# ALRhub/fancy_gym

Measured on AMD Instinct MI355X. Metric: MP trajectories/sec (7-DoF, 5 basis, 100 steps) at 1/2/4/8 GPUs; % roofline, higher is better.
Workload: dtype f32; 1 GPU; cfg2: ProDMP 7-DoF, 5 basis(+goal), 100 steps, exp phase tau=1.5, alpha=10; trajectory (pos, vel) + PD tracking-controller actions, fused; batch_per_gpu=4096, global_batch=4096, launch=hipgraph

## Files before the change

fancy_gym_amd/_lib.py:

```python
from __future__ import annotations

import ctypes as C
import os
from typing import Optional

_HERE = os.path.dirname(os.path.abspath(__file__))
LIB_PATH = os.environ.get("MPK_LIB") or os.path.join(_HERE, "libmpk.so")

MPK_ABI_VERSION = 4
MP_TYPES = {"promp": 0, "dmp": 1, "prodmp": 2}
PHASE_TYPES = {"linear": 0, "exp": 1}
BASIS_TYPES = {"rbf": 0, "zero_rbf": 1, "prodmp": 2}
CTRL_TYPES = {"motor": 0, "velocity": 1, "position": 2}
PLANT_TYPES = {"static": 0, "double_integrator": 1, "velocity_direct": 2}

MPK_EINVAL, MPK_ENOTIMPL, MPK_EHIP, MPK_ERANGE, MPK_ENODEV, MPK_ECOMM = -1, -2, -3, -4, -5, -6
MPK_COMM_ID_BYTES = 128
MPK_OPT_AUTO = -1
RELATIVE_GOAL_MODES = {"before_scale": 0, "after_scale": 1}
GOAL_OFFSET_MODES = {"ignore": 0, "add": 1}
SINGLE_RBF_MODES = {"unit_gap": 0, "refuse": 1}
DMP_FIRST_SAMPLE_MODES = {"init": 0, "step": 1}
REWARD_TYPES = {None: 0, "none": 0, "simple_reacher": 1}
AGG_MODES = {"sum": 0, "mean": 1, "last": 2}
OPTION_KEYS = ("mapping", "bulk", "quad", "pd_quad", "write_through", "ipw", "phase", "phase_table", "phase_chunk",
               "pd_simple", "split", "lds_pad", "pipe", "flat", "phase_flat", "ring", "ring_np", "ring_ns", "ring_m", "ring_dbg", "ring_parts", "tiles_wpb", "serial_order", "ring_nc", "pd_generic", "dmp_response", "ablations", "ring_tb", "pd_helper", "phase_waves", "phase_split", "phase_pipe", "pd_pipe", "hole_sampled", "vjp_generic")


class MPKLibraryError(RuntimeError):
    """libmpk.so is missing / failed to load / reported a HIP failure."""


class mpk_config(C.Structure):
    _fields_ = [
        ("abi_version", C.c_int32), ("device", C.c_int32),
        ("mp_type", C.c_int32), ("phase_type", C.c_int32), ("basis_type", C.c_int32),
        ("num_dof", C.c_int32), ("num_basis", C.c_int32), ("num_basis_outside", C.c_int32),
        ("num_basis_zero_start", C.c_int32), ("num_basis_zero_goal", C.c_int32),
        ("learn_tau", C.c_int32), ("learn_delay", C.c_int32),
        ("auto_scale_basis", C.c_int32), ("relative_goal", C.c_int32),
        ("disable_goal", C.c_int32), ("disable_weights", C.c_int32),
        ("pre_compute_length_factor", C.c_int32),
        ("relative_goal_mode", C.c_int32), ("goal_offset_mode", C.c_int32), ("single_rbf_mode", C.c_int32),
        ("dmp_first_sample", C.c_int32), ("reserved0", C.c_int32),
        ("tau", C.c_double), ("delay", C.c_double), ("alpha_phase", C.c_double),
        ("tau_bound", C.c_double * 2), ("delay_bound", C.c_double * 2),
        ("basis_bandwidth_factor", C.c_double), ("basis_alpha", C.c_double), ("basis_dt", C.c_double),
        ("weights_scale", C.c_double), ("goal_scale", C.c_double), ("dmp_alpha", C.c_double),
        ("dt", C.c_double), ("duration", C.c_double), ("goal_offset", C.c_double),
    ]


class mpk_rollout_cfg(C.Structure):
    _fields_ = [
        ("controller_type", C.c_int32), ("plant_type", C.c_int32), ("dt", C.c_double),
        ("p_gains", C.POINTER(C.c_double)), ("d_gains", C.POINTER(C.c_double)),
        ("act_low", C.POINTER(C.c_double)), ("act_high", C.POINTER(C.c_double)),
    ]


class mpk_validity_gate(C.Structure):
    _fields_ = [
        ("pos_low", C.POINTER(C.c_double)), ("pos_high", C.POINTER(C.c_double)),
        ("check_tau_delay", C.c_int32), ("reserved0", C.c_int32),
        ("tau_bound", C.c_double * 2), ("delay_bound", C.c_double * 2),
        ("raw_params", C.c_void_p), ("valid", C.c_void_p), ("penalty", C.c_void_p),
    ]


class mpk_hole_task(C.Structure):
    _fields_ = [
        ("collision_penalty", C.c_double), ("allow_self_collision", C.c_int32), ("allow_wall_collision", C.c_int32),
        ("steps_before_reward", C.c_int32), ("rew_fct", C.c_int32),
    ]


HOLE_REW_FCTS = {"simple": 0, "vel_acc": 1, "unbounded": 2}


def hole_rew_fct(rew_fct: str, steps_before_reward: int) -> int:
    if rew_fct not in HOLE_REW_FCTS:
        raise ValueError("Unknown reward function {}".format(rew_fct))
    if rew_fct != "simple" and int(steps_before_reward) != 199:
        raise ValueError(f"rew_fct {rew_fct!r} pays at the reference's step 199: steps_before_reward must be 199, "
                         f"got {steps_before_reward}")
    return HOLE_REW_FCTS[rew_fct]


RESET_ENVS = {"simple_reacher": 0, "hole_reacher": 1}


class mpk_reacher_reset_task(C.Structure):
    _fields_ = [
        ("env", C.c_int32), ("random_start", C.c_int32), ("target", C.c_double * 2),
        ("hole_width", C.c_double), ("hole_x", C.c_double), ("hole_depth", C.c_double),
        ("seed_base", C.c_uint64), ("seed_base_given", C.c_int32), ("reserved0", C.c_int32), ("reserved1", C.c_int64 * 2),
    ]


class mpk_obs_cfg(C.Structure):
    _fields_ = [
        ("env", C.c_int32), ("n_links", C.c_int32), ("col_mask", C.c_uint64), ("time_div", C.c_double), ("reserved", C.c_int64 * 2),
    ]


class mpk_env_step_task(C.Structure):
    _fields_ = [
        ("env", C.c_int32), ("n_links", C.c_int32), ("dt", C.c_double), ("max_episode_steps", C.c_int32), ("autoreset", C.c_int32),
        ("hole", mpk_hole_task), ("reserved", C.c_int64 * 2),
    ]


class mpk_replan_state(C.Structure):
    _fields_ = [
        ("traj_steps", C.c_void_p), ("plan_steps", C.c_void_p), ("done", C.c_void_p), ("seg_len", C.c_void_p),
        ("done_out", C.c_void_p), ("cond_pos", C.c_void_p), ("cond_vel", C.c_void_p),
        ("every", C.c_int32), ("max_planning_times", C.c_int32), ("horizon", C.c_int32), ("reserved0", C.c_int32),
    ]


_vp, _i32, _dbl = C.c_void_p, C.c_int32, C.c_double

SIGNATURES = {
    "mpk_last_error": (C.c_char_p, []),
    "mpk_abi_version": (C.c_int, []),
    "mpk_source_hash": (C.c_char_p, []),
    "mpk_device_count": (C.c_int, []),
    "mpk_create": (C.c_int, [C.POINTER(mpk_config), C.POINTER(_vp)]),
    "mpk_destroy": (None, [_vp]),
    "mpk_num_params": (C.c_int, [_vp]),
    "mpk_num_steps": (C.c_int, [_vp]),
    "mpk_num_dof": (C.c_int, [_vp]),
    "mpk_params_bounds": (C.c_int, [_vp, _vp, _vp]),
    "mpk_set_duration": (C.c_int, [_vp, _dbl, _dbl]),
    "mpk_set_option": (C.c_int, [_vp, C.c_char_p, C.c_int64]),
    "mpk_get_option": (C.c_int, [_vp, C.c_char_p, C.POINTER(C.c_int64)]),
    "mpk_times": (C.c_int, [_vp, _vp]),
    "mpk_trajectory": (C.c_int, [_vp, _vp, _vp, _vp, _vp, _dbl, _vp, _vp, _i32, _vp]),
    "mpk_trajectory_actions": (C.c_int, [_vp, _vp, _vp, _vp, _dbl, C.POINTER(mpk_rollout_cfg), _vp, _vp,
                                         _vp, _vp, _vp, _i32, _vp]),
    "mpk_trajectory_rollout": (C.c_int, [_vp, _vp, _vp, _vp, _dbl, C.POINTER(mpk_rollout_cfg), _vp, _vp, _vp,
                                         _vp, _vp, _vp, _i32, _vp]),
    "mpk_episode_reset": (C.c_int, [_vp, _vp, _vp, _vp, _vp, _vp, _vp, _vp, _vp, _vp, _i32, _vp]),
    "mpk_replan_step": (C.c_int, [_vp, _vp, _vp, _vp, _dbl, C.POINTER(mpk_rollout_cfg), _vp, _vp,
                                  C.POINTER(mpk_replan_state), _vp, _vp, _vp, _i32, _vp]),
    "mpk_episode_return": (C.c_int, [_vp, _vp, _vp, _vp, _dbl, C.POINTER(mpk_rollout_cfg), _vp, _vp, C.POINTER(mpk_replan_state),
                                     _vp, _vp, _i32, _vp, _vp, _i32, _i32, _vp, _i32, _vp]),
    "mpk_replan_step_gated": (C.c_int, [_vp, _vp, _vp, _vp, _dbl, C.POINTER(mpk_rollout_cfg), _vp, _vp,
                                        C.POINTER(mpk_replan_state), C.POINTER(mpk_validity_gate), _vp, _vp, _vp, _i32, _vp]),
    "mpk_episode_return_gated": (C.c_int, [_vp, _vp, _vp, _vp, _dbl, C.POINTER(mpk_rollout_cfg), _vp, _vp, C.POINTER(mpk_replan_state),
                                           C.POINTER(mpk_validity_gate), _vp, _vp, _i32, _vp, _vp, _i32, _i32, _vp, _i32, _vp]),
    "mpk_reward_aggregate": (C.c_int, [_vp, _vp, _vp, _i32, _vp, _i32, _i32, _vp]),
    "mpk_pd_rollout": (C.c_int, [_vp, C.POINTER(mpk_rollout_cfg), _vp, _vp, _vp, _vp, _vp, _vp, _i32, _i32, _vp]),
    "mpk_condition_gather": (C.c_int, [_vp, _vp, _vp, _vp, _vp, _vp, _i32, _i32, _vp]),
    "mpk_unpin_tables": (C.c_int, [_vp]),
    "mpk_check_range": (C.c_int, [_vp, _vp]),
    "mpk_poll_fault": (C.c_int, [_vp]),
    "mpk_gate_flags": (C.c_int, [_vp, _vp, _vp, _vp, _vp, _vp, _i32, _vp]),
    "mpk_reacher_rollout": (C.c_int, [_vp, C.POINTER(mpk_rollout_cfg), _vp, _vp, _vp, _vp, _vp, _vp, _vp, _i32, _vp,
                                      _vp, _i32, _i32, _vp]),
    "mpk_hole_reacher_rollout": (C.c_int, [_vp, C.POINTER(mpk_rollout_cfg), _vp, _vp, _vp, _vp, _vp, _vp, C.POINTER(mpk_hole_task),
                                           _vp, _vp, _vp, _vp, _i32, _vp, _vp, _vp, C.POINTER(mpk_replan_state), _i32, _i32, _vp]),
    "mpk_hole_reacher_rollout2": (C.c_int, [_vp, C.POINTER(mpk_rollout_cfg), _vp, _vp, _vp, _vp, _vp, _vp, C.POINTER(mpk_hole_task),
                                            _vp, _vp, _vp, _vp, _i32, _vp, _vp, _vp, C.POINTER(mpk_replan_state), _vp, _i32, _i32,
                                            _vp]),
    "mpk_reacher_reset": (C.c_int, [_vp, C.POINTER(mpk_reacher_reset_task), _vp, _vp, _vp, _vp, _vp, _vp, _vp, _vp, _vp, _vp,
                                    _i32, _vp]),
    "mpk_reacher_observation": (C.c_int, [_vp, C.POINTER(mpk_obs_cfg), _vp, _vp, _vp, _vp, _vp, _i32, _vp]),
    "mpk_reacher_step_observations": (C.c_int, [_vp, C.POINTER(mpk_obs_cfg), C.POINTER(mpk_rollout_cfg), _vp, _vp, _vp, _vp, _vp, _vp,
                                                _vp, _vp, _vp, _vp, _i32, _i32, _vp]),
    "mpk_replan_advance": (C.c_int, [_vp, _vp, _vp, _vp, _vp, _i32, _i32, _i32, _i32, _i32, _vp]),
    "mpk_traj_validity": (C.c_int, [_vp, _vp, _vp, _vp, _vp, _i32, _vp, _vp, _vp, _i32, _i32, _vp]),
    "mpk_traj_validity_penalty": (C.c_int, [_vp, _vp, _vp, _vp, _vp, _i32, _vp, _vp, _vp, _vp, _i32, _i32, _vp]),
    "mpk_prodmp_tables": (C.c_int, [_vp, _vp, _vp, _vp, _vp, _vp, _vp, _vp]),
    "mpk_prodmp_indices": (C.c_int, [_vp, _dbl, _vp, _vp, _vp]),
    "mpk_scaled_basis": (C.c_int, [_vp, _vp, _i32, _vp, _vp]),
    "mpk_selftest_division": (C.c_int, [_vp, C.c_float, C.c_uint32, C.c_uint64, C.POINTER(C.c_uint64), _vp]),
    "mpk_host_prodmp_tables": (C.c_int, [C.POINTER(mpk_config), _vp, _vp, _vp, _vp, _vp, _vp, _vp, _vp]),
    "mpk_host_rbf": (C.c_int, [C.POINTER(mpk_config), _vp, _vp]),
    "mpk_host_times": (C.c_int, [_dbl, _dbl, _vp, _i32]),
    "mpk_host_num_params": (C.c_int, [C.POINTER(mpk_config)]),
    "mpk_comm_unique_id": (C.c_int, [_vp]),
    "mpk_comm_create": (C.c_int, [_vp, _i32, _i32, _i32, C.POINTER(_vp)]),
    "mpk_comm_rank": (C.c_int, [_vp]),
    "mpk_comm_world": (C.c_int, [_vp]),
    "mpk_allgather": (C.c_int, [_vp, _vp, _vp, C.c_int64, _vp]),
    "mpk_comm_destroy": (None, [_vp]),
    "mpk_last_kernel": (C.c_char_p, [_vp]),
    "mpk_reacher_autoreset": (C.c_int, [_vp, C.POINTER(mpk_reacher_reset_task), C.POINTER(mpk_obs_cfg), _vp, _vp, _vp, _vp, _vp, _vp,
                                        _vp, _vp, _vp, _vp, _vp, _vp, _vp, _vp, _i32, _vp]),
    "mpk_reacher_env_step": (C.c_int, [_vp, C.POINTER(mpk_env_step_task), C.POINTER(mpk_reacher_reset_task), _vp, _vp, _vp, _vp, _vp,
                                       _vp, _vp, _vp, _vp, _vp, _vp, _vp, _vp, _vp, _vp, _i32, _vp]),
    "mpk_trajectory_vjp": (C.c_int, [_vp, _vp, _vp, _dbl, _vp, _vp, _vp, _i32, _vp]),
    "mpk_reacher_rollout_vjp": (C.c_int, [_vp, C.POINTER(mpk_rollout_cfg), _vp, _vp, _vp, _vp, _vp, _vp, _vp, _i32, _vp, _vp, _vp,
                                          _vp, _vp, _vp, _vp, _vp, _i32, _i32, _vp]),
}

_lib: Optional[C.CDLL] = None

_ROOT = os.path.dirname(_HERE)
KERNEL_UNITS = ("mpk_traj_family.hip", "mpk_traj_ring.hip", "mpk_episode.hip", "mpk_traj_launch.hip", "mpk_traj_wide.hip", "mpk_traj_vjp.hip", "mpk_traj_phase.hip",
                "mpk_phase_fused.hip", "mpk_rollout.hip", "mpk_rollout_vjp.hip", "mpk_hole.hip", "mpk_reset.hip", "mpk_obs.hip", "mpk_autoreset.hip", "mpk_env_step.hip", "mpk_misc.hip")
KERNEL_HEADERS = ("mpk_dev.h", "mpk_tile.h", "mpk_traj_tiles.h", "mpk_traj_stream.h", "mpk_traj_flat.h", "mpk_traj_ring.h", "mpk_traj_quad.h",
                  "mpk_traj_pipe.h", "mpk_traj_route.h", "mpk_reward.h", "mpk_phase.h", "mpk_trace_reader.h", "mpk_nprng.h", "mpk_plant.h", "mpk_reacher_env.h", "mpk_hole_geom.h")
SOURCE_FILES = (os.path.join(_ROOT, "include", "mpk.h"), os.path.join(_HERE, "csrc", "mpk_internal.h"),
                os.path.join(_HERE, "csrc", "mpk_host.cpp")) + \
    tuple(os.path.join(_HERE, "csrc", f) for f in KERNEL_HEADERS + KERNEL_UNITS)


def stamp(extra_flags: str = "") -> Optional[str]:
    import hashlib
    h = source_hash()
    if h is None or not extra_flags.strip():
        return h
    return h[:48] + "f1a9" + hashlib.sha256(extra_flags.strip().encode()).hexdigest()[:12]


def source_hash() -> Optional[str]:
    import hashlib
    h = hashlib.sha256()
    for path in SOURCE_FILES:
        if not os.path.exists(path):
            return None
        h.update(os.path.basename(path).encode() + b"\n")
        with open(path, "rb") as f:
            h.update(f.read())
    return h.hexdigest()


def embedded_source_hash(path: str = None) -> Optional[str]:
    import re
    path = path or LIB_PATH
    try:
        with open(path, "rb") as f:
            m = re.search(rb"MPK_SOURCE_HASH=([0-9a-f]{64}|unstamped)", f.read())
    except OSError:
        return None
    return m.group(1).decode() if m else None


def load() -> C.CDLL:
    global _lib
    if _lib is not None:
        return _lib
    if not os.path.exists(LIB_PATH):
        raise MPKLibraryError(
            f"{LIB_PATH} not found. Build it with `python -c 'import __graft_entry__ as g; g.build()'` "
            f"(hipcc --offload-arch=gfx950). fancy_gym_amd has no CPU fallback.")
    try:
        lib = C.CDLL(LIB_PATH)
    except OSError as e:
        raise MPKLibraryError(f"cannot load {LIB_PATH}: {e}") from e
    for name, (res, args) in SIGNATURES.items():
        try:
            fn = getattr(lib, name)
        except AttributeError as e:
            raise MPKLibraryError(f"{LIB_PATH} does not export {name}") from e
        fn.restype = res
        fn.argtypes = args
    if lib.mpk_abi_version() != MPK_ABI_VERSION:
        raise MPKLibraryError("libmpk.so ABI version mismatch")
    want, got = source_hash(), (lib.mpk_source_hash() or b"").decode()
    if want is not None and "MPK_LIB" not in os.environ and got != want:
        raise MPKLibraryError(
            f"{LIB_PATH} was built from other sources (stamped {got[:12]}..., checked out {want[:12]}...). Rebuild it with "
            f"`python -c 'import __graft_entry__ as g; g.build()'`.")
    _lib = lib
    return lib


def last_error() -> str:
    msg = load().mpk_last_error()
    return msg.decode() if msg else ""


def check(rc: int) -> int:
    if rc >= 0:
        return rc
    msg = last_error()
    if rc == MPK_EINVAL:
        raise ValueError(msg)
    if rc == MPK_ENOTIMPL:
        raise NotImplementedError(msg)
    if rc == MPK_ERANGE:
        raise RuntimeError(msg)
    raise MPKLibraryError(f"libmpk error {rc}: {msg}")


def set_option(key: str, value: int = MPK_OPT_AUTO, handle=None) -> None:
    check(load().mpk_set_option(handle, key.encode(), int(value)))


def get_option(key: str, handle=None) -> int:
    v = C.c_int64()
    check(load().mpk_get_option(handle, key.encode(), C.byref(v)))
    return int(v.value)


def reset_options(handle=None) -> None:
    for k in OPTION_KEYS:
        set_option(k, MPK_OPT_AUTO, handle)
```

fancy_gym_amd/csrc/mpk_host.cpp:

```cpp
#include <hip/hip_runtime.h>
#include <dlfcn.h>

#include <cmath>
#include <cstdio>
#include <cstring>
#include <limits>
#include <map>
#include <mutex>

#include "mpk_internal.h"

namespace mpk {

static thread_local std::string g_err;
void set_error(const std::string& msg) { g_err = msg; }

#define MPK_HIP(call)                                                                          \
    do {                                                                                       \
        hipError_t e_ = (call);                                                                \
        if (e_ != hipSuccess) {                                                                \
            set_error(std::string(#call) + ": " + hipGetErrorString(e_));                      \
            return MPK_EHIP;                                                                   \
        }                                                                                      \
    } while (0)
// ... 34 lines not shown
        if (i < steps / 2) {
            prod = step * (float)i;
            v = start + prod;
        } else {
            prod = step * (float)(steps - 1 - i);
            v = end - prod;
        }
        out[i - 1] = v;
    }
    return out;
}

static double unbound_phase(const mpk_config& c, double t) {
    const double s = (t - c.delay) / c.tau;
    return c.phase_type == MPK_PHASE_LINEAR ? s : std::exp(-c.alpha_phase * s);
}
static double bound_phase(const mpk_config& c, double t) {
    double s = (t - c.delay) / c.tau;
    if (c.phase_type == MPK_PHASE_LINEAR) return std::fmin(std::fmax(s, 0.0), 1.0);
    return std::exp(-c.alpha_phase * std::fmax(s, 0.0));
}

void build_rbf(const mpk_config& c, HostTables& t) {
    int n = c.num_basis;
    int outside = c.num_basis_outside;
    if (c.basis_type == MPK_BASIS_ZERO_RBF) {
        n += c.num_basis_zero_start + c.num_basis_zero_goal;
        outside = 0;
    }
    t.n_total = n;
    t.centers.assign(n, 0.0);
    t.bw.assign(n, 0.0);
    const double dist = n > 1 ? c.tau / (double)(n - 2 * outside - 1) : c.tau;
    const double lo = -outside * dist + c.delay;
    const double hi = c.tau + outside * dist + c.delay;
    for (int k = 0; k < n; ++k) {
        double ct = n > 1 ? lo + k * ((hi - lo) / (double)(n - 1)) : lo;
        if (n > 1 && k == n - 1) ct = hi;
        t.centers[k] = unbound_phase(c, ct);
    }
    for (int k = 0; k < n; ++k) {
        double gap = 1.0;
        if (n > 1) gap = k < n - 1 ? t.centers[k + 1] - t.centers[k] : t.centers[n - 1] - t.centers[n - 2];
        t.bw[k] = c.basis_bandwidth_factor / (gap * gap);
    }
}

static void rbf_row(const HostTables& t, double x, int n_used, int first, double* out) {
    double sum = 0.0;
    std::vector<double> b(t.n_total);
    for (int k = 0; k < t.n_total; ++k) {
        const double dx = x - t.centers[k];
        b[k] = std::exp(-(dx * dx * t.bw[k]) / 2.0);
        sum += b[k];
    }
    for (int k = 0; k < n_used; ++k) out[k] = t.n_total > 1 ? b[first + k] / sum : b[first + k];
}

void build_prodmp(const mpk_config& c, HostTables& t) {
    build_rbf(c, t);
    const int nb = c.num_basis, K = nb + 1;
    const float sdt = (float)c.basis_dt / (float)c.tau;
    t.scaled_dt = sdt;
    const int per_unit = (int)std::nearbyint(1.0 / (double)sdt);
    const int N = c.pre_compute_length_factor * per_unit + 1;
    t.n_pc = N;
    t.y1.resize(N); t.y2.resize(N); t.dy1.resize(N); t.dy2.resize(N);
    t.pos_basis.assign((size_t)N * K, 0.0);
    t.vel_basis.assign((size_t)N * K, 0.0);
    t.scale.assign(K, 0.0);
    const double alpha = c.basis_alpha, half = 0.5 * alpha;
    const double L = (double)c.pre_compute_length_factor;
    const double step = L / (double)(N - 1);
    std::vector<double> s(N), dp1((size_t)N * nb), dp2((size_t)N * nb), phi(nb);
    std::vector<double> p1(nb, 0.0), p2(nb, 0.0);
    for (int i = 0; i < N; ++i) {
        s[i] = (i == N - 1) ? L : i * step;
        const double e = std::exp(half * s[i]);
        t.y1[i] = std::exp(-half * s[i]);
        t.y2[i] = s[i] * t.y1[i];
        t.dy1[i] = -half * t.y1[i];
        t.dy2[i] = -half * t.y2[i] + t.y1[i];
        const double pc_time = s[i] * c.tau + c.delay;
        const double x = bound_phase(c, pc_time);
        rbf_row(t, x, nb, 0, phi.data());
        for (int k = 0; k < nb; ++k) {
            dp1[(size_t)i * nb + k] = ((s[i] * e) * x) * phi[k];
            dp2[(size_t)i * nb + k] = (e * x) * phi[k];
        }
        if (i > 0) {
            const double ds = s[i] - s[i - 1];
            for (int k = 0; k < nb; ++k) {
                p1[k] += ds * (dp1[(size_t)i * nb + k] + dp1[(size_t)(i - 1) * nb + k]) / 2.0;
                p2[k] += ds * (dp2[(size_t)i * nb + k] + dp2[(size_t)(i - 1) * nb + k]) / 2.0;
            }
        }
        const double q1 = (half * s[i] - 1.0) * e + 1.0;
        const double q2 = half * (e - 1.0);
        for (int k = 0; k < nb; ++k) {
            t.pos_basis[(size_t)i * K + k] = p2[k] * t.y2[i] - p1[k] * t.y1[i];
            t.vel_basis[(size_t)i * K + k] = p2[k] * t.dy2[i] - p1[k] * t.dy1[i];
        }
        t.pos_basis[(size_t)i * K + nb] = q2 * t.y2[i] - q1 * t.y1[i];
        t.vel_basis[(size_t)i * K + nb] = q2 * t.dy2[i] - q1 * t.dy1[i];
    }
    for (int k = 0; k < K; ++k) {
        double m = -std::numeric_limits<double>::infinity();
        for (int i = 0; i < N; ++i) m = std::fmax(m, t.pos_basis[(size_t)i * K + k]);
        t.scale[k] = 1.0 / m;
    }
}

struct CacheEntry {
    bool valid = false;
    uint32_t key = 0;
    int T = 0;
    SharedTables st;
    size_t floats = 0;
    uint64_t stamp = 0;
    bool pinned = false, deferred = false;
    unsigned long long capture_id = 0;
};

struct Handle {
    mpk_config cfg{};
    HostTables tab;
    DevCfg dev{};
    int num_cu = 256;
    double duration = 0.0, dt = 0.0;
    std::vector<float> times;
    double* d_tab = nullptr;
    std::vector<float> rows32;
    float* d_rows32 = nullptr;
    int rows32_stride = 0;
    float* d_times = nullptr;
    int32_t* d_flag = nullptr;
    unsigned* d_tickets = nullptr;
    unsigned ticket_next = 0;
    std::vector<unsigned> ticket_free;
    std::map<std::pair<unsigned long long, uintptr_t>, unsigned> ticket_of;
    std::mutex ticket_mu;
    int* h_fault = nullptr;
    int* d_fault = nullptr;
    int32_t* d_idx = nullptr;
    int idx_cap = 0;
    static constexpr int kCache = 64;
    CacheEntry cache[kCache];
    DevCfg dev_resp{};
    bool resp_ok = false;
    CacheEntry cache_resp[kCache];
    std::string kernel_name_buf;
    uint64_t stamp = 0;
    const char* last_kernel = "";
    Tuning tune;
    float* d_pre = nullptr;
    size_t pre_cap = 0;
};

static Tuning effective_tuning(const Handle* h);

static int check_cfg(const mpk_config& c) {
    if (c.abi_version != MPK_ABI_VERSION) { set_error("mpk_config.abi_version mismatch"); return MPK_EINVAL; }
    if (c.mp_type < 0 || c.mp_type > 2) { set_error("unknown mp_type"); return MPK_EINVAL; }
    if (c.phase_type < 0 || c.phase_type > 1) { set_error("unknown phase_type"); return MPK_EINVAL; }
    if (c.basis_type < 0 || c.basis_type > 2) { set_error("unknown basis_type"); return MPK_EINVAL; }
    if (c.num_dof < 0) { set_error("num_dof must be >= 0"); return MPK_EINVAL; }
    if (c.num_basis < 1) { set_error("num_basis must be >= 1 (basis length 0 is not implemented upstream)"); return MPK_EINVAL; }
    if (c.basis_type == MPK_BASIS_PRODMP && c.phase_type != MPK_PHASE_EXP) {
        set_error("prodmp basis requires the exp phase generator");
        return MPK_EINVAL;
    }
    if ((c.mp_type == MPK_MP_PRODMP) != (c.basis_type == MPK_BASIS_PRODMP)) {
        set_error("prodmp trajectory generator and prodmp basis generator must be used together");
        return MPK_EINVAL;
    }
    if (!(c.tau > 0.0)) { set_error("tau must be > 0"); return MPK_EINVAL; }
    if (!(c.dt > 0.0) || !(c.duration > 0.0)) { set_error("dt and duration must be > 0"); return MPK_EINVAL; }
    if (c.basis_type == MPK_BASIS_PRODMP && (c.pre_compute_length_factor < 1 || c.pre_compute_length_factor > 6)) {
        set_error("pre_compute_length_factor must be in [1, 6]");
        return MPK_EINVAL;
    }
    if (c.basis_type == MPK_BASIS_RBF && c.num_basis > 1 && c.num_basis - 2 * c.num_basis_outside - 1 <= 0) {
        set_error("num_basis_outside too large for num_basis");
        return MPK_EINVAL;
    }
    if (c.mp_type == MPK_MP_PRODMP && c.disable_goal && c.disable_weights) {
        set_error("disable_goal and disable_weights cannot both be set");
        return MPK_EINVAL;
    }
    if (c.relative_goal_mode < 0 || c.relative_goal_mode > 1 || c.goal_offset_mode < 0 || c.goal_offset_mode > 1 ||
        c.single_rbf_mode < 0 || c.single_rbf_mode > 1 || c.dmp_first_sample < 0 || c.dmp_first_sample > 1) {
        set_error("relative_goal_mode, goal_offset_mode, single_rbf_mode and dmp_first_sample take 0 or 1");
        return MPK_EINVAL;
    }
    if (c.goal_offset_mode == MPK_GOAL_OFFSET_ADD && !std::isfinite(c.goal_offset)) {
        set_error("goal_offset must be finite");
        return MPK_EINVAL;
    }
    if (c.single_rbf_mode == MPK_SINGLE_RBF_REFUSE && c.basis_type != MPK_BASIS_PRODMP) {
        const int n = c.num_basis + (c.basis_type == MPK_BASIS_ZERO_RBF ? c.num_basis_zero_start + c.num_basis_zero_goal : 0);
        if (n == 1) {
            set_error("a single radial basis function has no neighbouring centre to take its bandwidth from "
                      "(single_rbf_mode = MPK_SINGLE_RBF_REFUSE)");
            return MPK_EINVAL;
        }
    }
    return MPK_OK;
}

static int local_per_dof(const mpk_config& c) {
    switch (c.mp_type) {
        case MPK_MP_PROMP: return c.num_basis;
        case MPK_MP_DMP: return c.num_basis + 1;
        default: return (c.disable_weights ? 0 : c.num_basis) + (c.disable_goal ? 0 : 1);
    }
}

static void quantise(mpk_config& q) {
    auto f32 = [](double v) { return (double)(float)v; };
    q.tau = f32(q.tau); q.delay = f32(q.delay); q.alpha_phase = f32(q.alpha_phase);
    q.basis_bandwidth_factor = f32(q.basis_bandwidth_factor); q.basis_alpha = f32(q.basis_alpha);
    q.basis_dt = f32(q.basis_dt); q.weights_scale = f32(q.weights_scale); q.goal_scale = f32(q.goal_scale);
    q.dmp_alpha = f32(q.dmp_alpha); q.goal_offset = f32(q.goal_offset);
}

static void fill_devcfg(Handle* h) {
    const mpk_config& c = h->cfg;
    DevCfg& d = h->dev;
    d = DevCfg{};
    d.mp_type = c.mp_type; d.phase_type = c.phase_type; d.basis_type = c.basis_type;
    d.D = c.num_dof; d.nb = c.num_basis; d.n_total = h->tab.n_total;
    d.zs = c.basis_type == MPK_BASIS_ZERO_RBF ? c.num_basis_zero_start : 0;
    const bool zero_pad = c.basis_type == MPK_BASIS_ZERO_RBF;
    {
        const HostTables& t = h->tab;
        bool uni = c.basis_type != MPK_BASIS_PRODMP && c.phase_type == MPK_PHASE_LINEAR && t.n_total >= 2;
        if (uni) {
            const int n = t.n_total;
            const double D = (t.centers[n - 1] - t.centers[0]) / (double)(n - 1);
            for (int k = 0; k < n && uni; ++k)
                uni = std::fabs(t.centers[k] - (t.centers[0] + k * D)) <= 1e-12 * std::fabs(D) * n &&
                      std::fabs(t.bw[k] - t.bw[0]) <= 1e-12 * t.bw[0];
            const double span = std::fmax(std::fabs(1.0 - t.centers[0]), std::fabs(0.0 - t.centers[0])) + std::fabs(D) * n;
            uni = uni && 0.5 * t.bw[0] * span * span < 600.0;
        }
        d.rbf_uniform = uni ? 1 : 0;
    }
    d.relgoal_before_scale = c.relative_goal_mode == MPK_RELGOAL_BEFORE_SCALE ? 1 : 0;
    d.goal_off_on = c.mp_type == MPK_MP_PRODMP && c.goal_offset_mode == MPK_GOAL_OFFSET_ADD && c.goal_offset != 0.0 ? 1 : 0;
    d.goal_offset = (float)c.goal_offset;
    if (c.mp_type == MPK_MP_PRODMP) d.KT = c.num_basis + 3 + d.goal_off_on;
    else if (c.mp_type == MPK_MP_PROMP) d.KT = c.num_basis + (zero_pad ? 1 : 0);
    else d.KT = c.num_basis;
    d.KP = (d.KT + 3) / 4 * 4;
    d.Kloc = local_per_dof(c);
    d.off = (c.learn_tau ? 1 : 0) + (c.learn_delay ? 1 : 0);
    d.P = d.off + d.D * d.Kloc;
    d.T = steps_for(h->duration, h->dt);
    d.learn_tau = c.learn_tau; d.learn_delay = c.learn_delay;
    d.relative_goal = c.relative_goal; d.disable_goal = c.disable_goal; d.disable_weights = c.disable_weights;
    d.n_pc = h->tab.n_pc; d.len_factor = c.pre_compute_length_factor;
    d.tau = (float)c.tau; d.delay = (float)c.delay; d.alpha_phase = (float)c.alpha_phase;
    d.scaled_dt = h->tab.scaled_dt;
    d.tau_lo = (float)c.tau_bound[0]; d.tau_hi = (float)c.tau_bound[1];
    d.delay_lo = (float)c.delay_bound[0]; d.delay_hi = (float)c.delay_bound[1];
    d.ws = (float)c.weights_scale; d.gs = (float)c.goal_scale;
    d.dmp_alpha = (float)c.dmp_alpha; d.dmp_beta = (float)(c.dmp_alpha / 4.0);
    d.tab = h->d_tab;
    d.rows32 = h->d_rows32;
    d.rows32_stride = h->rows32_stride;
    d.base_times = h->d_times;
    d.t_last = h->times.empty() ? 0.f : h->times.back();
    h->resp_ok = false;
    h->dev_resp = d;
    if (c.mp_type == MPK_MP_DMP && !c.learn_tau && !c.learn_delay && d.D >= 1 && d.D <= kMaxD && c.num_basis + 3 <= kMaxKP &&
        !h->times.empty()) {
        float ds_max = 0.f;
        for (size_t i = 0; i + 1 < h->times.size(); ++i) {
            const float s0 = std::fmax((h->times[i] - d.delay) / d.tau, 0.f), s1 = std::fmax((h->times[i + 1] - d.delay) / d.tau, 0.f);
            ds_max = std::fmax(ds_max, s1 - s0);
        }
        DevCfg& r = h->dev_resp;
        r.mp_type = MPK_MP_PRODMP;
        r.dmp_resp = 1;
        r.rows32 = nullptr; r.rows32_stride = 0;
        r.KT = c.num_basis + 3;
        r.KP = (r.KT + 3) / 4 * 4;
        r.relative_goal = 0; r.disable_goal = 0; r.disable_weights = 0; r.goal_off_on = 0;
        h->resp_ok = (double)d.dmp_alpha * (double)ds_max <= 1.0;
    }
}

static int upload_times(Handle* h) {
    const int T = steps_for(h->duration, h->dt);
    if (T < 1) { set_error("duration/dt gives no time steps"); return MPK_EINVAL; }
    h->times = build_times(h->duration, T);
    if (h->d_times) { (void)hipFree(h->d_times); h->d_times = nullptr; }
    MPK_HIP(hipMalloc((void**)&h->d_times, sizeof(float) * T));
    MPK_HIP(hipMemcpy(h->d_times, h->times.data(), sizeof(float) * T, hipMemcpyHostToDevice));
    for (auto& e : h->cache) { e.valid = false; e.pinned = false; e.deferred = false; }
    for (auto& e : h->cache_resp) { e.valid = false; e.pinned = false; e.deferred = false; }
    return MPK_OK;
}

static void free_handle(Handle* h) {
    if (!h) return;
// ... 167 lines not shown
int mpk_create(const mpk_config* cfg, mpk_handle* out) {
    if (!cfg || !out) { set_error("NULL argument"); return MPK_EINVAL; }
    int rc = check_cfg(*cfg);
    if (rc != MPK_OK) return rc;
    int ndev = 0;
    if (hipGetDeviceCount(&ndev) != hipSuccess || ndev <= 0) {
        set_error("no HIP device visible: libmpk has no CPU fallback");
        return MPK_ENODEV;
    }
    if (cfg->device < 0 || cfg->device >= ndev) { set_error("device ordinal out of range"); return MPK_EINVAL; }
    MPK_ON_DEVICE(cfg->device);
    Handle* h = new Handle();
    h->cfg = *cfg;
    quantise(h->cfg);
    cfg = &h->cfg;
    h->duration = cfg->duration; h->dt = cfg->dt;
    hipDeviceProp_t prop;
    if (hipGetDeviceProperties(&prop, cfg->device) == hipSuccess) h->num_cu = prop.multiProcessorCount;
    std::vector<double> packed;
    if (cfg->basis_type == MPK_BASIS_PRODMP) {
        build_prodmp(*cfg, h->tab);
        const HostTables& t = h->tab;
        packed.reserve((size_t)t.n_pc * (4 + 2 * (cfg->num_basis + 1)));
        packed.insert(packed.end(), t.y1.begin(), t.y1.end());
        packed.insert(packed.end(), t.y2.begin(), t.y2.end());
        packed.insert(packed.end(), t.dy1.begin(), t.dy1.end());
        packed.insert(packed.end(), t.dy2.begin(), t.dy2.end());
        packed.insert(packed.end(), t.pos_basis.begin(), t.pos_basis.end());
        packed.insert(packed.end(), t.vel_basis.begin(), t.vel_basis.end());
        for (int k = 0; k <= cfg->num_basis; ++k) {
            float sc = k < cfg->num_basis ? (float)cfg->weights_scale : (float)cfg->goal_scale;
            if (cfg->auto_scale_basis) sc = (float)t.scale[k] * sc;
            packed.push_back((double)sc);
        }
        const int K = cfg->num_basis + 1;
        if (K + 2 <= 16) {
            const int KS = K + 2 <= 8 ? 8 : 16, RS = 2 * KS + 4;
            h->rows32.assign((size_t)t.n_pc * RS, 0.0f);
            h->rows32_stride = RS;
            for (int i = 0; i < t.n_pc; ++i) {
                float* r = h->rows32.data() + (size_t)i * RS;
                for (int kk = 0; kk < K; ++kk) {
                    r[2 * kk] = (float)t.pos_basis[(size_t)i * K + kk];
                    r[2 * kk + 1] = (float)t.vel_basis[(size_t)i * K + kk];
                }
                const double v[4] = {t.y1[i], t.y2[i], t.dy1[i], t.dy2[i]};
                std::memcpy(r + 2 * KS - 4, v, sizeof(v));
            }
        }
    } else {
        build_rbf(*cfg, h->tab);
        packed.insert(packed.end(), h->tab.centers.begin(), h->tab.centers.end());
        packed.insert(packed.end(), h->tab.bw.begin(), h->tab.bw.end());
        {
            const int n = h->tab.n_total;
            const double D = n > 1 ? (h->tab.centers[n - 1] - h->tab.centers[0]) / (double)(n - 1) : 0.0;
            const double bw0 = h->tab.bw[0];
            packed.push_back(bw0 * D);
            packed.push_back(0.5 * bw0 * D * D);
            packed.push_back(std::exp(-bw0 * D * D));
        }
    }
    auto fail = [&](int code) { free_handle(h); return code; };
    if (hipMalloc((void**)&h->d_tab, packed.size() * sizeof(double)) != hipSuccess) { set_error("hipMalloc(tables) failed"); return fail(MPK_EHIP); }
    if (hipMemcpy(h->d_tab, packed.data(), packed.size() * sizeof(double), hipMemcpyHostToDevice) != hipSuccess) { set_error("hipMemcpy(tables) failed"); return fail(MPK_EHIP); }
    if (!h->rows32.empty()) {
        if (hipMalloc((void**)&h->d_rows32, h->rows32.size() * sizeof(float)) != hipSuccess) { set_error("hipMalloc(row table) failed"); return fail(MPK_EHIP); }
        if (hipMemcpy(h->d_rows32, h->rows32.data(), h->rows32.size() * sizeof(float), hipMemcpyHostToDevice) != hipSuccess) { set_error("hipMemcpy(row table) failed"); return fail(MPK_EHIP); }
    }
    if (hipMalloc((void**)&h->d_flag, sizeof(int32_t)) != hipSuccess) { set_error("hipMalloc(flag) failed"); return fail(MPK_EHIP); }
    if (hipMemset(h->d_flag, 0, sizeof(int32_t)) != hipSuccess) { set_error("hipMemset(flag) failed"); return fail(MPK_EHIP); }
    if (hipHostMalloc((void**)&h->h_fault, 64, hipHostMallocMapped) != hipSuccess) { set_error("hipHostMalloc(fault word) failed"); return fail(MPK_EHIP); }
    *h->h_fault = 0;
    if (hipHostGetDevicePointer((void**)&h->d_fault, h->h_fault, 0) != hipSuccess) { set_error("hipHostGetDevicePointer(fault word) failed"); return fail(MPK_EHIP); }
    if (hipMalloc((void**)&h->d_tickets, kTicketSlots * 128) != hipSuccess) { set_error("hipMalloc(ticket counters) failed"); return fail(MPK_EHIP); }
    if (hipMemset(h->d_tickets, 0, kTicketSlots * 128) != hipSuccess) { set_error("hipMemset(ticket counters) failed"); return fail(MPK_EHIP); }
    rc = upload_times(h);
    if (rc != MPK_OK) return fail(rc);
    fill_devcfg(h);
    if (const int nf = fast_rows_floats(h->dev)) {
        if (hipMalloc((void**)&h->d_rows32, (size_t)nf * sizeof(float)) != hipSuccess) { set_error("hipMalloc(forcing-row table) failed"); return fail(MPK_EHIP); }
        rc = launch_fast_rows_table(h->dev, h->d_rows32, nullptr);
        if (rc != MPK_OK) return fail(rc);
        if (hipDeviceSynchronize() != hipSuccess) { set_error("forcing-row table kernel failed"); return fail(MPK_EHIP); }
        h->rows32_stride = fast_rows_stride(h->dev);
        fill_devcfg(h);
    }
    rc = prealloc_cache(h);
    if (rc != MPK_OK) return fail(rc);
    *out = reinterpret_cast<mpk_handle>(h);
    return MPK_OK;
}

void mpk_destroy(mpk_handle hh) { free_handle(reinterpret_cast<Handle*>(hh)); }

int mpk_num_params(mpk_handle hh) {
    if (!hh) { set_error("NULL handle"); return MPK_EINVAL; }
    return reinterpret_cast<Handle*>(hh)->dev.P;
}
int mpk_num_steps(mpk_handle hh) {
    if (!hh) { set_error("NULL handle"); return MPK_EINVAL; }
    return reinterpret_cast<Handle*>(hh)->dev.T;
}
int mpk_num_dof(mpk_handle hh) {
    if (!hh) { set_error("NULL handle"); return MPK_EINVAL; }
    return reinterpret_cast<Handle*>(hh)->dev.D;
}

int mpk_params_bounds(mpk_handle hh, float* low, float* high) {
    if (!hh || !low || !high) { set_error("NULL argument"); return MPK_EINVAL; }
    Handle* h = reinterpret_cast<Handle*>(hh);
    int i = 0;
    if (h->cfg.learn_tau) { low[i] = (float)h->cfg.tau_bound[0]; high[i] = (float)h->cfg.tau_bound[1]; ++i; }
    if (h->cfg.learn_delay) { low[i] = (float)h->cfg.delay_bound[0]; high[i] = (float)h->cfg.delay_bound[1]; ++i; }
    for (; i < h->dev.P; ++i) { low[i] = -std::numeric_limits<float>::infinity(); high[i] = std::numeric_limits<float>::infinity(); }
    return MPK_OK;
}

int mpk_set_duration(mpk_handle hh, double duration, double dt) {
    if (!hh) { set_error("NULL handle"); return MPK_EINVAL; }
    Handle* h = reinterpret_cast<Handle*>(hh);
    if (!(duration > 0.0) || !(dt > 0.0)) { set_error("dt and duration must be > 0"); return MPK_EINVAL; }
    if (duration == h->duration && dt == h->dt) return MPK_OK;
    MPK_ON_DEVICE(h->cfg.device);
    MPK_HIP(hipDeviceSynchronize());
    h->duration = duration; h->dt = dt;
    release_capture_tickets(h);
    int rc = upload_times(h);
    if (rc != MPK_OK) return rc;
    fill_devcfg(h);
    return prealloc_cache(h);
}

namespace {
struct OptKey { const char* name; int Tuning::*field; int64_t lo, hi; };
const OptKey kOptKeys[] = {
    {"mapping", &Tuning::mapping, 0, 2},         {"bulk", &Tuning::bulk, 0, 2},
    {"quad", &Tuning::quad, 0, 4},               {"pd_quad", &Tuning::pd_quad, 0, 3},
    {"write_through", &Tuning::write_through, 0, 1}, {"ipw", &Tuning::ipw, 0, 1 << 20},
    {"phase", &Tuning::phase, 0, 1},             {"phase_table", &Tuning::phase_table, 0, 1},
    {"phase_chunk", &Tuning::phase_chunk, 0, 16}, {"pd_simple", &Tuning::pd_simple, 0, 1},
    {"split", &Tuning::split, 0, 1},             {"lds_pad", &Tuning::lds_pad, 0, 48},
    {"pipe", &Tuning::pipe, 0, 1},               {"flat", &Tuning::flat, 0, 1},
    {"phase_flat", &Tuning::phase_flat, 0, 1},   {"ring", &Tuning::ring, 0, 2},
    {"ring_np", &Tuning::ring_np, 1, 14},        {"ring_ns", &Tuning::ring_ns, 1, 8},
    {"ring_m", &Tuning::ring_m, 1, 8},           {"ring_dbg", &Tuning::ring_dbg, 0, 255},
    {"ring_parts", &Tuning::ring_parts, 1, 8},   {"tiles_wpb", &Tuning::tiles_wpb, 1, 8},
    {"serial_order", &Tuning::serial_order, 0, 2}, {"ring_nc", &Tuning::ring_nc, 1, 6},
    {"pd_generic", &Tuning::pd_generic, 0, 1},   {"dmp_response", &Tuning::dmp_response, 0, 1},
    {"ablations", &Tuning::ablations, 0, 1},     {"ring_tb", &Tuning::ring_tb, 1, 64},
    {"pd_helper", &Tuning::pd_helper, 0, 1},     {"phase_waves", &Tuning::phase_waves, 1, 32},
    {"phase_split", &Tuning::phase_split, 1, 64},   {"phase_pipe", &Tuning::phase_pipe, 0, 1},
    {"pd_pipe", &Tuning::pd_pipe, 0, 1},         {"hole_sampled", &Tuning::hole_sampled, 0, 1},
    {"vjp_generic", &Tuning::vjp_generic, 0, 1},
};
const OptKey* find_opt(const char* key) {
    if (!key) return nullptr;
    for (const OptKey& k : kOptKeys)
        if (std::strcmp(k.name, key) == 0) return &k;
    return nullptr;
}
}

namespace mpk {
static Tuning effective_tuning(const Handle* h) {
    Tuning t = g_tune;
    for (const OptKey& k : kOptKeys)
        if (h->tune.*(k.field) >= 0) t.*(k.field) = h->tune.*(k.field);
    return t;
}
}

int mpk_set_option(mpk_handle hh, const char* key, int64_t value) {
    const OptKey* k = find_opt(key);
    if (!k) { set_error(std::string("unknown option key: ") + (key ? key : "(null)")); return MPK_EINVAL; }
    if (value != MPK_OPT_AUTO && (value < k->lo || value > k->hi)) {
        set_error(std::string("option value out of range for ") + key);
        return MPK_EINVAL;
    }
    Tuning& t = hh ? reinterpret_cast<Handle*>(hh)->tune : g_tune;
    t.*(k->field) = (int)value;
    return MPK_OK;
}

int mpk_get_option(mpk_handle hh, const char* key, int64_t* value) {
    const OptKey* k = find_opt(key);
    if (!k || !value) { set_error(std::string("unknown option key: ") + (key ? key : "(null)")); return MPK_EINVAL; }
    const Tuning t = hh ? effective_tuning(reinterpret_cast<Handle*>(hh)) : g_tune;
    *value = t.*(k->field);
    return MPK_OK;
}

int mpk_check_range(mpk_handle hh, void* stream) {
    if (!hh) { set_error("NULL handle"); return MPK_EINVAL; }
    Handle* h = reinterpret_cast<Handle*>(hh);
    MPK_ON_DEVICE(h->cfg.device);
    int32_t flag = 0;
    MPK_HIP(hipMemcpyAsync(&flag, h->d_flag, sizeof(flag), hipMemcpyDeviceToHost, (hipStream_t)stream));
    MPK_HIP(hipStreamSynchronize((hipStream_t)stream));
    {
        const int fr = pending_ring_fault(h);
        if (fr != MPK_OK) {
            if (flag) {
                MPK_HIP(hipMemsetAsync(h->d_flag, 0, sizeof(flag), (hipStream_t)stream));
                set_error(std::string(mpk_last_error()) + "; ALSO: Time is beyond the pre-computation range. Set larger pre-computation factor");
            }
            return fr;
        }
    }
    if (!flag) return MPK_OK;
    MPK_HIP(hipMemsetAsync(h->d_flag, 0, sizeof(flag), (hipStream_t)stream));
    set_error("Time is beyond the pre-computation range. Set larger pre-computation factor");
    return MPK_ERANGE;
}

int mpk_poll_fault(mpk_handle hh) {
    if (!hh) { set_error("NULL handle"); return MPK_EINVAL; }
    return pending_ring_fault(reinterpret_cast<Handle*>(hh));
}

static void release_capture_tickets(Handle* h) {
    std::lock_guard<std::mutex> lock(h->ticket_mu);
    for (auto it = h->ticket_of.begin(); it != h->ticket_of.end();) {
        if (it->first.first != 0ull) { h->ticket_free.push_back(it->second); it = h->ticket_of.erase(it); }
        else ++it;
    }
}

int mpk_unpin_tables(mpk_handle hh) {
    if (!hh) { set_error("NULL handle"); return MPK_EINVAL; }
    Handle* h = reinterpret_cast<Handle*>(hh);
    release_capture_tickets(h);
    for (auto* cache : {h->cache, h->cache_resp})
        for (int i = 0; i < Handle::kCache; ++i) {
            CacheEntry& e = cache[i];
            if (e.pinned) { e.pinned = false; if (e.deferred) e.valid = false; e.deferred = false; }
        }
    return MPK_OK;
}

int mpk_times(mpk_handle hh, float* times) {
    if (!hh || !times) { set_error("NULL argument"); return MPK_EINVAL; }
    Handle* h = reinterpret_cast<Handle*>(hh);
    std::memcpy(times, h->times.data(), sizeof(float) * h->times.size());
    return MPK_OK;
}

static unsigned* ticket_slot(Handle* h, void* stream) {
    unsigned long long cap_id = 0;
    hipStreamCaptureStatus cs = hipStreamCaptureStatusNone;
    if (hipStreamGetCaptureInfo((hipStream_t)stream, &cs, &cap_id) != hipSuccess) { (void)hipGetLastError(); cs = hipStreamCaptureStatusNone; }
    if (cs != hipStreamCaptureStatusActive) cap_id = 0;
    std::lock_guard<std::mutex> lock(h->ticket_mu);
    const auto key = std::make_pair(cap_id, reinterpret_cast<uintptr_t>(stream));
    auto it = h->ticket_of.find(key);
    if (it == h->ticket_of.end()) {
        unsigned slot;
        if (!h->ticket_free.empty()) { slot = h->ticket_free.back(); h->ticket_free.pop_back(); }
        else if (h->ticket_next < kTicketSlots) slot = h->ticket_next++;
        else return nullptr;
        it = h->ticket_of.emplace(key, slot).first;
    }
    return h->d_tickets + (size_t)it->second * 32;
}

static int pending_ring_fault(Handle* h) {
    if (!h->h_fault) return MPK_OK;
    const int f = __atomic_exchange_n(h->h_fault, 0, __ATOMIC_RELAXED);
    if (!(f & 2)) { if (f) __atomic_fetch_or(h->h_fault, f & ~2, __ATOMIC_RELAXED); return MPK_OK; }
    char msg[512];
    std::snprintf(msg, sizeof msg, "k_traj_ring: a wave of an earlier launch on this handle gave up waiting for its partner (role mask 0x%x: "
                  "1 producer / buffer, 2 ticket, 4 store engine / batch, 8 action writer, 16 consumer / tile, 32 consumer / writer, 64 reward helper, 128 k_phase_fused pipeline, 256 rollout pipeline, 512 k_reacher_reset goal draw at its rejection cap): "
                  "outputs (closed loop: plant and replanning state too) of that launch are incomplete", (unsigned)f >> 8);
    set_error(msg);
    return MPK_EHIP;
}

static bool fused_capable(const Handle* h) {
    if (!shared_phase(h, nullptr)) return false;
    if (h->cfg.mp_type == MPK_MP_DMP) return dmp_response(h, nullptr, effective_tuning(h));
    return mfma_capable(h);
}

static bool fused_phase_capable(const Handle* h) {
    return !shared_phase(h, nullptr) && h->cfg.mp_type != MPK_MP_DMP && phase_fused_capable(h->dev);
}

static int fill_gate(const Handle* h, const mpk_validity_gate* g, GateDev* out) {
    if (!g->pos_low || !g->pos_high || !g->valid) { set_error("validity gate: NULL pos_low / pos_high / valid"); return MPK_EINVAL; }
    if (h->dev.D > kMaxD) { set_error("validity gate: num_dof too large"); return MPK_EINVAL; }
    for (int d = 0; d < h->dev.D; ++d) { out->lo[d] = g->pos_low[d]; out->hi[d] = g->pos_high[d]; }
    out->check_td = g->check_tau_delay ? 1 : 0;
    if (out->check_td && h->dev.P < 2) { set_error("validity gate: check_tau_delay needs at least two parameters per episode"); return MPK_EINVAL; }
    out->tau_b[0] = g->tau_bound[0]; out->tau_b[1] = g->tau_bound[1];
    out->delay_b[0] = g->delay_bound[0]; out->delay_b[1] = g->delay_bound[1];
    out->raw_params = g->raw_params; out->valid = g->valid; out->penalty = g->penalty;
    return MPK_OK;
}

static int phase_fused_common(Handle* h, const float* params, const float* init_pos, const float* init_vel, double init_time_shared,
                              float* pos, float* vel, float* actions, const RolloutDev& rd, double* q, double* qd,
                              const int32_t* n_steps, const ReplanDev* rp, const GateDev* gate, double* ret, int32_t* seg_out,
                              int32_t B, void* stream) {
    if (!params || !init_pos || !init_vel) { set_error("NULL buffer"); return MPK_EINVAL; }
    {
        const int fr = pending_ring_fault(h);
        if (fr != MPK_OK) return fr;
    }
    return launch_phase_fused(h->dev, params, init_pos, init_vel, (float)init_time_shared, pos, vel, actions, rd, q, qd, n_steps, rp,
                              gate, ret, seg_out, h->d_flag, B, h->num_cu, stream, &h->last_kernel, effective_tuning(h), h->d_fault);
}

static int traj_common(Handle* h, const float* params, const float* init_pos, const float* init_vel,
                       const float* init_time, double init_time_shared, float* pos, float* vel, float* actions,
                       const RolloutDev* rd, const double* c_pos, const double* c_vel, int32_t B, void* stream,
                       double* q_state = nullptr, double* qd_state = nullptr, const int32_t* n_steps = nullptr,
                       const ReplanDev* rp = nullptr, const GateDev* gate = nullptr) {
    if (B < 0) { set_error("B must be >= 0"); return MPK_EINVAL; }
    if (B == 0 || h->dev.D == 0) return MPK_OK;
    if (!params || !init_pos || !init_vel || !pos || !vel) { set_error("NULL buffer"); return MPK_EINVAL; }
    MPK_ON_DEVICE(h->cfg.device);
    {
        const int fr = pending_ring_fault(h);
        if (fr != MPK_OK) return fr;
    }
    const Tuning tune = effective_tuning(h);
    if (h->cfg.mp_type == MPK_MP_DMP && h->cfg.dmp_first_sample == MPK_DMP_FIRST_IS_STEP) {
        const size_t need = (size_t)B * h->dev.D;
        if (need > h->pre_cap) {
            hipStreamCaptureStatus cs = hipStreamCaptureStatusNone;
            if (hipStreamIsCapturing((hipStream_t)stream, &cs) == hipSuccess && cs == hipStreamCaptureStatusActive) {
                set_error("MPK_DMP_FIRST_IS_STEP: run one eager call with this batch size before capturing a graph");
                return MPK_EINVAL;
            }
            if (h->d_pre) { MPK_HIP(hipDeviceSynchronize()); (void)hipFree(h->d_pre); h->d_pre = nullptr; h->pre_cap = 0; }
            MPK_HIP(hipMalloc((void**)&h->d_pre, 2 * need * sizeof(float)));
            h->pre_cap = need;
        }
        float* p1 = h->d_pre;
        float* v1 = h->d_pre + h->pre_cap;
        int rc = launch_dmp_prestep(h->dev, params, init_pos, init_vel, init_time, (float)init_time_shared, p1, v1, B, stream);
        if (rc != MPK_OK) return rc;
        init_pos = p1; init_vel = v1;
    }
    if (shared_phase(h, init_time) && wide_capable(h) && !actions && !q_state && !rp && traj_wide_fits(h->dev)) {
        SharedTables st;
        int rc = get_shared(h, (float)init_time_shared, stream, &st);
        if (rc != MPK_OK) return rc;
        rc = launch_traj_wide(h->dev, st, params, init_pos, init_vel, pos, vel, B, h->num_cu, stream, &h->last_kernel);
        if (rc != MPK_ENOTIMPL) return rc;
    }
    if (dmp_response(h, init_time, tune)) {
        SharedTables st;
        int rc = get_shared(h, (float)init_time_shared, stream, &st, true);
        if (rc != MPK_OK) return rc;
        unsigned* ticket = ticket_slot(h, stream);
        const char* name = "";
        rc = launch_traj_shared(h->dev_resp, st, params, init_pos, init_vel, pos, vel, actions, rd, c_pos, c_vel,
                                q_state, qd_state, n_steps, B, h->num_cu, stream, &name, tune, rp, ticket, h->d_fault, gate);
        if (rc == MPK_OK) {
            h->kernel_name_buf = name;
            const size_t at = h->kernel_name_buf.find("prodmp");
            if (at != std::string::npos) h->kernel_name_buf.replace(at, 6, "dmp_resp");
            h->last_kernel = h->kernel_name_buf.c_str();
        }
        if (rc != MPK_ENOTIMPL || actions) return rc;
    }
    if (shared_phase(h, init_time) && mfma_capable(h)) {
        SharedTables st;
        int rc = get_shared(h, (float)init_time_shared, stream, &st);
        if (rc != MPK_OK) return rc;
        unsigned* ticket = ticket_slot(h, stream);
        rc = launch_traj_shared(h->dev, st, params, init_pos, init_vel, pos, vel, actions, rd, c_pos, c_vel,
                                q_state, qd_state, n_steps, B, h->num_cu, stream, &h->last_kernel, tune, rp, ticket, h->d_fault, gate);
        if (rc != MPK_ENOTIMPL || actions) return rc;
    }
    if (actions) { set_error("fused actions need a shared-phase configuration with D <= 16 and <= 16 basis columns"); return MPK_ENOTIMPL; }
    return launch_traj_rows(h->dev, params, init_pos, init_vel, init_time, (float)init_time_shared, pos, vel,
                            h->d_flag, B, h->num_cu, stream, &h->last_kernel, tune);
}

int mpk_trajectory(mpk_handle hh, const float* params, const float* init_pos, const float* init_vel,
                   const float* init_time, double init_time_shared, float* pos, float* vel, int32_t B,
                   void* stream) {
    if (!hh) { set_error("NULL handle"); return MPK_EINVAL; }
    return traj_common(reinterpret_cast<Handle*>(hh), params, init_pos, init_vel, init_time, init_time_shared,
                       pos, vel, nullptr, nullptr, nullptr, nullptr, B, stream);
}

int mpk_trajectory_vjp(mpk_handle hh, const float* g_pos, const float* g_vel, double init_time_shared, float* g_params,
                       float* g_init_pos, float* g_init_vel, int32_t B, void* stream) {
    if (!hh) { set_error("NULL handle"); return MPK_EINVAL; }
    Handle* h = reinterpret_cast<Handle*>(hh);
    if (B < 0) { set_error("B must be >= 0"); return MPK_EINVAL; }
    if (h->cfg.learn_tau || h->cfg.learn_delay) {
        set_error("mpk_trajectory_vjp: a learned tau / delay makes the trajectory non-linear in those two parameters (and they are "
                  "clipped to their bounds): only shared-phase handles are differentiable");
        return MPK_ENOTIMPL;
    }
    const Tuning tune = effective_tuning(h);
    const bool dmp = h->cfg.mp_type == MPK_MP_DMP;
    if (dmp && (h->cfg.dmp_first_sample == MPK_DMP_FIRST_IS_STEP || !dmp_response(h, nullptr, tune))) {
        set_error("mpk_trajectory_vjp: a DMP handle is differentiable on its response route only (<= 16 DoF, <= 13 basis functions, "
                  "alpha ds <= 1, dmp_first_sample = init, option \"dmp_response\" not 0)");
        return MPK_ENOTIMPL;
    }
    if (B == 0 || h->dev.D == 0 || (!g_params && !g_init_pos && !g_init_vel)) return MPK_OK;
    MPK_ON_DEVICE(h->cfg.device);
    SharedTables st;
    int rc = get_shared(h, (float)init_time_shared, stream, &st, dmp);
    if (rc != MPK_OK) return rc;
    return launch_traj_vjp(dmp ? h->dev_resp : h->dev, st, g_pos, g_vel, g_params, g_init_pos, g_init_vel, B, h->num_cu, stream,
                           &h->last_kernel, tune);
}

int mpk_trajectory_actions(mpk_handle hh, const float* params, const float* init_pos, const float* init_vel,
                           double init_time_shared, const mpk_rollout_cfg* rc, const double* c_pos,
                           const double* c_vel, float* pos, float* vel, float* actions, int32_t B, void* stream) {
    if (!hh) { set_error("NULL handle"); return MPK_EINVAL; }
    Handle* h = reinterpret_cast<Handle*>(hh);
    if (B == 0) return MPK_OK;
    if (!actions || !c_pos || !c_vel) { set_error("NULL buffer"); return MPK_EINVAL; }
    RolloutDev rd;
    int r = fill_rollout(h, rc, &rd);
    if (r != MPK_OK) return r;
    MPK_ON_DEVICE(h->cfg.device);
    if (rd.plant_type != MPK_PLANT_STATIC) { set_error("mpk_trajectory_actions tracks a frozen state (MPK_PLANT_STATIC); use mpk_trajectory_rollout"); return MPK_EINVAL; }
    if (fused_capable(h)) {
        r = traj_common(h, params, init_pos, init_vel, nullptr, init_time_shared, pos, vel, actions, &rd, c_pos, c_vel,
                        B, stream);
        if (r != MPK_ENOTIMPL) return r;
    } else if (fused_phase_capable(h) && B > 0 && pos && vel) {
        r = phase_fused_common(h, params, init_pos, init_vel, init_time_shared, pos, vel, actions, rd, const_cast<double*>(c_pos),
                               const_cast<double*>(c_vel), nullptr, nullptr, nullptr, nullptr, nullptr, B, stream);
        if (r != MPK_ENOTIMPL) return r;
    }
    r = traj_common(h, params, init_pos, init_vel, nullptr, init_time_shared, pos, vel, nullptr, nullptr, nullptr,
                    nullptr, B, stream);
    if (r != MPK_OK) return r;
    return launch_pd_rollout(rd, h->dev.D, pos, vel, const_cast<double*>(c_pos), const_cast<double*>(c_vel), nullptr,
                             actions, B, h->dev.T, stream, effective_tuning(h), h->d_fault);
}

int mpk_trajectory_rollout(mpk_handle hh, const float* params, const float* init_pos, const float* init_vel,
                           double init_time_shared, const mpk_rollout_cfg* rc, double* q, double* qd,
                           const int32_t* n_steps, float* pos, float* vel, float* actions, int32_t B, void* stream) {
    if (!hh) { set_error("NULL handle"); return MPK_EINVAL; }
    Handle* h = reinterpret_cast<Handle*>(hh);
    if (B == 0) return MPK_OK;
    if (!actions || !q || !qd) { set_error("NULL buffer"); return MPK_EINVAL; }
    RolloutDev rd;
    int r = fill_rollout(h, rc, &rd);
    if (r != MPK_OK) return r;
    MPK_ON_DEVICE(h->cfg.device);
    if (rd.plant_type != MPK_PLANT_DOUBLE_INTEGRATOR) { set_error("mpk_trajectory_rollout integrates MPK_PLANT_DOUBLE_INTEGRATOR; for a frozen state use mpk_trajectory_actions"); return MPK_EINVAL; }
    if (fused_capable(h)) {
        r = traj_common(h, params, init_pos, init_vel, nullptr, init_time_shared, pos, vel, actions, &rd, nullptr,
                        nullptr, B, stream, q, qd, n_steps);
        if (r != MPK_ENOTIMPL) return r;
    } else if (fused_phase_capable(h) && B > 0 && pos && vel) {
        r = phase_fused_common(h, params, init_pos, init_vel, init_time_shared, pos, vel, actions, rd, q, qd, n_steps, nullptr, nullptr,
                               nullptr, nullptr, B, stream);
        if (r != MPK_ENOTIMPL) return r;
    }
    r = traj_common(h, params, init_pos, init_vel, nullptr, init_time_shared, pos, vel, nullptr, nullptr, nullptr,
                    nullptr, B, stream);
    if (r != MPK_OK) return r;
    return launch_pd_rollout(rd, h->dev.D, pos, vel, q, qd, n_steps, actions, B, h->dev.T, stream, effective_tuning(h), h->d_fault);
}

int mpk_replan_step_gated(mpk_handle hh, const float* params, const float* init_pos, const float* init_vel,
                          double init_time_shared, const mpk_rollout_cfg* rc, double* q, double* qd,
                          const mpk_replan_state* st, const mpk_validity_gate* gate, float* pos, float* vel, float* actions,
                          int32_t B, void* stream) {
    if (!hh) { set_error("NULL handle"); return MPK_EINVAL; }
    Handle* h = reinterpret_cast<Handle*>(hh);
    if (B < 0) { set_error("B must be >= 0"); return MPK_EINVAL; }
    if (B == 0) return MPK_OK;
    if (!st || !st->traj_steps || !st->plan_steps || !st->done || !st->seg_len) { set_error("NULL replanning state"); return MPK_EINVAL; }
    if ((st->cond_pos == nullptr) != (st->cond_vel == nullptr)) { set_error("cond_pos and cond_vel go together"); return MPK_EINVAL; }
    if (st->every < 1 || st->horizon < 1) { set_error("every and horizon must be >= 1"); return MPK_EINVAL; }
    if (!actions || !q || !qd) { set_error("NULL buffer"); return MPK_EINVAL; }
    if (st->cond_pos && (st->cond_pos == init_pos || st->cond_vel == init_vel)) { set_error("cond_pos / cond_vel must not alias init_pos / init_vel"); return MPK_EINVAL; }
    RolloutDev rd;
    int r = fill_rollout(h, rc, &rd);
    if (r != MPK_OK) return r;
    if (rd.plant_type != MPK_PLANT_DOUBLE_INTEGRATOR) { set_error("mpk_replan_step integrates MPK_PLANT_DOUBLE_INTEGRATOR"); return MPK_EINVAL; }
    GateDev gd;
    if (gate) {
        r = fill_gate(h, gate, &gd);
        if (r != MPK_OK) return r;
    }
    MPK_ON_DEVICE(h->cfg.device);
    ReplanDev rp;
    rp.traj_steps = st->traj_steps; rp.plan_steps = st->plan_steps; rp.done = st->done; rp.seg_len = st->seg_len;
    rp.done_out = st->done_out; rp.cond_pos = st->cond_pos; rp.cond_vel = st->cond_vel;
    rp.every = st->every; rp.max_planning_times = st->max_planning_times; rp.horizon = st->horizon;
    if (fused_capable(h)) {
        r = traj_common(h, params, init_pos, init_vel, nullptr, init_time_shared, pos, vel, actions, &rd, nullptr,
                        nullptr, B, stream, q, qd, nullptr, &rp, gate ? &gd : nullptr);
        if (r != MPK_ENOTIMPL) return r;
    } else if (fused_phase_capable(h) && pos && vel) {
        r = phase_fused_common(h, params, init_pos, init_vel, init_time_shared, pos, vel, actions, rd, q, qd, nullptr, &rp,
                               gate ? &gd : nullptr, nullptr, nullptr, B, stream);
        if (r != MPK_ENOTIMPL) return r;
    }
    r = traj_common(h, params, init_pos, init_vel, nullptr, init_time_shared, pos, vel, nullptr, nullptr, nullptr,
                    nullptr, B, stream);
    if (r != MPK_OK) return r;
    if (gate) {
        r = launch_validity(pos, gd.raw_params ? gd.raw_params : params, h->dev.P, h->dev.D, gd.lo, gd.hi, gd.check_td, gd.tau_b, gd.delay_b,
                            gd.valid, gd.penalty, B, h->dev.T, stream);
        if (r != MPK_OK) return r;
    }
    r = launch_replan_advance(rp.traj_steps, rp.plan_steps, rp.seg_len, rp.done, rp.every, rp.max_planning_times,
                              rp.horizon, h->dev.T, B, stream, gate ? gd.valid : nullptr);
    if (r != MPK_OK) return r;
    if (rp.done_out) MPK_HIP(hipMemcpyAsync(rp.done_out, rp.done, (size_t)B, hipMemcpyDeviceToDevice, (hipStream_t)stream));
    r = launch_pd_rollout(rd, h->dev.D, pos, vel, q, qd, rp.seg_len, actions, B, h->dev.T, stream, effective_tuning(h), h->d_fault);
    if (r != MPK_OK) return r;
    if (rp.cond_pos) return launch_condition_gather(pos, vel, rp.seg_len, rp.cond_pos, rp.cond_vel, B, h->dev.T, h->dev.D, stream);
    return MPK_OK;
}

int mpk_replan_step(mpk_handle hh, const float* params, const float* init_pos, const float* init_vel,
                    double init_time_shared, const mpk_rollout_cfg* rc, double* q, double* qd,
                    const mpk_replan_state* st, float* pos, float* vel, float* actions, int32_t B, void* stream) {
// ... 724 lines not shown
```

fancy_gym_amd/csrc/mpk_internal.h:

```cpp
#pragma once
#include <cstdint>
#include <string>
#include <vector>

#include "mpk.h"

namespace mpk {

constexpr int kMaxKP = 16;
constexpr int kMaxD = 16;
constexpr int kMaxDofArgs = 32;

struct HostTables {
    int n_total = 0;
    std::vector<double> centers, bw;
    int n_pc = 0;
    float scaled_dt = 0.f;
    std::vector<double> y1, y2, dy1, dy2, pos_basis, vel_basis, scale;
};

void build_rbf(const mpk_config& c, HostTables& t);
void build_prodmp(const mpk_config& c, HostTables& t);
std::vector<float> build_times(double duration, int T);
int steps_for(double duration, double dt);

struct Tuning {
    int mapping = -1, bulk = -1, quad = -1, pd_quad = -1, write_through = -1, ipw = -1, phase = -1, phase_table = -1,
        phase_chunk = -1, pd_simple = -1, split = -1, lds_pad = -1, pipe = -1, flat = -1, phase_flat = -1,
        ring = -1, ring_np = -1, ring_ns = -1, ring_m = -1, ring_dbg = -1, ring_parts = -1, tiles_wpb = -1, serial_order = -1, ring_nc = -1,
        pd_generic = -1, dmp_response = -1, ablations = -1, ring_tb = -1, pd_helper = -1, phase_waves = -1, phase_split = -1, phase_pipe = -1, pd_pipe = -1,
        hole_sampled = -1, vjp_generic = -1;
};

struct DevCfg {
    int mp_type, phase_type, basis_type;
    int D, nb, n_total, zs;
    int KT, KP;
    int P, Kloc, off;
    int T;
    int learn_tau, learn_delay, relative_goal, disable_goal, disable_weights;
    int rbf_uniform;
    int relgoal_before_scale;
    int dmp_resp;
    int goal_off_on;
    float goal_offset;
    int n_pc, len_factor;
    float tau, delay, alpha_phase, scaled_dt;
    float tau_lo, tau_hi, delay_lo, delay_hi;
    float ws, gs, dmp_alpha, dmp_beta;
    const double* tab;
    const float* rows32;
    int rows32_stride;
    const float* base_times;
    float t_last;
};

struct RolloutDev {
    int controller_type, plant_type;
    double dt;
    double pg[kMaxDofArgs], dg[kMaxDofArgs], lo[kMaxDofArgs], hi[kMaxDofArgs];
};

struct ReplanDev {
    int32_t* traj_steps = nullptr;
    int32_t* plan_steps = nullptr;
    uint8_t* done = nullptr;
    int32_t* seg_len = nullptr;
    uint8_t* done_out = nullptr;
    float* cond_pos = nullptr;
    float* cond_vel = nullptr;
    int every = 1, max_planning_times = 0, horizon = 0;
};

inline float f32_at_least(double x) {
    float f = (float)x;
    if ((double)f < x) f = __builtin_nextafterf(f, __builtin_inff());
    return f;
}
inline float f32_at_most(double x) {
    float f = (float)x;
    if ((double)f > x) f = __builtin_nextafterf(f, -__builtin_inff());
    return f;
}

struct GateDev {
    double lo[kMaxD], hi[kMaxD];
    int check_td = 0;
    double tau_b[2] = {0.0, 0.0}, delay_b[2] = {0.0, 0.0};
    const float* raw_params = nullptr;
    uint8_t* valid = nullptr;
    double* penalty = nullptr;
};

struct SharedTables {
    float* A = nullptr;
    float* aux = nullptr;
    int TS = 0, n_out = 0;
};

struct Handle;

int launch_build_shared(const DevCfg& c, float init_time, const SharedTables& st, int32_t* idx_out,
                        int32_t* range_flag, void* stream);
int launch_traj_shared(const DevCfg& c, const SharedTables& st, const float* params, const float* init_pos,
                       const float* init_vel, float* pos, float* vel, float* actions, const RolloutDev* rc,
                       const double* c_pos, const double* c_vel, double* q_state, double* qd_state,
                       const int32_t* n_steps, int B, int num_cu, void* stream, const char** kernel_name,
                       const Tuning& tune, const ReplanDev* rp = nullptr, unsigned* ticket = nullptr, int* fault = nullptr,
                       const GateDev* gate = nullptr);
int launch_episode_return(const DevCfg& c, const SharedTables& st, const float* params, const float* init_pos, const float* init_vel,
                          const RolloutDev& rc, double* q_state, double* qd_state, const int32_t* n_steps, const ReplanDev* rp,
                          int reward_type, const double* goal, const int32_t* step0, int steps_before_reward, int agg, double* ret,
                          int32_t* seg_out, int B, int num_cu, void* stream, const char** kernel_name, const Tuning& tune,
                          const GateDev* gate = nullptr);
int launch_reward_aggregate(const double* rewards, const int32_t* seg_len, int agg, double* out, int B, int T, void* stream);
int launch_traj_wide(const DevCfg& c, const SharedTables& st, const float* params, const float* init_pos,
                     const float* init_vel, float* pos, float* vel, int B, int num_cu, void* stream,
                     const char** kernel_name);
int launch_traj_vjp(const DevCfg& c, const SharedTables& st, const float* g_pos, const float* g_vel, float* g_params, float* g_init_pos,
                    float* g_init_vel, int B, int num_cu, void* stream, const char** kernel_name, const Tuning& tune);
int launch_traj_rows(const DevCfg& c, const float* params, const float* init_pos, const float* init_vel,
                     const float* init_time, float init_time_shared, float* pos, float* vel, int32_t* range_flag,
                     int B, int num_cu, void* stream, const char** kernel_name, const Tuning& tune);
int launch_pd_rollout(const RolloutDev& rc, int D, const float* des_pos, const float* des_vel, double* q,
                      double* qd, const int32_t* n_steps, float* actions, int B, int T, void* stream,
                      const Tuning& tune, int* fault = nullptr);
bool phase_fused_capable(const DevCfg& c);
int launch_phase_fused(const DevCfg& c, const float* params, const float* init_pos, const float* init_vel, float init_time_shared,
                       float* pos, float* vel, float* actions, const RolloutDev& rc, double* q, double* qd, const int32_t* n_steps,
                       const ReplanDev* rp, const GateDev* gate, double* ret, int32_t* seg_out, int32_t* range_flag, int B, int num_cu,
                       void* stream, const char** kernel_name, const Tuning& tune, int* fault);
int fast_rows_floats(const DevCfg& c);
int fast_rows_stride(const DevCfg& c);
int launch_fast_rows_table(const DevCfg& c, float* out, void* stream);
int launch_dmp_prestep(const DevCfg& c, const float* params, const float* init_pos, const float* init_vel,
                       const float* init_time, float init_time_shared, float* pos1, float* vel1, int B, void* stream);
int launch_condition_gather(const float* pos, const float* vel, const int32_t* seg_len, float* cond_pos, float* cond_vel,
                            int B, int T, int D, void* stream);
int launch_reacher_rollout(const RolloutDev& rc, int D, const float* des_pos, const float* des_vel, double* q,
                           double* qd, const int32_t* n_steps, const int32_t* step0, const double* goal,
                           int steps_before_reward, float* actions, double* rewards, int B, int T, void* stream,
                           const Tuning& tune, int* fault);
int launch_reacher_rollout_vjp(const RolloutDev& rc, int D, const float* des_pos, const float* des_vel, const double* q0,
                               const double* qd0, const int32_t* n_steps, const int32_t* step0, const double* goal,
                               int steps_before_reward, const double* g_rewards, const double* g_q, const double* g_qd,
                               float* g_des_pos, float* g_des_vel, double* g_q0, double* g_qd0, double* g_goal, int B, int T,
                               void* stream, const char** kernel_name);
struct HoleLaunch {
    RolloutDev rc;
    const float* des_pos = nullptr;
    const float* des_vel = nullptr;
    double* q = nullptr;
    double* qd = nullptr;
    const int32_t* n_steps = nullptr;
    const int32_t* step0 = nullptr;
    const double* hole = nullptr;
    float* actions = nullptr;
    double* rewards = nullptr;
    double* ret = nullptr;
    int32_t* n_exec = nullptr;
    uint8_t* collided = nullptr;
    uint8_t* success = nullptr;
    ReplanDev rp;
    double penalty = 0.0;
    int allow_self = 0, allow_wall = 0, steps_before_reward = 0, agg = 0;
    int rew_fct = 0;
    double* reward_state = nullptr;
};
int launch_hole_rollout(const HoleLaunch& h, int B, int T, int D, void* stream, const Tuning& tune);
int launch_episode_reset(const double* init_q, const double* init_qd, double* q, double* qd, float* cond_pos,
                         float* cond_vel, int32_t* traj_steps, int32_t* plan_steps, uint8_t* done, int B, int D,
                         void* stream);
struct ResetLaunch {
    const uint64_t* seeds = nullptr;
    uint64_t seed_base = 0;
    int seeded_base = 0;
    void* rng = nullptr;
    double* q = nullptr;
    double* qd = nullptr;
    float* cond_pos = nullptr;
    float* cond_vel = nullptr;
    int32_t* traj_steps = nullptr;
    int32_t* plan_steps = nullptr;
    uint8_t* done = nullptr;
    double* task_out = nullptr;
    double target[2] = {0.0, 0.0};
    double hole_width = 0.0, hole_x = 0.0, hole_depth = 0.0;
    int env = 0, random_start = 0;
};
int launch_reacher_reset(const ResetLaunch& l, int B, int D, void* stream, int* fault);
struct ObsLaunch {
    uint64_t mask = 0;
    double time_div = 0.0;
    int env = 0, D = 0, n_full = 0, n_out = 0;
};
int launch_reacher_obs(const ObsLaunch& l, const double* q, const double* qd, const double* task, const int32_t* steps, float* out,
                       int B, void* stream);
int launch_reacher_step_obs(const ObsLaunch& l, const RolloutDev& rc, const float* des_pos, const float* des_vel, const double* q0,
                            const double* qd0, const double* task, const int32_t* n_exec, const int32_t* step0, float* out,
                            double* q_end, double* qd_end, int B, int T, void* stream);
int launch_reacher_autoreset(const ResetLaunch& l, const ObsLaunch* o, const uint8_t* mask, uint8_t* reset_mask, float* final_obs,
                             float* obs, int B, int D, void* stream, int* fault);
struct EnvStepLaunch {
    ResetLaunch reset;
    ObsLaunch obs_layout;
    const float* actions = nullptr;
    double* reward_state = nullptr;
    double* reward = nullptr;
    uint8_t* terminated = nullptr;
    uint8_t* truncated = nullptr;
    uint8_t* collided = nullptr;
    uint8_t* success = nullptr;
    uint8_t* reset_mask = nullptr;
    float* final_obs = nullptr;
    float* obs = nullptr;
    double dt = 0.0, penalty = 0.0;
    int allow_self = 0, allow_wall = 0, steps_before_reward = 0, max_steps = 0, autoreset = 0, rew_fct = 0;
};
int launch_reacher_env_step(const EnvStepLaunch& e, int B, int D, void* stream, int* fault);
int launch_gate_flags(const uint8_t* valid, const uint8_t* was_done, const uint8_t* done, uint8_t* terminated, uint8_t* truncated, int B,
                      void* stream);
int launch_replan_advance(int32_t* traj_steps, int32_t* plan_steps, int32_t* seg_len, uint8_t* done, int every,
                          int max_planning_times, int horizon, int T, int B, void* stream, const uint8_t* valid = nullptr);
int launch_validity(const float* pos, const float* params, int P, int D, const double* lo, const double* hi,
                    int check_td, const double* tb, const double* db, uint8_t* valid, double* penalty, int B, int T,
                    void* stream);

int launch_scaled_basis(const DevCfg& c, const float* times, int n, float* out, void* stream);
int launch_div_sweep(float d, uint32_t first, uint64_t count, unsigned long long* mismatches, void* stream);

size_t shared_tables_floats(const DevCfg& c, int* TS, int* n_out);
bool shared_tables_lean(const DevCfg& c);
bool traj_wide_fits(const DevCfg& c);


void set_error(const std::string& msg);

}
```

fancy_gym_amd/csrc/mpk_tile.h:

```cpp
#pragma once
#include "mpk_dev.h"

namespace mpk {

struct TrajArgs {
    DevCfg c;
    const float* A;
    const float* aux;
    int TS;
    const float* params;
    const float* init_pos;
    const float* init_vel;
    float* pos;
    float* vel;
    float* actions;
    const double* c_pos;
    const double* c_vel;
    int B, sh, G, vec_ok;
    int pitch, cps, shifted, td3;
    unsigned inv_cps;
    unsigned nrt_magic;
    int gstride;
    int wt;
    int flat_img;
    int ring_np, ring_ns, ring_m, ring_nbuf;
    int ring_nc;
    int ring_aw;
    unsigned* ring_ctr;
    int ring_tb;
    int ring_parts;
    int burst;
    int lean;
    int inorder;
    int wpb;
    int ring_dbg;
    int* fault;
    unsigned ser_blocks;
    double* q_state;
    double* qd_state;
    const int32_t* n_steps;
    double plant_dt;
    ReplanDev rp;
    uint8_t* gate_valid;
    double* gate_penalty;
    const float* gate_raw;
    int gate_check_td;
    double gate_tb[2], gate_db[2];
};

struct ActArgs {
    double pg[kMaxD], dg[kMaxD], lo[kMaxD], hi[kMaxD];
    double glo[kMaxD], ghi[kMaxD];
    float glo32[kMaxD], ghi32[kMaxD];
};

constexpr int kStageStride = 256;
constexpr int kStageFloats = 4 * kStageStride;

struct EpArgs {
    double* ret;
    const double* goal;
    const int32_t* step0;
    int32_t* seg_out;
    int steps_before_reward;
    int agg;
    int km;
    int wpb;
};

constexpr int kEpImg = 4 * kStageStride + 8;
constexpr int kEpImgPlain = 2 * kStageStride + 8;
constexpr int kEpSlots = 8;
constexpr int kEpMaxPass = 2;
constexpr int kEpSlotInts = 8;


enum : int { XK_ZERO = 0, XK_PARAM = 1, XK_IPOS = 2, XK_IVEL = 3, XK_ONE = 4 };

template <int MP>
__device__ __forceinline__ int x_kind(const DevCfg& c, int k, int* loc) {
    const int nb = c.nb;
    if (MP == MPK_MP_PRODMP) {
        const bool isw = k < nb, isg = k == nb;
        *loc = (isw && !c.disable_weights) ? k : ((isg && !c.disable_goal && !c.disable_weights) ? nb : 0);
        const int kw = c.disable_weights ? XK_ZERO : XK_PARAM, kg = c.disable_goal ? XK_ZERO : XK_PARAM;
        const int klast = (k == nb + 3 && c.goal_off_on) ? XK_ONE : XK_ZERO;
        return isw ? kw : (isg ? kg : (k == nb + 1 ? XK_IPOS : (k == nb + 2 ? XK_IVEL : klast)));
    } else if (MP == MPK_MP_PROMP) {
        const bool isw = k < nb;
        *loc = isw ? k : 0;
        return isw ? XK_PARAM : ((k == nb && c.KT > nb) ? XK_IPOS : XK_ZERO);
    } else {
        const bool isw = k < nb;
        *loc = isw ? k : 0;
        return isw ? XK_PARAM : XK_ZERO;
    }
}

template <int KM>
struct LaneMap {
    int col, q, bl, d, dsafe, NTW;
    bool dvalid;
    bool isp[KM], isip[KM], isiv[KM];
    float cst[KM];
    unsigned poff[KM];
    unsigned ioff;
    unsigned wofs;
    int sseg, w4;
    unsigned rofs, gofs;
};

template <int MP, int KM>
__device__ __forceinline__ LaneMap<KM> make_lane_map(const TrajArgs& a, int lane) {
    const DevCfg& c = a.c;
    LaneMap<KM> L;
    const int D = c.D, DP = 1 << a.sh;
    L.NTW = 16 >> a.sh;
    L.col = lane & 15; L.q = lane >> 4;
    L.bl = L.col >> a.sh; L.d = L.col & (DP - 1);
    L.dvalid = L.d < D;
    L.dsafe = L.dvalid ? L.d : D - 1;
#pragma unroll
    for (int m = 0; m < KM; ++m) {
        int loc;
        const int kind = x_kind<MP>(c, 4 * m + L.q, &loc);
        L.isp[m] = L.dvalid && kind == XK_PARAM;
        L.isip[m] = L.dvalid && kind == XK_IPOS;
        L.isiv[m] = L.dvalid && kind == XK_IVEL;
        L.cst[m] = L.dvalid && kind == XK_ONE ? 1.0f : 0.0f;
        L.poff[m] = (unsigned)(L.bl * c.P + c.off + L.dsafe * c.Kloc + loc);
    }
    L.ioff = (unsigned)(L.bl * D + L.dsafe);
    L.wofs = (unsigned)(L.bl * a.pitch + 4 * L.q * D + L.d);
    L.sseg = (int)(((unsigned)lane * a.inv_cps) >> 16);
    L.w4 = (lane - L.sseg * a.cps) * 4;
    L.rofs = (unsigned)(L.sseg * a.pitch + L.w4);
    L.gofs = (unsigned)(L.sseg * c.T * D + L.w4);
    return L;
}

__device__ __forceinline__ unsigned ep_shift(const TrajArgs& a, int b) {
    return a.shifted ? (((unsigned)b & 3u) * (unsigned)a.td3) & 3u : 0u;
}

template <int KM>
struct GroupIn {
    float raw[KM];
    float ip, iv;
    double cp, cv;
};

template <class T>
__device__ __forceinline__ T ld_off(const T* base, unsigned byte_off) {
    return *reinterpret_cast<const T*>(reinterpret_cast<const char*>(base) + byte_off);
}

template <int MP, bool ACT, int KM>
__device__ __forceinline__ GroupIn<KM> load_group(const TrajArgs& a, const LaneMap<KM>& L, int g) {
    const DevCfg& c = a.c;
    GroupIn<KM> in;
    const int b0 = g * L.NTW;
    const bool bv = b0 + L.bl < a.B;
    const float* pb = a.params + (size_t)b0 * c.P;
    const unsigned io = bv ? L.ioff : (unsigned)L.dsafe;
    const unsigned pclamp = bv ? 0u : (unsigned)(L.bl * c.P);
#pragma unroll
    for (int m = 0; m < KM; ++m) in.raw[m] = ld_off(pb, 4u * (L.poff[m] - pclamp));
    in.ip = MP != MPK_MP_DMP ? ld_off(a.init_pos + (size_t)b0 * c.D, 4u * io) : 0.0f;
    in.iv = MP == MPK_MP_PRODMP ? ld_off(a.init_vel + (size_t)b0 * c.D, 4u * io) : 0.0f;
    in.cp = 0.0; in.cv = 0.0;
    if (ACT) { in.cp = ld_off(a.c_pos + (size_t)b0 * c.D, 8u * io); in.cv = ld_off(a.c_vel + (size_t)b0 * c.D, 8u * io); }
    return in;
}

template <int KM>
__device__ __forceinline__ void finish_group(const LaneMap<KM>& L, const GroupIn<KM>& in, float (&xb)[KM]) {
#pragma unroll
    for (int m = 0; m < KM; ++m) xb[m] = L.isp[m] ? in.raw[m] : (L.isip[m] ? in.ip : (L.isiv[m] ? in.iv : L.cst[m]));
}

__device__ __forceinline__ void park_gains(const ActArgs& act, int lane, int d, float* sSt) {
    double pgd = 0.0, dgd = 0.0, lod = 0.0, hid = 0.0;
#pragma unroll
    for (int dd = 0; dd < kMaxD; ++dd)
        if (dd == d) { pgd = act.pg[dd]; dgd = act.dg[dd]; lod = act.lo[dd]; hid = act.hi[dd]; }
    if (lane < 16) {
        double* sg = reinterpret_cast<double*>(sSt + 3 * kStageStride);
        sg[lane] = pgd; sg[16 + lane] = dgd; sg[32 + lane] = lod; sg[48 + lane] = hid;
    }
    __builtin_amdgcn_wave_barrier();
}

struct Gains { double pg, dg, lo, hi; };

__device__ __forceinline__ Gains parked_gains(const double* sg) { return Gains{sg[0], sg[16], sg[32], sg[48]}; }

constexpr size_t kActArgsOffset = (sizeof(TrajArgs) + alignof(ActArgs) - 1) / alignof(ActArgs) * alignof(ActArgs);
__device__ __forceinline__ Gains kernarg_gains(int d) {
    typedef const __attribute__((address_space(4))) char* kptr;
    kptr base = (kptr)__builtin_amdgcn_kernarg_segment_ptr() + kActArgsOffset;
    typedef const __attribute__((address_space(4))) double* dptr;
    Gains gn;
    gn.pg = ((dptr)(base + offsetof(ActArgs, pg)))[d];
    gn.dg = ((dptr)(base + offsetof(ActArgs, dg)))[d];
    gn.lo = ((dptr)(base + offsetof(ActArgs, lo)))[d];
    gn.hi = ((dptr)(base + offsetof(ActArgs, hi)))[d];
    return gn;
}

struct GateLim { double lo, hi; float lo32, hi32; };
__device__ __forceinline__ GateLim kernarg_gate(int d) {
    typedef const __attribute__((address_space(4))) char* kptr;
    kptr base = (kptr)__builtin_amdgcn_kernarg_segment_ptr() + kActArgsOffset;
    typedef const __attribute__((address_space(4))) double* dptr;
    typedef const __attribute__((address_space(4))) float* fptr;
    GateLim g;
    g.lo = ((dptr)(base + offsetof(ActArgs, glo)))[d];
    g.hi = ((dptr)(base + offsetof(ActArgs, ghi)))[d];
    g.lo32 = ((fptr)(base + offsetof(ActArgs, glo32)))[d];
    g.hi32 = ((fptr)(base + offsetof(ActArgs, ghi32)))[d];
    return g;
}

__device__ __forceinline__ float fmax_nan(float a, float b) { return __builtin_elementwise_maximum(a, b); }
__device__ __forceinline__ float fmin_nan(float a, float b) { return __builtin_elementwise_minimum(a, b); }
template <int NQ>
struct GateScan {
    float mx[NQ], mn[NQ];
    unsigned long long tiles;
    unsigned nan;
    __device__ __forceinline__ void init(const GateLim& gl) {
#pragma unroll
        for (int j = 0; j < NQ; ++j) { mx[j] = gl.lo32; mn[j] = gl.hi32; }
        tiles = 0ull;
        nan = (gl.lo != gl.lo || gl.hi != gl.hi) ? ~0u : 0u;
    }
};
template <int NQ>
__device__ __forceinline__ bool gate_scan_tile(GateScan<NQ>& g, const int j, f32x4 acc, const int rt, const int lq, const bool dvalid,
                                               const GateLim& gl, const int T) {
    if ((rt + 1) * 16 > T) {
        const int row0 = rt * 16 + 4 * lq;
#pragma unroll
        for (int r = 0; r < 4; ++r) acc[r] = row0 + r < T ? acc[r] : gl.lo32;
    }
    float hi4 = fmax_nan(fmax_nan(acc[0], acc[1]), fmax_nan(acc[2], acc[3]));
    float lo4 = fmin_nan(fmin_nan(acc[0], acc[1]), fmin_nan(acc[2], acc[3]));
    if (__any(hi4 != hi4) != 0) {
        if (hi4 != hi4) g.nan |= 1u << j;
        hi4 = __builtin_fmaxf(__builtin_fmaxf(acc[0], acc[1]), __builtin_fmaxf(acc[2], acc[3]));
        lo4 = __builtin_fminf(__builtin_fminf(acc[0], acc[1]), __builtin_fminf(acc[2], acc[3]));
    }
    g.mx[j] = __builtin_fmaxf(g.mx[j], hi4); g.mn[j] = __builtin_fminf(g.mn[j], lo4);
    return dvalid && (hi4 > gl.hi32 || lo4 < gl.lo32);
}
template <int KM, int NQ>
__device__ __forceinline__ bool gate_verdict(const TrajArgs& a, const LaneMap<KM>& L, const GateScan<NQ>& g, const float* __restrict__ ap,
                                             const int TS, const int km, const float (&xz)[NQ][KM], const int g0, const GateLim& gl,
                                             double& over, double& under, bool& pnan) {
    const int T = a.c.T, NRT = (T + 15) >> 4;
    const int DP = 1 << a.sh;
    const unsigned long long em = (unsigned long long)(((1u << DP) - 1u) << (L.bl * DP)) * 0x0001000100010001ull;
    unsigned long long any = 0ull;
    bool mine = false;
    pnan = false;
#pragma unroll
    for (int j = 0; j < NQ; ++j) {
        const bool ep = L.dvalid && (g0 + j) * L.NTW + L.bl < a.B;
        const unsigned long long mj = __ballot(ep && (g.mx[j] > gl.hi32 || g.mn[j] < gl.lo32));
        const unsigned long long nj = __ballot(ep && ((g.nan >> j) & 1u));
        any |= mj;
        if (L.q == j) { mine = (mj & em) != 0ull; pnan = (nj & em) != 0ull; }
    }
    over = 0.0; under = 0.0;
    if (any != 0ull) {
        double ov[NQ], un[NQ];
#pragma unroll
        for (int j = 0; j < NQ; ++j) { ov[j] = 0.0; un[j] = 0.0; }
        for (int rt = 0; rt < NRT; ++rt) {
            if (rt < 64 && !((g.tiles >> rt) & 1ull)) continue;
            float af[KM];
#pragma unroll
            for (int m = 0; m < KM; ++m) af[m] = m < km ? ap[(4 * m) * TS + rt * 16] : 0.0f;
            const int row0 = rt * 16 + 4 * L.q;
#pragma unroll
            for (int j = 0; j < NQ; ++j) {
                f32x4 acc = {0.f, 0.f, 0.f, 0.f};
#pragma unroll
                for (int m = 0; m < KM; ++m)
                    if (m < km) acc = __builtin_amdgcn_mfma_f32_16x16x4f32(af[m], xz[j][m], acc, 0, 0, 0);
#pragma unroll
                for (int r = 0; r < 4; ++r) {
                    const double x = (double)acc[r];
                    const bool in = row0 + r < T && L.dvalid;
                    ov[j] += in ? gate_excess(x - gl.hi) : 0.0;
                    un[j] += in ? gate_excess(gl.lo - x) : 0.0;
                }
            }
        }
#pragma unroll
        for (int j = 0; j < NQ; ++j) {
            for (int sft = 16; sft <= 32; sft <<= 1) { ov[j] += __shfl_xor(ov[j], sft); un[j] += __shfl_xor(un[j], sft); }
            for (int sft = 1; sft < DP; sft <<= 1) { ov[j] += __shfl_xor(ov[j], sft); un[j] += __shfl_xor(un[j], sft); }
            if (L.q == j) { over = ov[j]; under = un[j]; }
        }
    }
    return mine;
}
template <int KM, int NQ>
__device__ __forceinline__ bool gate_pass(const TrajArgs& a, const LaneMap<KM>& L, const float* __restrict__ ap, const int TS, const int km,
                                          const float (&xb)[NQ][KM], const int g0, const GateLim& gl, double& over, double& under,
                                          bool& pnan) {
    const int T = a.c.T, NRT = (T + 15) >> 4;
    float xz[NQ][KM];
#pragma unroll
    for (int j = 0; j < NQ; ++j)
#pragma unroll
        for (int m = 0; m < KM; ++m) xz[j][m] = g0 + j < a.G ? xb[j][m] : 0.0f;
    GateScan<NQ> g;
    g.init(gl);
    constexpr int UN = 4;
    for (int rt0 = 0; rt0 < NRT; rt0 += UN) {
        float af[UN][KM];
#pragma unroll
        for (int u = 0; u < UN; ++u)
// ... 137 lines not shown

__device__ __forceinline__ void dmp_tile_steps(const float* __restrict__ sF, float* __restrict__ sP, float* __restrict__ sV,
                                               const float* __restrict__ ds16, const int stride, const int t0,
                                               const int T, const float alpha, const float beta, const float eg,
                                               const TauDiv& td, float& ey, float& ez) {
    float fr[16], dsr[16];
#pragma unroll
    for (int tl = 0; tl < 16; ++tl) fr[tl] = sF[tl * stride];
#pragma unroll
    for (int j = 0; j < 4; ++j) {
        const float4 x = reinterpret_cast<const float4*>(ds16)[j];
        dsr[4 * j] = x.x; dsr[4 * j + 1] = x.y; dsr[4 * j + 2] = x.z; dsr[4 * j + 3] = x.w;
    }
#pragma unroll
    for (int tl = 0; tl < 16; ++tl) {
        sP[tl * stride] = ey;
        sV[tl * stride] = div_tau(ez, td);
        const float t1 = eg - ey;
        const float t2 = beta * t1;
        const float t3 = t2 - ez;
        const float t4 = alpha * t3;
        const float acc = t4 + fr[tl];
        const float ez_n = ez + dsr[tl] * acc;
        const float ey_n = ey + dsr[tl] * ez_n;
        const bool live = t0 + tl < T - 1;
        ez = live ? ez_n : ez;
        ey = live ? ey_n : ey;
    }
}

template <int MP, int CT>
__device__ __forceinline__ void tile_epilogue(const f32x4& acc0, const f32x4& acc1, const f32x4& acc2,
                                              const float (&dtd)[4], double cp, double cv, const Gains& gn,
                                              float* sSt, unsigned wofs, int D, const int astride = kStageStride,
                                              const int nrows = 4) {
    const double pgd = gn.pg, dgd = gn.dg, lod = gn.lo, hid = gn.hi;
#pragma unroll
    for (int r = 0; r < 4; ++r) {
        if (r >= nrows) break;
        const float p = acc0[r];
        float v;
        if (MP == MPK_MP_PRODMP) v = acc1[r];
        else v = (acc1[r] - acc2[r]) * dtd[r];
        float* w = sSt + wofs + r * D;
        w[0] = p;
        w[astride] = v;
        if (CT >= 0 && CT < 3) {
            double u;
            if (CT == MPK_CTRL_MOTOR) u = pgd * ((double)p - cp) + dgd * ((double)v - cv);
            else if (CT == MPK_CTRL_POSITION) u = (double)p;
            else u = (double)v;
            u = fmin(fmax(u, lod), hid);
            w[2 * astride] = (float)u;
        }
        if (CT >= 3) w[2 * astride] = 0.0f;
    }
}

__device__ __forceinline__ unsigned lds_addr(const float* p) { return (unsigned)reinterpret_cast<uintptr_t>(p); }
template <int OFF>
__device__ __forceinline__ void lds_w32(const unsigned ad, const float v) {
    static_assert(OFF >= 0 && OFF < 65536, "ds offset field");
    asm volatile("ds_write_b32 %0, %1 offset:%2" ::"v"(ad), "v"(v), "n"(OFF));
}
template <int OFF>
__device__ __forceinline__ float lds_r32(const unsigned ad) {
    static_assert(OFF >= 0 && OFF < 65536, "ds offset field");
    float v;
    asm volatile("ds_read_b32 %0, %1 offset:%2" : "=v"(v) : "v"(ad), "n"(OFF));
    return v;
}

__device__ __noinline__ void store_tile_generic(float* pos, float* vel, float* actions, int mask, int B, int T, int D,
                                                int NTW, const float* sSt, int lane, int b0, int rt, int rows) {
    const int SEG = 16 * D, len = rows * D;
    for (int j = 0; j < 3; ++j) {
        if (!((mask >> j) & 1)) continue;
        float* outp = j == 0 ? pos : (j == 1 ? vel : actions);
        for (int sb = 0; sb < NTW; ++sb) {
            const int bb = b0 + sb;
            if (bb >= B) continue;
            float* gp = outp + ((size_t)bb * T + rt * 16) * D;
            for (int e = lane; e < len; e += 64) gp[e] = sSt[j * kStageStride + sb * SEG + e];
        }
    }
}

#ifndef MPK_WT_PRED
#define MPK_WT_PRED 0
#endif
#ifndef MPK_WT_ASM
#define MPK_WT_ASM 1
#endif
#ifndef MPK_STORE_AUX
#define MPK_STORE_AUX 16
#endif
typedef int i32x4_t __attribute__((ext_vector_type(4)));
typedef int i32x2_t __attribute__((ext_vector_type(2)));
struct WtDst { __amdgpu_buffer_rsrc_t rsrc; unsigned off; };
__device__ __forceinline__ WtDst wt_dst(const float* p) {
    const unsigned long long pu = reinterpret_cast<unsigned long long>(p);
    const unsigned lo = __builtin_amdgcn_readfirstlane((unsigned)pu), hi = __builtin_amdgcn_readfirstlane((unsigned)(pu >> 32));
    const unsigned long long base = (((unsigned long long)hi << 32) | lo) - (1ull << 30);
    WtDst d;
    d.rsrc = __builtin_amdgcn_make_buffer_rsrc(reinterpret_cast<void*>(base), 0, -1, 0x00020000);
    d.off = (unsigned)pu - (unsigned)base;
    return d;
}

template <bool WT>
__device__ __forceinline__ void store16(float* p, const f32x4& v) {
    if (WT && MPK_WT_ASM) {
        asm volatile("global_store_dwordx4 %0, %1, off sc1\n\ts_nop 1" ::"v"(p), "v"(v) : "memory");
    } else if (WT) {
        const WtDst d = wt_dst(p);
        __builtin_amdgcn_raw_buffer_store_b128(__builtin_bit_cast(i32x4_t, v), d.rsrc, (int)d.off, 0, MPK_STORE_AUX);
    } else {
        *reinterpret_cast<f32x4*>(p) = v;
    }
}

template <bool WT>
__device__ __forceinline__ void store8(float* p, const f32x2& v) {
    if (WT && MPK_WT_ASM) {
        asm volatile("global_store_dwordx2 %0, %1, off sc1\n\ts_nop 1" ::"v"(p), "v"(v) : "memory");
    } else if (WT) {
        const WtDst d = wt_dst(p);
        __builtin_amdgcn_raw_buffer_store_b64(__builtin_bit_cast(i32x2_t, v), d.rsrc, (int)d.off, 0, MPK_STORE_AUX);
    } else {
        *reinterpret_cast<f32x2*>(p) = v;
    }
}

template <bool WT>
__device__ __forceinline__ void store4(float* p, float v) {
    if (WT && MPK_WT_ASM) {
        asm volatile("global_store_dword %0, %1, off sc1\n\ts_nop 1" ::"v"(p), "v"(v) : "memory");
    } else if (WT) {
        const WtDst d = wt_dst(p);
        __builtin_amdgcn_raw_buffer_store_b32(__builtin_bit_cast(int, v), d.rsrc, (int)d.off, 0, MPK_STORE_AUX);
    } else {
        *p = v;
    }
}

constexpr unsigned kWtSkip = 0xFFFFFFF0u;
__device__ __forceinline__ __amdgpu_buffer_rsrc_t wt_rsrc(const float* base_uniform) {
    return __builtin_amdgcn_make_buffer_rsrc(const_cast<float*>(base_uniform), 0, (int)0x80000000u, 0x00020000);
}
__device__ __forceinline__ void wt_store16(__amdgpu_buffer_rsrc_t r, unsigned off, const f32x4& v) {
    __builtin_amdgcn_raw_buffer_store_b128(__builtin_bit_cast(i32x4_t, v), r, (int)off, 0, MPK_STORE_AUX);
}

template <int MASK, int KM, bool WT>
__device__ __forceinline__ void tile_store_sel(const TrajArgs& a, const LaneMap<KM>& L, const float* sSt, int lane,
                                               int b0, int rt, int rows) {
    constexpr bool SP = (MASK & 1) != 0, SV = (MASK & 2) != 0, SA = (MASK & 4) != 0;
    const int D = a.c.D, T = a.c.T, len = rows * D;
    if (a.vec_ok) {
        const int bb = b0 + L.sseg;
        const int lo = (int)ep_shift(a, bb), hi = lo + len, c0 = L.w4;
        const bool in_seg = L.sseg < L.NTW && bb < a.B && c0 < hi && c0 + 4 > lo;
        if (WT && MPK_WT_PRED) {
            const bool whole = in_seg && c0 >= lo && c0 + 4 <= hi;
            const unsigned off = whole ? (unsigned)((((size_t)bb * T + rt * 16) * D - lo + c0) * sizeof(float)) : kWtSkip;
            const unsigned ro = L.sseg < L.NTW ? L.rofs : 0u;
            if (SP) wt_store16(wt_rsrc(a.pos), off, *reinterpret_cast<const f32x4*>(sSt + ro));
            if (SV) wt_store16(wt_rsrc(a.vel), off, *reinterpret_cast<const f32x4*>(sSt + kStageStride + ro));
            if (SA) wt_store16(wt_rsrc(a.actions), off, *reinterpret_cast<const f32x4*>(sSt + 2 * kStageStride + ro));
            if (!a.shifted) return;
        }
        if (in_seg) {
            const size_t go = ((size_t)bb * T + rt * 16) * D - lo + c0;
            f32x4 d0 = {0.f, 0.f, 0.f, 0.f}, d1 = d0, d2 = d0;
            if (SP) d0 = *reinterpret_cast<const f32x4*>(sSt + L.rofs);
            if (SV) d1 = *reinterpret_cast<const f32x4*>(sSt + kStageStride + L.rofs);
            if (SA) d2 = *reinterpret_cast<const f32x4*>(sSt + 2 * kStageStride + L.rofs);
            if (c0 >= lo && c0 + 4 <= hi) {
                if (!(WT && MPK_WT_PRED)) {
                    if (SP) store16<WT>(a.pos + go, d0);
                    if (SV) store16<WT>(a.vel + go, d1);
                    if (SA) store16<WT>(a.actions + go, d2);
                }
            } else if (a.td3 == 2) {
                const bool head = c0 < lo;
                const int o = head ? 2 : 0;
                const f32x2 p2 = {head ? d0[2] : d0[0], head ? d0[3] : d0[1]};
                const f32x2 v2 = {head ? d1[2] : d1[0], head ? d1[3] : d1[1]};
                if (SP) store8<WT>(a.pos + go + o, p2);
                if (SV) store8<WT>(a.vel + go + o, v2);
                if (SA) {
                    const f32x2 a2 = {head ? d2[2] : d2[0], head ? d2[3] : d2[1]};
                    store8<WT>(a.actions + go + o, a2);
                }
            } else {
#pragma unroll
                for (int e = 0; e < 4; ++e) {
                    if (c0 + e >= lo && c0 + e < hi) {
                        if (SP) store4<WT>(a.pos + go + e, d0[e]);
                        if (SV) store4<WT>(a.vel + go + e, d1[e]);
                        if (SA) store4<WT>(a.actions + go + e, d2[e]);
                    }
                }
            }
        }
    } else {
        store_tile_generic(a.pos, a.vel, a.actions, MASK, a.B, T, D, L.NTW, sSt, lane, b0, rt, rows);
    }
}

template <int NST, int KM, bool WT>
__device__ __forceinline__ void tile_store(const TrajArgs& a, const LaneMap<KM>& L, const float* sSt, int lane,
                                           int b0, int rt, int rows) {
    tile_store_sel<(NST > 2 ? 7 : 3), KM, WT>(a, L, sSt, lane, b0, rt, rows);
}

__device__ __forceinline__ void demand_args(const TrajArgs& a, unsigned grid_x) {
    asm volatile("" ::"s"(grid_x), "s"(a.c.D), "s"(a.c.nb), "s"(a.c.KT), "s"(a.c.P), "s"(a.c.Kloc), "s"(a.c.off), "s"(a.c.T),
                 "s"(a.c.disable_weights), "s"(a.c.disable_goal), "s"(a.c.goal_off_on), "s"(a.A), "s"(a.aux), "s"(a.TS), "s"(a.params),
                 "s"(a.init_pos), "s"(a.init_vel), "s"(a.pos), "s"(a.vel), "s"(a.actions), "s"(a.c_pos), "s"(a.c_vel),
                 "s"(a.sh), "s"(a.G), "s"(a.vec_ok), "s"(a.pitch), "s"(a.cps), "s"(a.shifted), "s"(a.td3),
                 "s"(a.inv_cps), "s"(a.nrt_magic), "s"(a.gstride));
}

__device__ __forceinline__ void load_ds16(const float* __restrict__ p, float (&v)[16]) {
#pragma unroll
    for (int j = 0; j < 4; ++j) {
        const float4 x = reinterpret_cast<const float4*>(p)[j];
        v[4 * j] = x.x; v[4 * j + 1] = x.y; v[4 * j + 2] = x.z; v[4 * j + 3] = x.w;
    }
}

}
```

fancy_gym_amd/csrc/mpk_traj_family.hip:

```cpp
#include "mpk_traj_tiles.h"
#include "mpk_traj_stream.h"
#include "mpk_traj_flat.h"
#include "mpk_traj_quad.h"
#include "mpk_traj_pipe.h"
#include "mpk_traj_route.h"

namespace mpk {

#ifndef MPK_DEVICE_ONLY
template <int MP, int CT>
static int launch_traj_t(const TrajArgs& ta, const ActArgs& aa, const TrajRoute& r, void* stream) {
    auto go = [&](auto kern, unsigned threads, bool full_lds = false) {
        if (full_lds && r.lds > 48 * 1024) (void)allow_full_lds(kern);
        hipLaunchKernelGGL(kern, dim3(r.blocks), dim3(threads), r.lds, (hipStream_t)stream, ta, aa);
    };
    with_km(ta.c.KP / 4, [&](auto km) {
        constexpr int KM = decltype(km)::value;
        switch (r.family) {
            case TrajFamily::Pipe:
                if constexpr (MP != MPK_MP_DMP && CT >= 3) {
                    if (r.gate) go(k_traj_pipe<MP, CT, KM, false, true>, 320);
                    else if (r.lean) go(k_traj_pipe<MP, CT, KM, true>, 320);
                    else go(k_traj_pipe<MP, CT, KM, false>, 320);
                }
                break;
            case TrajFamily::Flat:
                if constexpr (MP != MPK_MP_DMP && CT < 3) go(k_traj_flat<MP, CT, KM>, 256, true);
                break;
            case TrajFamily::Split:
                if constexpr (MP != MPK_MP_DMP && CT >= 3)
                    with_flag(r.write_through, [&](auto wt) { go(k_traj_split<MP, CT, KM, decltype(wt)::value>, 256); });
                break;
            case TrajFamily::Quarter:
                if constexpr (MP == MPK_MP_DMP || CT >= 3) {
                    if (r.nq == 1) go(k_traj_quad<MP, CT, KM, 1>, 256);
                    else if (r.nq == 2) go(k_traj_quad<MP, CT, KM, 2>, 256);
                    else go(k_traj_quad<MP, CT, KM, 4>, 256);
                }
                break;
            case TrajFamily::Stream:
                with_flag(r.bulk, [&](auto bulk) { go(k_traj_stream<MP, CT, KM, decltype(bulk)::value>, 256, decltype(bulk)::value); });
                break;
            case TrajFamily::Tiles:
                if constexpr (MP != MPK_MP_DMP && CT < 3)
                    with_flag(r.write_through, [&](auto wt) { go(k_traj_tiles<MP, CT, KM, decltype(wt)::value>, (unsigned)ta.wpb * 64u); });
                break;
            default: break;
        }
    });
    MPK_LAUNCH_CHECK();
    return MPK_OK;
}

template <int MP>
int launch_traj_ct(const TrajArgs& ta, const ActArgs& aa, const TrajRoute& r, void* stream) {
    auto go = [&](auto ct) { return launch_traj_t<MP, decltype(ct)::value>(ta, aa, r, stream); };
    if constexpr (MP == MPK_MP_DMP) return go(std::integral_constant<int, -1>());
    else return r.family == TrajFamily::Pipe || r.family == TrajFamily::Split ? with_closed_ct(r.ct, go) : with_ct(r.ct, go);
}

#ifdef MPK_MP_UNIT
template int launch_traj_ct<MPK_MP_UNIT>(const TrajArgs&, const ActArgs&, const TrajRoute&, void*);
#else
template int launch_traj_ct<MPK_MP_PROMP>(const TrajArgs&, const ActArgs&, const TrajRoute&, void*);
template int launch_traj_ct<MPK_MP_DMP>(const TrajArgs&, const ActArgs&, const TrajRoute&, void*);
template int launch_traj_ct<MPK_MP_PRODMP>(const TrajArgs&, const ActArgs&, const TrajRoute&, void*);
#endif
#endif

}
```

fancy_gym_amd/csrc/mpk_traj_launch.hip:

```cpp
#include <cstdio>

#include "mpk_tile.h"
#include "mpk_traj_quad.h"
#include "mpk_traj_pipe.h"
#include "mpk_traj_stream.h"
#include "mpk_traj_ring.h"
#include "mpk_traj_route.h"

namespace mpk {

bool shared_tables_lean(const DevCfg& c) { return c.KP > kMaxKP || c.D > kMaxD; }

size_t shared_tables_floats(const DevCfg& c, int* TS, int* n_out) {
    const int TP = (c.T + 15) / 16 * 16;
    const int ts = ((TP + 15) / 32) * 32 + 16;
    const bool lean = shared_tables_lean(c);
    const int no = c.mp_type == MPK_MP_PRODMP ? 2 : (c.mp_type == MPK_MP_PROMP && !lean ? 3 : 1);
    *TS = ts;
    *n_out = no;
    return (lean ? 1 : 2) * (size_t)no * c.KP * ts;
}

__global__ void __launch_bounds__(256) k_build_shared(const DevCfg c, const float init_time, float* __restrict__ A,
                                                      float* __restrict__ aux, const int TS, const int n_out, const int lean,
                                                      int32_t* __restrict__ idx_out, int32_t* __restrict__ flag) {
    const int tid = threadIdx.x, T = c.T, KP = c.KP;
    for (int i = tid; i < n_out * KP * TS; i += 256) A[i] = 0.0f;
    for (int i = tid; i < TS; i += 256) aux[i] = 0.0f;
    __syncthreads();
    if (c.dmp_resp) {
        const int nb = c.nb;
        for (int t = tid; t < T; t += 256) {
            const float time = c.base_times[t] + init_time;
            const double x = phase_f64(c, time, c.tau, c.delay, ExpLiteral());
            rbf_cols(c, x, x * (double)c.ws, A + t, TS);
            if (t < T - 1) {
                const float s0 = scaled_time(time, c.delay, c.tau);
                const float s1 = scaled_time(c.base_times[t + 1] + init_time, c.delay, c.tau);
                aux[t] = s1 - s0;
            }
        }
        __syncthreads();
        if (tid < nb + 3) {
            const int k = tid;
            const double al = (double)c.dmp_alpha, be = (double)c.dmp_beta, tau = (double)c.tau, itau = div_pos(1.0, (double)c.tau);
            const double G = k == nb ? (double)c.gs : 0.0;
            double y = k == nb + 1 ? 1.0 : 0.0, z = k == nb + 2 ? tau : 0.0;
            constexpr int U = 16;
            float fn[U], dn[U];
            auto fetch = [&](const int t0) {
#pragma unroll
                for (int u = 0; u < U; ++u) {
                    const int t = t0 + u < T ? t0 + u : T - 1;
                    fn[u] = k < nb ? A[(size_t)k * TS + t] : 0.0f;
                    dn[u] = aux[t];
                }
            };
            fetch(0);
            for (int t0 = 0; t0 < T; t0 += U) {
                float fv[U], dv[U];
#pragma unroll
                for (int u = 0; u < U; ++u) { fv[u] = fn[u]; dv[u] = dn[u]; }
                if (t0 + U < T) fetch(t0 + U);
#pragma unroll
                for (int u = 0; u < U; ++u) {
                    const int t = t0 + u;
                    if (t < T) {
                        A[(size_t)(0 * KP + k) * TS + t] = (float)y;
                        A[(size_t)(1 * KP + k) * TS + t] = (float)(z * itau);
                        if (t < T - 1) {
                            const double acc = al * (be * (G - y) - z) + (double)fv[u];
                            z = z + (double)dv[u] * acc;
                            y = y + (double)dv[u] * z;
                        }
                    }
                }
            }
        }
        __syncthreads();
        for (int i = tid; i < TS; i += 256) aux[i] = 0.0f;
    } else if (c.mp_type == MPK_MP_PRODMP) {
        const float sb = scaled_time(init_time, c.delay, c.tau);
        const int idxb = min(prodmp_index(sb, c.scaled_dt), c.n_pc - 1);
        ProdmpBC bc;
        prodmp_bc(c, idxb, bc);
        if (idx_out && tid == 0) idx_out[T] = idxb;
        for (int t = tid; t < T; t += 256) {
            const float time = c.base_times[t] + init_time;
            const float s = scaled_time(time, c.delay, c.tau);
            if (s > (float)c.len_factor) atomicOr(flag, 1);
            const int idx = min(prodmp_index(s, c.scaled_dt), c.n_pc - 1);
            if (idx_out) idx_out[t] = idx;
            double xi[4];
            prodmp_xi(c, bc, idx, xi);
            for (int k = 0; k < c.KT; ++k) {
                float h, hv;
                prodmp_col(c, bc, idx, xi, k, (double)c.tau, div_pos(1.0, (double)c.tau), &h, &hv);
                A[(size_t)(0 * KP + k) * TS + t] = h;
                A[(size_t)(1 * KP + k) * TS + t] = hv;
            }
        }
    } else if (c.mp_type == MPK_MP_PROMP) {
        for (int t = tid; t < T; t += 256) {
            const float time = c.base_times[t] + init_time;
            const double x = phase_f64(c, time, c.tau, c.delay, ExpLiteral());
            rbf_cols(c, x, (double)c.ws, A + t, TS);
            if (c.KT > c.nb) A[(size_t)c.nb * TS + t] = 1.0f;
        }
        __syncthreads();
        for (int t = tid; t < T; t += 256) {
            const int th = t < T - 1 ? t + 1 : T - 1, tl = t < T - 1 ? t : T - 2;
            for (int k = 0; k < c.KT && !lean; ++k) {
                A[(size_t)(1 * KP + k) * TS + t] = A[(size_t)k * TS + th];
                A[(size_t)(2 * KP + k) * TS + t] = A[(size_t)k * TS + tl];
            }
            aux[t] = 1.0f / ((c.base_times[th] + init_time) - (c.base_times[tl] + init_time));
        }
    } else {
        for (int t = tid; t < T; t += 256) {
            const float time = c.base_times[t] + init_time;
            const double x = phase_f64(c, time, c.tau, c.delay, ExpLiteral());
            rbf_cols(c, x, x * (double)c.ws, A + t, TS);
            if (t < T - 1) {
                const float s0 = scaled_time(time, c.delay, c.tau);
                const float s1 = scaled_time(c.base_times[t + 1] + init_time, c.delay, c.tau);
                aux[t] = s1 - s0;
            }
        }
    }
    __syncthreads();
    if (lean) return;
    const int RS = n_out * KP;
    float* At = A + (size_t)RS * TS;
    for (int i = tid; i < RS * TS; i += 256) {
        const int t = i / RS, e = i - t * RS;
        const int jk = n_out == 2 ? (e & 1) * KP + (e >> 1) : e;
        At[i] = A[(size_t)jk * TS + t];
    }
}

#ifndef MPK_DEVICE_ONLY
int launch_build_shared(const DevCfg& c, float init_time, const SharedTables& st, int32_t* idx_out,
                        int32_t* range_flag, void* stream) {
    if (c.mp_type == MPK_MP_PROMP && c.T < 2) {
        set_error("promp needs at least two time steps for the finite-difference velocity");
        return MPK_EINVAL;
    }
    hipLaunchKernelGGL(k_build_shared, dim3(1), dim3(256), 0, (hipStream_t)stream, c, init_time, st.A, st.aux, st.TS,
                       st.n_out, shared_tables_lean(c) ? 1 : 0, idx_out, range_flag);
    MPK_LAUNCH_CHECK();
    return MPK_OK;
}
#endif

#ifndef MPK_DEVICE_ONLY
static void fill_gate_args(const GateDev* gate, const float* params, int D, TrajArgs& ta, ActArgs& aa) {
    ta.gate_valid = nullptr; ta.gate_penalty = nullptr; ta.gate_raw = nullptr; ta.gate_check_td = 0;
    ta.gate_tb[0] = ta.gate_tb[1] = ta.gate_db[0] = ta.gate_db[1] = 0.0;
    if (!gate) return;
    ta.gate_valid = gate->valid; ta.gate_penalty = gate->penalty;
    ta.gate_raw = gate->raw_params ? gate->raw_params : params;
    ta.gate_check_td = gate->check_td;
    ta.gate_tb[0] = gate->tau_b[0]; ta.gate_tb[1] = gate->tau_b[1];
    ta.gate_db[0] = gate->delay_b[0]; ta.gate_db[1] = gate->delay_b[1];
    for (int d = 0; d < D; ++d) {
        aa.glo[d] = gate->lo[d]; aa.ghi[d] = gate->hi[d];
        aa.glo32[d] = f32_at_least(gate->lo[d]); aa.ghi32[d] = f32_at_most(gate->hi[d]);
    }
}

int plan_episode_return(const DevCfg& c, const SharedTables& st, const float* params, const float* init_pos, const float* init_vel,
                        const RolloutDev& rc, double* q_state, double* qd_state, const int32_t* n_steps, const ReplanDev* rp,
                        int reward_type, const double* goal, const int32_t* step0, int steps_before_reward, int agg, double* ret,
                        int32_t* seg_out, int B, int num_cu, const Tuning& tune, const GateDev* gate, TrajArgs& ta, ActArgs& aa,
                        EpArgs& ea, EpRoute& r) {
    ta.wpb = 4; ta.ring_parts = 1;
    if (rp) ta.rp = *rp;
    ta.q_state = q_state; ta.qd_state = qd_state; ta.n_steps = n_steps; ta.plant_dt = rc.dt;
    ta.c = c; ta.A = st.A; ta.aux = st.aux; ta.TS = st.TS;
    ta.params = params; ta.init_pos = init_pos; ta.init_vel = init_vel;
    ta.B = B;
    int sh = 0;
    while ((1 << sh) < c.D) ++sh;
    ta.sh = sh;
    const int NTW = 16 >> sh;
    ta.G = (B + NTW - 1) / NTW;
    const int SEG = 16 * c.D;
    ta.pitch = SEG; ta.cps = SEG / 4 > 0 ? SEG / 4 : 1; ta.inv_cps = 65536u / (unsigned)ta.cps + 1u; ta.vec_ok = 1;
    for (int d = 0; d < c.D; ++d) { aa.pg[d] = rc.pg[d]; aa.dg[d] = rc.dg[d]; aa.lo[d] = rc.lo[d]; aa.hi[d] = rc.hi[d]; }
    fill_gate_args(gate, params, c.D, ta, aa);
    ea.ret = ret; ea.goal = goal; ea.step0 = step0; ea.seg_out = seg_out; ea.steps_before_reward = steps_before_reward; ea.agg = agg;
    ea.km = c.KP / 4;
    const size_t table_bytes = ((size_t)st.n_out * c.KP * st.TS + st.TS) * sizeof(float);
    const long simds = (long)num_cu * 4;
    int nq = ta.G >= 4 * simds ? 4 : (ta.G >= 2 * simds ? 2 : 1);
    if (tune.quad == 2) nq = 4; else if (tune.quad == 3) nq = 2; else if (tune.quad == 4) nq = 1;
    while (reward_type && nq > 1 && nq * NTW > 4 * kEpMaxPass) nq >>= 1;
    const size_t img = reward_type ? kEpImg : kEpImgPlain;
    auto lds_of = [&](int n, int w) { return table_bytes + ((size_t)w * n * img + (size_t)w * kEpSlots * kEpSlotInts) * sizeof(float); };
    while (nq > 1 && lds_of(nq, 4) > kLdsPerCu) nq >>= 1;
    if (lds_of(nq, 4) > kLdsPerCu || (reward_type && nq * NTW > 4 * kEpMaxPass)) { set_error("trajectory too long for the episode kernel's LDS budget"); return MPK_ENOTIMPL; }
    const long units = ((long)ta.G + nq - 1) / nq;
    const long w4 = (long)(kLdsPerCu / lds_of(nq, 4)) * 4, w8 = lds_of(nq, 8) <= kLdsPerCu ? (long)(kLdsPerCu / lds_of(nq, 8)) * 8 : 0;
    int wpb = w8 > w4 && units >= 8L * num_cu ? 8 : 4;
    if (tune.tiles_wpb == 4 || tune.tiles_wpb == 8) wpb = tune.tiles_wpb == 8 && w8 > 0 ? 8 : 4;
    ea.wpb = wpb;
    r.lds = lds_of(nq, wpb);
    const long per_cu = (long)(kLdsPerCu / r.lds) < 1 ? 1 : (long)(kLdsPerCu / r.lds);
    long blocks = (units + wpb - 1) / wpb;
    const long cap = (long)num_cu * (per_cu > 8 ? 8 : per_cu);
    if (blocks > cap) blocks = cap;
    if (blocks >= 8) blocks = (blocks + 7) / 8 * 8;
    r.blocks = (int)blocks;
    r.ct = rc.controller_type + 3; r.nq = nq; r.rwd = reward_type;
    const bool pd = c.mp_type == MPK_MP_PRODMP;
    r.name = reward_type ? (pd ? "k_episode_return<prodmp,reacher>" : "k_episode_return<promp,reacher>")
                         : (pd ? "k_episode_return<prodmp>" : "k_episode_return<promp>");
    if (c.mp_type == MPK_MP_DMP) { set_error("internal: the episode kernel takes promp / prodmp rows"); return MPK_EINVAL; }
    return MPK_OK;
}

int launch_episode_return(const DevCfg& c, const SharedTables& st, const float* params, const float* init_pos, const float* init_vel,
                          const RolloutDev& rc, double* q_state, double* qd_state, const int32_t* n_steps, const ReplanDev* rp,
                          int reward_type, const double* goal, const int32_t* step0, int steps_before_reward, int agg, double* ret,
                          int32_t* seg_out, int B, int num_cu, void* stream, const char** kernel_name, const Tuning& tune,
                          const GateDev* gate) {
    TrajArgs ta{};
    ActArgs aa{};
    EpArgs ea{};
    EpRoute r{};
    const int rc_ = plan_episode_return(c, st, params, init_pos, init_vel, rc, q_state, qd_state, n_steps, rp, reward_type, goal, step0,
                                        steps_before_reward, agg, ret, seg_out, B, num_cu, tune, gate, ta, aa, ea, r);
    if (r.name) *kernel_name = r.name;
    if (rc_ != MPK_OK) return rc_;
    return by_mp_type(c.mp_type, [&](auto mp) { return launch_episode_kernel<decltype(mp)::value>(ta, aa, ea, r, stream); });
}

struct TrajFacts {
    const DevCfg& c;
    const Tuning& tune;
    int B, num_cu;
    bool dmp, closed, act, gated;
    bool ptr_ok;
    bool in_ok;
    int NTW, NRT, TD, nst;
    long max_waves;
    size_t table_bytes;
    size_t lds_pad;
    double out_bytes;
    int ov;
    bool pipe, split;
    bool serial;
    bool episode_major;
    int flat_img;
    size_t lds_flat;
    bool flat_ok, flat_takes_it;
    double stream_from;
    unsigned* ticket;
};

static int at_most(long n, long cap) { return (int)(n < cap ? n : cap); }

static bool plan_ring_open(const TrajFacts& f, TrajArgs& ta, TrajRoute& r) {
    const Tuning& tune = f.tune;
    const bool forced_other = tune.flat == 1 || tune.bulk >= 0 || tune.quad >= 0 || tune.pipe == 1 || tune.split == 1 || f.ov == 1;
    const bool want = tune.ring == 1 || (tune.ring < 0 && !forced_other && f.out_bytes > (f.flat_takes_it ? kRingTrajBytes : kRingBytes));
    int NS = tune.ring_ns > 0 ? tune.ring_ns : 2;
    int NP = tune.ring_np > 0 ? tune.ring_np : 8;
    if (NS > 8) NS = 8;
    if (NP + NS > kRingThreads / 64) NP = kRingThreads / 64 - NS;
    const size_t fixed = f.table_bytes + kRingSyncInts * sizeof(int);
    const int gimg = f.NTW * f.TD;
    auto buf_of = [&](int m) { return (size_t)f.nst * m * gimg * sizeof(float); };
    auto fits = [&](int m) { return fixed + 2 * buf_of(m) <= kLdsPerCu && ((long)m * gimg) % 4 == 0; };
    int M = tune.ring_m > 0 ? tune.ring_m : 4;
    while (M > 1 && !fits(M)) --M;
    if (!(f.ptr_ok && want && !f.closed && !f.dmp && tune.ring != 2 && fits(M))) return false;
    const size_t buf_bytes = buf_of(M);
    long nbuf = (long)((kLdsPerCu - fixed) / buf_bytes);
    if (nbuf * M > 32) nbuf = 32 / M;
    if (nbuf > 3) nbuf = 3;
    int P = tune.ring_parts > 0 ? tune.ring_parts : (int)((NP + nbuf * M - 1) / (nbuf * M));
    if (P > f.NRT) P = f.NRT;
    if (P > 8) P = 8;
    if (P < 1) P = 1;
    ta.flat_img = gimg;
    ta.ring_np = NP; ta.ring_ns = NS; ta.ring_m = M; ta.ring_nbuf = (int)nbuf; ta.ring_parts = P;
    ta.ring_ctr = f.ticket;
    ta.ring_tb = (int)((kRingTicketBytes + buf_bytes - 1) / buf_bytes);
    const long batches = ((long)ta.G + M - 1) / M;
    {
        const long fine = batches / (16L * (batches < (long)f.num_cu ? batches : (long)f.num_cu));
        if (tune.ring_tb > 0) ta.ring_tb = tune.ring_tb;
        else if ((long)ta.ring_tb > fine) ta.ring_tb = (int)fine;
    }
    if (ta.ring_tb < 1) ta.ring_tb = 1;
    while (2 * ta.ring_tb * M * P < NP) ++ta.ring_tb;
    r.family = TrajFamily::RingOpen;
    r.lds = fixed + (size_t)nbuf * buf_bytes;
    r.blocks = at_most(batches, f.num_cu);
    return true;
}

static bool plan_ring_closed(const TrajFacts& f, TrajArgs& ta, TrajRoute& r) {
    const DevCfg& c = f.c;
    const Tuning& tune = f.tune;
    if (!(f.closed && !f.gated && !f.dmp && f.act && f.ptr_ok && f.TD % 4 == 0 && (c.D == 5 || c.D == 7) && c.KP <= 8 && !f.split &&
          tune.ring != 0 && tune.ring != 2)) return false;
    const bool forced_other = tune.quad >= 0 || tune.pipe == 1 || tune.split == 1 || f.ov != 0 || tune.bulk >= 0;
    const bool want = tune.ring == 1 || (tune.ring < 0 && !forced_other && !f.pipe && f.out_bytes > kRingClosedBytes);
    int NS = tune.ring_ns > 0 ? tune.ring_ns : 1;
    int NP = tune.ring_np > 0 ? tune.ring_np : 8;
    int NC = tune.ring_nc > 0 ? tune.ring_nc : 3;
    if (NS > 4) NS = 4;
    const int AW = (ta.ring_dbg & 8) ? 0 : 1;
    if (NP + NS + NC * (1 + AW) > kRingThreadsClosed / 64) NP = kRingThreadsClosed / 64 - NS - NC * (1 + AW);
    int M = tune.ring_m > 0 && tune.ring_m < 4 ? tune.ring_m : 4;
    const int gimg = f.NTW * f.TD;
    const size_t fixed = f.table_bytes + kRingSyncInts * sizeof(int);
    const size_t stage = (size_t)NC * 4 * kStageStride * sizeof(float);
    while (M > 1 && fixed + stage + 2 * (size_t)2 * M * gimg * sizeof(float) > kLdsPerCu) --M;
    const size_t buf_bytes = (size_t)2 * M * gimg * sizeof(float);
    long nbuf = fixed + stage < kLdsPerCu ? (long)((kLdsPerCu - fixed - stage) / buf_bytes) : 0;
    if (nbuf * M > 32) nbuf = 32 / M;
    if (nbuf > 4) nbuf = 4;
    const bool ring_pays = tune.ring == 1 || M == 4;
    if (!(want && ring_pays && NP >= 1 && nbuf >= 2 && ((long)M * gimg) % 4 == 0 && 16 * c.D * f.NTW <= kStageStride)) return false;
    ta.flat_img = gimg;
    ta.ring_np = NP; ta.ring_ns = NS; ta.ring_nc = NC; ta.ring_aw = AW; ta.ring_m = M; ta.ring_nbuf = (int)nbuf; ta.ring_parts = 1;
    ta.ring_ctr = f.ticket;
    ta.ring_tb = (int)((kRingTicketBytes + buf_bytes * 3 / 2 - 1) / (buf_bytes * 3 / 2));
    if (ta.ring_tb < 2) ta.ring_tb = 2;
    if (tune.ring_tb > 0) ta.ring_tb = tune.ring_tb;
    while (2 * ta.ring_tb * M < NP) ++ta.ring_tb;
    r.family = TrajFamily::RingClosed;
    r.lds = fixed + (size_t)nbuf * buf_bytes + stage;
    r.blocks = at_most(((long)ta.G + M - 1) / M, f.num_cu);
    return true;
}

static bool plan_pipe(const TrajFacts& f, TrajArgs& ta, TrajRoute& r) {
    if (!f.pipe) return false;
    const long units = (ta.G + kPipeGroups - 1) / kPipeGroups;
    r.family = TrajFamily::Pipe;
    r.lds = f.table_bytes;
    r.blocks = at_most(units, (long)f.num_cu * 6);
    if (r.blocks >= 8) r.blocks = r.blocks / 8 * 8;
    ta.lean = units > 2 * (long)f.num_cu ? 1 : 0;
    r.gate = f.gated;
    r.lean = ta.lean && !f.gated;
    return true;
}

static bool plan_quarter(const TrajFacts& f, TrajArgs& ta, TrajRoute& r) {
    const Tuning& tune = f.tune;
    const long num_cu = f.num_cu;
    auto fits = [&](int nq) {
        return f.table_bytes + (4 * nq * kQuadImg) * sizeof(float) <= kLdsDefault;
    };
    const int quad_mode = tune.quad < 0 ? 1 : tune.quad;
    const long units4 = (ta.G + 3) / 4, units2 = (ta.G + 1) / 2;
    int nq = 0;
    if (f.serial && quad_mode != 0) {
        if (quad_mode == 2) nq = fits(4) ? 4 : 0;
        else if (quad_mode == 3) nq = fits(2) ? 2 : 0;
        else if (quad_mode == 4) nq = fits(1) ? 1 : 0;
        else if (f.dmp && fits(4)) {
            if (units4 <= num_cu * 8 && units2 > num_cu * 12) nq = 4;
            else if (fits(2) && units2 >= num_cu * 6) nq = 2;
        }
        else if (fits(4) && f.out_bytes <= kWtBytes &&
                 (units4 >= num_cu * 8 || (f.closed && units2 > num_cu * 8 && units4 <= num_cu * 8))) nq = 4;
        else if (fits(2) && units2 >= num_cu * 4) nq = 2;
        else if (f.closed && fits(1)) nq = 1;
    }
    if (f.gated && nq == 0 && f.serial && tune.quad != 0 && fits(1)) nq = 1;
    if (nq == 0) return false;
    r.family = TrajFamily::Quarter;
    r.nq = nq;
    r.gate = f.gated;
    r.lds = f.table_bytes + f.lds_pad;
    const long units = (ta.G + nq - 1) / nq;
    r.blocks = (int)((at_most(units, f.max_waves) + 3L) / 4);
    if (r.blocks >= 8) r.blocks = (r.blocks + 7) / 8 * 8;
    if (tune.serial_order >= 1) {
        ta.inorder = 1;
        if (tune.serial_order == 1) r.blocks = (int)((units + 3) / 4);
    }
    return true;
}

static bool plan_burst(const TrajFacts& f, TrajArgs& ta, TrajRoute& r) {
    const Tuning& tune = f.tune;
    if (!(f.episode_major && f.flat_ok && tune.ring == 2)) return false;
    int M = tune.ring_m > 0 ? tune.ring_m : 4;
    int WPG = tune.ring_np > 0 ? tune.ring_np : 1;
    if (M > 8) M = 8;
    if (M * WPG > 8) WPG = 8 / M < 1 ? 1 : 8 / M;
    const size_t bytes = (size_t)f.nst * M * f.flat_img * sizeof(float);
    if (f.table_bytes + bytes > kLdsPerCu) return false;
    ta.flat_img = f.flat_img;
    ta.burst = 1; ta.ring_m = M; ta.ring_np = WPG;
    r.family = TrajFamily::Burst;
    r.lds = f.table_bytes + bytes;
    r.blocks = (int)(((long)ta.G + M - 1) / M);
    return true;
}

static bool plan_flat(const TrajFacts& f, TrajArgs& ta, TrajRoute& r) {
    const DevCfg& c = f.c;
    const Tuning& tune = f.tune;
    if (!(f.episode_major && f.flat_ok && tune.flat != 0 && (tune.flat == 1 || (f.out_bytes > f.stream_from && tune.bulk < 0)))) return false;
    ta.flat_img = f.flat_img;
    r.lds = f.lds_flat + f.lds_pad;
    const long wg_cap = tune.phase_waves >= 4 ? tune.phase_waves / 4 : 2;
    const long wg = (long)(kLdsPerCu / r.lds) < wg_cap ? (long)(kLdsPerCu / r.lds) : wg_cap;
    const long resident = (long)f.num_cu * (wg < 1 ? 1 : wg) * 4;
    const bool dof_compiled = (c.D == 5 || c.D == 7) && c.KP <= 8 && !(ta.ring_dbg & 64);
    if (dof_compiled) ta.burst = 2;
    r.family = dof_compiled ? TrajFamily::FlatD : TrajFamily::Flat;
    r.blocks = (int)((at_most(ta.G, resident) + 3L) / 4);
    if (r.blocks >= 8) r.blocks = (r.blocks + 7) / 8 * 8;
    return true;
}

static bool plan_stream(const TrajFacts& f, TrajArgs& ta, TrajRoute& r) {
    const DevCfg& c = f.c;
    const Tuning& tune = f.tune;
    if (!f.episode_major) return false;
    const int EPC = kChunkGroups * f.NTW;
    const size_t img_floats = (size_t)EPC * (c.P + 2 * c.D + 4 * c.D);
    const size_t lds_bulk = f.table_bytes + 4 * 2 * img_floats * sizeof(float);
    const bool bulk_shape = (EPC * c.P) % 4 == 0 && (EPC * c.D) % 4 == 0 && (EPC * c.P) / 4 <= 128 && (EPC * c.D) / 2 <= 64 && f.in_ok &&
                            lds_bulk + 4 * kStageFloats * sizeof(float) <= kLdsDefault;
    const int bulk_mode = tune.bulk < 0 ? 1 : tune.bulk;
    const long chunks = (ta.G + kChunkGroups - 1) / kChunkGroups;
    const bool auto_ok = f.out_bytes > kCachedBytes && chunks >= f.max_waves / 2 && !f.dmp;
    r.family = TrajFamily::Stream;
    r.bulk = bulk_shape && bulk_mode != 0 && (bulk_mode == 2 || auto_ok);
    r.lds = (r.bulk ? lds_bulk : f.table_bytes) + f.lds_pad;
    long waves = at_most(r.bulk ? chunks : (long)ta.G, f.max_waves);
    if (tune.phase_waves > 0 && waves > (long)f.num_cu * tune.phase_waves) waves = (long)f.num_cu * tune.phase_waves;
    r.blocks = (int)((waves + 3) / 4);
    if (r.blocks >= 8) r.blocks = (r.blocks + 7) / 8 * 8;
    return true;
}

static void plan_tiles(const TrajFacts& f, TrajArgs& ta, TrajRoute& r) {
    const Tuning& tune = f.tune;
    const int NRT = f.NRT;
    const long items = (long)ta.G * NRT;
    long ipw = (items + f.max_waves - 1) / f.max_waves;
    if (tune.ipw > 0) ipw = tune.ipw;
    const long wave_cap = (long)((1ull << 32) / (unsigned long long)NRT) - 8 * NRT;
    if ((items + ipw - 1) / ipw > wave_cap) ipw = (items + wave_cap - 1) / wave_cap;
    const long waves = (items + ipw - 1) / ipw;
    const int wpb = (tune.tiles_wpb == 1 || tune.tiles_wpb == 2) && !f.split ? tune.tiles_wpb : 4;
    ta.wpb = wpb;
    int blocks = (int)((waves + wpb - 1) / wpb);
    {
        int g8 = 8, rem = NRT;
        while (rem) { const int t = g8 % rem; g8 = rem; rem = t; }
        const int unit = blocks >= 8 ? NRT / g8 * 8 : NRT;
        blocks = (blocks + unit - 1) / unit * unit;
    }
    ta.gstride = blocks * wpb / NRT;
    ta.nrt_magic = NRT > 1 ? (unsigned)((1ull << 32) / (unsigned long long)NRT) + 1u : 0u;
    if (blocks < 1) blocks = 1;
    r.family = TrajFamily::Tiles;
    r.lds = f.lds_pad;
    if (f.split) {
        const int EPW = 64 >> ta.sh;
        const long units = ((long)f.B + EPW - 1) / EPW;
        ta.ser_blocks = (unsigned)at_most((units + 3) / 4, (long)f.num_cu * 8);
        blocks += (int)ta.ser_blocks;
        r.family = TrajFamily::Split;
    }
    r.blocks = blocks;
}

static const char* traj_kernel_name(const TrajRoute& r, int mp_type, bool act, bool closed) {
#define MPK_NAMES(k)                                                           \
    {{k "<promp>", k "<promp,act>", k "<promp,closed>", k "<promp,closed,gate>"}, \
     {k "<dmp>", k "<dmp>", k "<dmp>", k "<dmp>"},                                \
     {k "<prodmp>", k "<prodmp,act>", k "<prodmp,closed>", k "<prodmp,closed,gate>"}}
    static const char* const names[][3][4] = {
        MPK_NAMES("k_traj_tiles"), MPK_NAMES("k_traj_split"), MPK_NAMES("k_traj_stream"), MPK_NAMES("k_traj_flat"), MPK_NAMES("k_traj_burst"),
        MPK_NAMES("k_traj_quad"), MPK_NAMES("k_traj_duo"), MPK_NAMES("k_traj_mono"), MPK_NAMES("k_traj_pipe"), MPK_NAMES("k_traj_ring")};
#undef MPK_NAMES
    static_assert(MPK_MP_PROMP == 0 && MPK_MP_DMP == 1 && MPK_MP_PRODMP == 2, "the table's MP rows");
    int k = 0;
    switch (r.family) {
        case TrajFamily::Tiles: k = 0; break;
        case TrajFamily::Split: k = 1; break;
        case TrajFamily::Stream: k = 2; break;
        case TrajFamily::Flat: case TrajFamily::FlatD: k = 3; break;
        case TrajFamily::Burst: k = 4; break;
        case TrajFamily::Quarter: k = r.nq == 4 ? 5 : r.nq == 2 ? 6 : 7; break;
        case TrajFamily::Pipe: k = 8; break;
        case TrajFamily::RingOpen: case TrajFamily::RingClosed: k = 9; break;
    }
    return names[k][mp_type][r.gate ? 3 : closed ? 2 : act ? 1 : 0];
}

int plan_traj_shared(const DevCfg& c, const SharedTables& st, const float* params, const float* init_pos, const float* init_vel,
                     float* pos, float* vel, float* actions, const RolloutDev* rc, const double* c_pos, const double* c_vel,
                     double* q_state, double* qd_state, const int32_t* n_steps, int B, int num_cu, const Tuning& tune, const ReplanDev* rp,
                     unsigned* ticket, int* fault, const GateDev* gate, TrajArgs& ta, ActArgs& aa, TrajRoute& r) {
    TrajFacts f{c, tune};
    f.B = B; f.num_cu = num_cu; f.ticket = ticket;
    f.dmp = c.mp_type == MPK_MP_DMP;
    f.closed = q_state != nullptr;
    f.act = actions != nullptr;
    f.gated = gate != nullptr;
    const bool dmp = f.dmp, closed = f.closed, act = f.act, gated = f.gated;
    if (gated && !(closed && act)) { set_error("the validity gate belongs to the closed-loop step"); return MPK_EINVAL; }
    ta.fault = fault;
    ta.ring_dbg = tune.ring_dbg > 0 ? tune.ring_dbg : 0;
    if (tune.ablations != 1) ta.ring_dbg &= ~(1 | 2 | 128 | (closed ? 0 : 8));
    ta.wpb = 4; ta.ring_parts = 1;
    if (rp) ta.rp = *rp;
    ta.q_state = q_state; ta.qd_state = qd_state; ta.n_steps = n_steps; ta.plant_dt = rc ? rc->dt : 0.0;
    ta.c = c; ta.A = st.A; ta.aux = st.aux; ta.TS = st.TS;
    ta.params = params; ta.init_pos = init_pos; ta.init_vel = init_vel;
    ta.pos = pos; ta.vel = vel; ta.actions = actions; ta.c_pos = c_pos; ta.c_vel = c_vel;
    ta.B = B;
    int sh = 0;
    while ((1 << sh) < c.D) ++sh;
    ta.sh = sh;
    const int NTW = f.NTW = 16 >> sh;
    ta.G = (B + NTW - 1) / NTW;
    f.nst = 2 + (act ? 1 : 0);
    const int SEG = 16 * c.D, seg4 = SEG / 4, TD = f.TD = c.T * c.D;
    auto aligned16 = [](const void* p) { return (reinterpret_cast<uintptr_t>(p) & 15u) == 0; };
    const bool ptr_ok = f.ptr_ok = aligned16(pos) && aligned16(vel) && (!act || aligned16(actions));
    f.in_ok = aligned16(params) && aligned16(init_pos) && aligned16(init_vel) && (!act || closed || (aligned16(c_pos) && aligned16(c_vel)));
    ta.shifted = (ptr_ok && TD % 4 != 0 && NTW * (seg4 + 1) <= 64 && NTW * (SEG + 4) <= kStageStride) ? 1 : 0;
    ta.td3 = TD & 3;
    ta.pitch = ta.shifted ? SEG + 4 : SEG;
    ta.cps = ta.shifted ? seg4 + 1 : seg4;
    ta.inv_cps = 65536u / (unsigned)ta.cps + 1u;
    ta.vec_ok = ptr_ok && (TD % 4 == 0 || ta.shifted);
    int ct = -1;
    if (act) {
        ct = rc->controller_type + (closed ? 3 : 0);
        for (int d = 0; d < c.D; ++d) { aa.pg[d] = rc->pg[d]; aa.dg[d] = rc->dg[d]; aa.lo[d] = rc->lo[d]; aa.hi[d] = rc->hi[d]; }
    }
    fill_gate_args(gate, params, c.D, ta, aa);
    f.NRT = (c.T + 15) / 16;
    f.max_waves = (long)num_cu * 32;
    f.lds_pad = tune.lds_pad > 0 ? (size_t)tune.lds_pad * 1024 : 0;
    const size_t table_bytes = f.table_bytes = ((size_t)st.n_out * c.KP * st.TS + st.TS) * sizeof(float);
    const double out_bytes = f.out_bytes = (double)B * c.T * c.D * 4.0 * f.nst;
    const int ov = f.ov = tune.mapping == 1 || tune.mapping == 2 ? tune.mapping : 0;
    const bool variant_forced = ov == 2 || tune.quad == 0 || tune.quad >= 2 || tune.bulk == 2;
    const int last_rows = c.T - (c.T - 1) / 16 * 16;
    const bool split_shape = ptr_ok && TD % 4 == 0 && (last_rows * c.D) % 4 == 0;
    const bool pipe_fits = table_bytes + 2 * kPipeGroups * kQuadImg * sizeof(float) <= kLdsDefault;
    const long pipe_units = ((long)ta.G + kPipeGroups - 1) / kPipeGroups;
    f.pipe = closed && !dmp && pipe_fits && tune.split != 1 &&
             (tune.pipe == 1 || (tune.pipe != 0 && !variant_forced && pipe_units <= (gated ? 1L : 3L) * num_cu));
    f.split = !f.pipe && closed && !gated && !dmp && split_shape && tune.split == 1;
    f.flat_img = (NTW * TD + 3) / 4 * 4;
    f.lds_flat = table_bytes + (size_t)4 * f.nst * f.flat_img * sizeof(float);
    f.flat_ok = !closed && !dmp && ptr_ok && TD % 4 == 0 && f.lds_flat <= kLdsHalf;
    f.flat_takes_it = !act && f.flat_ok && tune.flat != 0;
    f.stream_from = f.flat_takes_it && tune.bulk < 0 ? kFlatTrajBytes : kCachedBytes;
    f.serial = (dmp || closed) && !f.split;
    const bool open_episode_major = !dmp && !closed && (ov == 2 || tune.flat == 1 || tune.ring >= 1 || (ov != 1 && out_bytes > f.stream_from));
    const bool stream_fits = table_bytes + 4 * kStageFloats * sizeof(float) <= kLdsDefault;
    if (f.serial && !stream_fits) { set_error("trajectory too long for the episode-major kernel's LDS budget"); return MPK_ENOTIMPL; }
    f.episode_major = f.serial || (open_episode_major && stream_fits);

    r = TrajRoute{};
    r.ct = dmp ? -1 : ct;
    if (!(plan_ring_open(f, ta, r) || plan_ring_closed(f, ta, r) || plan_pipe(f, ta, r) || plan_quarter(f, ta, r))) {
        if (gated) return MPK_ENOTIMPL;
        if (!(plan_burst(f, ta, r) || plan_flat(f, ta, r) || plan_stream(f, ta, r))) plan_tiles(f, ta, r);
    }
    if (r.blocks < 1) r.blocks = 1;
    const bool tile_major = r.family == TrajFamily::Tiles || r.family == TrajFamily::Split;
    if (tile_major && ta.gstride <= 0) { set_error("internal: tile-major launch without its group stride"); return MPK_EINVAL; }
    bool wt = tune.write_through >= 0 ? tune.write_through != 0 : (tile_major || out_bytes <= kWtBytes);
    if ((double)B * c.T * c.D * 4.0 >= 2147483648.0) wt = false;
    r.write_through = tile_major && wt;
    ta.wt = !tile_major && wt ? 1 : 0;
    r.name = traj_kernel_name(r, gated && dmp ? MPK_MP_PROMP : c.mp_type, act, closed);
    return gated && dmp ? MPK_ENOTIMPL : MPK_OK;
}

int launch_traj_shared(const DevCfg& c, const SharedTables& st, const float* params, const float* init_pos,
                       const float* init_vel, float* pos, float* vel, float* actions, const RolloutDev* rc,
                       const double* c_pos, const double* c_vel, double* q_state, double* qd_state,
                       const int32_t* n_steps, int B, int num_cu, void* stream, const char** kernel_name,
                       const Tuning& tune, const ReplanDev* rp, unsigned* ticket, int* fault, const GateDev* gate) {
    TrajArgs ta{};
    ActArgs aa{};
    TrajRoute r{};
    const int rc_ = plan_traj_shared(c, st, params, init_pos, init_vel, pos, vel, actions, rc, c_pos, c_vel, q_state, qd_state, n_steps, B,
                                     num_cu, tune, rp, ticket, fault, gate, ta, aa, r);
    if (r.name) *kernel_name = r.name;
    if (rc_ != MPK_OK) return rc_;
    switch (r.family) {
        case TrajFamily::RingOpen: case TrajFamily::RingClosed: case TrajFamily::Burst: case TrajFamily::FlatD:
            return by_mp_type(c.mp_type, [&](auto mp) { return launch_traj_ring<decltype(mp)::value>(ta, aa, r, stream); });
        default:
            return by_mp_type(c.mp_type, [&](auto mp) { return launch_traj_ct<decltype(mp)::value>(ta, aa, r, stream); });
    }
}
#endif

}
```

fancy_gym_amd/csrc/mpk_traj_route.h:

```cpp
#pragma once
#include "mpk_tile.h"

namespace mpk {

enum class TrajFamily : int {
    Tiles,
    Split,
    Stream,
    Flat,
    FlatD,
    Burst,
    Quarter,
    Pipe,
    RingOpen,
    RingClosed,
};

struct TrajRoute {
    TrajFamily family;
    int ct;
    bool write_through;
    bool bulk;
    int nq;
    bool lean, gate;
    int blocks;
    size_t lds;
    const char* name;
};

struct EpRoute {
    int ct, nq, rwd, blocks;
    size_t lds;
    const char* name;
};

#ifndef MPK_DEVICE_ONLY
int plan_traj_shared(const DevCfg& c, const SharedTables& st, const float* params, const float* init_pos, const float* init_vel,
                     float* pos, float* vel, float* actions, const RolloutDev* rc, const double* c_pos, const double* c_vel,
                     double* q_state, double* qd_state, const int32_t* n_steps, int B, int num_cu, const Tuning& tune, const ReplanDev* rp,
                     unsigned* ticket, int* fault, const GateDev* gate, TrajArgs& ta, ActArgs& aa, TrajRoute& r);
int plan_episode_return(const DevCfg& c, const SharedTables& st, const float* params, const float* init_pos, const float* init_vel,
                        const RolloutDev& rc, double* q_state, double* qd_state, const int32_t* n_steps, const ReplanDev* rp,
                        int reward_type, const double* goal, const int32_t* step0, int steps_before_reward, int agg, double* ret,
                        int32_t* seg_out, int B, int num_cu, const Tuning& tune, const GateDev* gate, TrajArgs& ta, ActArgs& aa,
                        EpArgs& ea, EpRoute& r);

template <int MP>
int launch_traj_ct(const TrajArgs& ta, const ActArgs& aa, const TrajRoute& r, void* stream);
template <int MP>
int launch_traj_ring(const TrajArgs& ta, const ActArgs& aa, const TrajRoute& r, void* stream);
template <int MP>
int launch_episode_kernel(const TrajArgs& ta, const ActArgs& aa, const EpArgs& ea, const EpRoute& r, void* stream);
#ifndef MPK_AMALGAMATED
#define MPK_ROUTE_LAUNCHERS(MP)                                                                                         \
    extern template int launch_traj_ct<MP>(const TrajArgs&, const ActArgs&, const TrajRoute&, void*);                   \
    extern template int launch_traj_ring<MP>(const TrajArgs&, const ActArgs&, const TrajRoute&, void*);                 \
    extern template int launch_episode_kernel<MP>(const TrajArgs&, const ActArgs&, const EpArgs&, const EpRoute&, void*);
MPK_ROUTE_LAUNCHERS(MPK_MP_PROMP)
MPK_ROUTE_LAUNCHERS(MPK_MP_DMP)
MPK_ROUTE_LAUNCHERS(MPK_MP_PRODMP)
#undef MPK_ROUTE_LAUNCHERS
#endif

template <typename F>
int by_mp_type(int mp_type, F&& f) {
    switch (mp_type) {
        case MPK_MP_PRODMP: return f(std::integral_constant<int, MPK_MP_PRODMP>());
        case MPK_MP_PROMP: return f(std::integral_constant<int, MPK_MP_PROMP>());
        default: return f(std::integral_constant<int, MPK_MP_DMP>());
    }
}

template <typename F>
void with_km(int km, F&& f) {
    switch (km) {
        case 1: f(std::integral_constant<int, 1>()); break;
        case 2: f(std::integral_constant<int, 2>()); break;
        case 3: f(std::integral_constant<int, 3>()); break;
        default: f(std::integral_constant<int, 4>()); break;
    }
}

template <typename F>
void with_flag(bool on, F&& f) {
    if (on) f(std::true_type()); else f(std::false_type());
}

template <typename F>
int with_closed_ct(int ct, F&& f) {
    switch (ct) {
        case 3 + MPK_CTRL_MOTOR: return f(std::integral_constant<int, 3 + MPK_CTRL_MOTOR>());
        case 3 + MPK_CTRL_VELOCITY: return f(std::integral_constant<int, 3 + MPK_CTRL_VELOCITY>());
        default: return f(std::integral_constant<int, 3 + MPK_CTRL_POSITION>());
    }
}

template <typename F>
int with_ct(int ct, F&& f) {
    switch (ct) {
        case MPK_CTRL_MOTOR: return f(std::integral_constant<int, MPK_CTRL_MOTOR>());
        case MPK_CTRL_VELOCITY: return f(std::integral_constant<int, MPK_CTRL_VELOCITY>());
        case MPK_CTRL_POSITION: return f(std::integral_constant<int, MPK_CTRL_POSITION>());
        case 3 + MPK_CTRL_MOTOR: case 3 + MPK_CTRL_VELOCITY: case 3 + MPK_CTRL_POSITION: return with_closed_ct(ct, f);
        default: return f(std::integral_constant<int, -1>());
    }
}
#endif

}
```

fancy_gym_amd/csrc/mpk_traj_tiles.h:

```cpp
#pragma once
#include "mpk_tile.h"

namespace mpk {

template <int MP, int CT, int KM, bool WT>
__device__ __forceinline__ void tiles_body(const TrajArgs& a, float* smem, const unsigned bid, const unsigned nblk) {
    static_assert(MP != MPK_MP_DMP, "dmp runs in k_traj_stream");
    static_assert(CT < 3, "closed-loop rollouts run in k_traj_stream / k_traj_split");
    constexpr bool ACT = CT >= 0;
    constexpr int NOUT = MP == MPK_MP_PRODMP ? 2 : 3;
    constexpr int NST = 2 + (ACT ? 1 : 0);
    const DevCfg& c = a.c;
    const int lane = threadIdx.x & 63;
    const int wave = __builtin_amdgcn_readfirstlane(threadIdx.x >> 6);
    const int KP = 4 * KM, TS = a.TS, D = c.D, T = c.T;
    float* sSt = smem + wave * kStageFloats;
    const LaneMap<KM> L = make_lane_map<MP, KM>(a, lane);
    const int NRT = (T + 15) >> 4;
    const int nb8 = (int)(nblk >> 3);
    const int vb = (nblk & 7) == 0 ? (int)(bid & 7) * nb8 + (int)(bid >> 3) : (int)bid;
    const int wid = vb * a.wpb + wave;
    const int gstride = a.gstride;
    int g = a.nrt_magic ? (int)__umulhi((unsigned)wid, a.nrt_magic) : wid;
    const int rt = wid - g * NRT;
    if (g >= a.G) return;
    MPK_STAMP(1);
    GroupIn<KM> cur = load_group<MP, ACT, KM>(a, L, g);
    Gains kg{0.0, 0.0, 0.0, 0.0};
    if (ACT) kg = kernarg_gains(L.dvalid ? L.d : 0);
    float af[NOUT][KM];
#pragma unroll
    for (int j = 0; j < NOUT; ++j)
#pragma unroll
        for (int m = 0; m < KM; ++m) af[j][m] = a.A[(size_t)(j * KP + 4 * m + L.q) * TS + rt * 16 + L.col];
    float dtd[4] = {1.f, 1.f, 1.f, 1.f};
    if (MP == MPK_MP_PROMP) {
#pragma unroll
        for (int r = 0; r < 4; ++r) dtd[r] = a.aux[rt * 16 + 4 * L.q + r];
    }
    const int rows = min(16, T - rt * 16);

    float xb[KM];
    finish_group<KM>(L, cur, xb);
    double cp = cur.cp, cv = cur.cv;
    MPK_STAMP(2);
    while (g < a.G) {
        const int gn = g + gstride;
        const GroupIn<KM> nxt = load_group<MP, ACT, KM>(a, L, gn < a.G ? gn : g);
        f32x4 acc0 = {0.f, 0.f, 0.f, 0.f}, acc1 = {0.f, 0.f, 0.f, 0.f}, acc2 = {0.f, 0.f, 0.f, 0.f};
#pragma unroll
        for (int m = 0; m < KM; ++m) {
            acc0 = __builtin_amdgcn_mfma_f32_16x16x4f32(af[0][m], xb[m], acc0, 0, 0, 0);
            acc1 = __builtin_amdgcn_mfma_f32_16x16x4f32(af[1][m], xb[m], acc1, 0, 0, 0);
            if (NOUT > 2) acc2 = __builtin_amdgcn_mfma_f32_16x16x4f32(af[NOUT > 2 ? 2 : 0][m], xb[m], acc2, 0, 0, 0);
        }
        if (L.dvalid)
            tile_epilogue<MP, CT>(acc0, acc1, acc2, dtd, cp, cv, kg, sSt, L.wofs + ep_shift(a, g * L.NTW + L.bl), D);
        __builtin_amdgcn_wave_barrier();
        MPK_STAMP(10);
#if MPK_TILES_COLLECT_FIRST
        finish_group<KM>(L, nxt, xb);
        asm volatile("" : "+v"(xb[0]));
        tile_store<NST, KM, WT>(a, L, sSt, lane, g * L.NTW, rt, rows);
        __builtin_amdgcn_wave_barrier();
        MPK_STAMP(11);
#else
        tile_store<NST, KM, WT>(a, L, sSt, lane, g * L.NTW, rt, rows);
        __builtin_amdgcn_wave_barrier();
        MPK_STAMP(11);
        finish_group<KM>(L, nxt, xb);
#endif
        cp = nxt.cp; cv = nxt.cv;
        g = gn;
    }
#ifdef MPK_TRACE
    MPK_STAMP(20);
    asm volatile("s_waitcnt vmcnt(0)" ::: "memory");
    MPK_STAMP(21);
#endif
}

#ifndef MPK_TILES_OCC
#ifndef MPK_TILES_COLLECT_FIRST
#define MPK_TILES_COLLECT_FIRST 0
#endif
#define MPK_TILES_OCC 7
#endif
template <int MP, int CT, int KM, bool WT>
__global__ void __launch_bounds__(256, (KM <= 2 ? MPK_TILES_OCC : 1)) k_traj_tiles(const TrajArgs a, const ActArgs act) {
    __shared__ __attribute__((aligned(16))) float smem[4 * kStageFloats];
    demand_args(a, gridDim.x);
    tiles_body<MP, CT, KM, WT>(a, smem, blockIdx.x, gridDim.x);
}

template <int MP, int CT, int KM, bool WT>
__device__ __forceinline__ void serial_body(const TrajArgs& a, const float* __restrict__ At,
                                            const float* __restrict__ aux, float* smem) {
    static_assert(CT >= 3, "closed loop only");
    constexpr int KP = 4 * KM;
    constexpr int NOUT = MP == MPK_MP_PRODMP ? 2 : 3;
    constexpr int RS = NOUT * KP;
    const DevCfg& c = a.c;
    const int lane = threadIdx.x & 63;
    const int wave = __builtin_amdgcn_readfirstlane(threadIdx.x >> 6);
    const int D = c.D, T = c.T, B = a.B, P = c.P;
    const int DP = 1 << a.sh, EPW = 64 >> a.sh;
    const int e = lane >> a.sh, d = lane & (DP - 1);
    const bool dvalid = d < D;
    float* sAct = smem + wave * (kStageFloats + 16 * RS);
    const int NRT = (T + 15) >> 4;
    const int units = (B + EPW - 1) / EPW;
    const int ustride = (int)a.ser_blocks * 4;
    const Gains gn = kernarg_gains(dvalid ? d : 0);
    const double pgd = gn.pg, dgd = gn.dg, lod = __builtin_canonicalize(gn.lo), hid = __builtin_canonicalize(gn.hi),
                 dtp = a.plant_dt;
    const int cps = a.cps;
    MPK_STAMP(1);
    MPK_STAMP(2);
    for (int u = (int)blockIdx.x * 4 + wave; u < units; u += ustride) {
        const int b = u * EPW + e;
        const bool on = dvalid && b < B;
        const int bs = on ? b : 0, ds = dvalid ? d : 0;
        float raw[KP];
        const float* prm = a.params + (size_t)bs * P + c.off + ds * c.Kloc;
        int kinds[KP];
#pragma unroll
        for (int k = 0; k < KP; ++k) {
            int loc;
            kinds[k] = x_kind<MP>(c, k, &loc);
            raw[k] = prm[loc];
        }
        const float ipv = a.init_pos[(size_t)bs * D + ds];
        const float ivv = MP == MPK_MP_PRODMP ? a.init_vel[(size_t)bs * D + ds] : 0.0f;
        const size_t si0 = (size_t)bs * D + ds;
        double qs = a.q_state[si0], qds = a.qd_state[si0];
        int nst = 0;
        if (on) {
            nst = T;
            if (a.rp.traj_steps) nst = replan_rule(a.rp, b, T, d == 0);
            else if (a.n_steps) nst = min(a.n_steps[b], T);
        }
        float (&x)[KP] = raw;
#pragma unroll
        for (int k = 0; k < KP; ++k) {
            const float v = kinds[k] == XK_PARAM ? raw[k] : (kinds[k] == XK_IPOS ? ipv : (kinds[k] == XK_IVEL ? ivv : (kinds[k] == XK_ONE ? 1.0f : 0.0f)));
            x[k] = on ? v : 0.0f;
        }
        const int tcond = (on && a.rp.cond_pos) ? min(max(nst - 1, 0), T - 1) : -1;
        int need = on ? max(nst, tcond + 1) : 0;
#pragma unroll
        for (int m = 32; m >= 1; m >>= 1) need = max(need, __shfl_xor(need, m));
        const int n_ser = __builtin_amdgcn_readfirstlane((need + 15) >> 4);
        float cpos = 0.0f, cvel = 0.0f;
        float* const ub = a.actions + (size_t)u * EPW * T * D;
        unsigned sgo[4], slds[4], sw4[4];
        bool sval[4];
#pragma unroll
        for (int i = 0; i < 4; ++i) {
            const int ch = lane + 64 * i;
            const int sg = (int)(((unsigned)ch * a.inv_cps) >> 16);
            const int w4 = (ch - sg * cps) * 4;
            sval[i] = sg < EPW && u * EPW + sg < B;
            sw4[i] = (unsigned)w4;
            sgo[i] = (unsigned)(sg * T * D + w4);
            slds[i] = (unsigned)(sg * 16 * D + w4);
        }
        MPK_STAMP(3);
        float* const slot = sAct + (dvalid ? e * (16 * D) + d : EPW * 16 * D);
        const int sstep = dvalid ? D : 0;
        float* const sRow = sAct + kStageFloats;
        constexpr int NR4 = 16 * RS / 4;
        constexpr int NRR = (NR4 + 63) / 64;
        f32x4 rr[NRR];
#pragma unroll
        for (int i = 0; i < NRR; ++i) rr[i] = f32x4{0.f, 0.f, 0.f, 0.f};
        auto fetch_rows = [&](int rt) {
            const f32x4* src = reinterpret_cast<const f32x4*>(At + (size_t)rt * 16 * RS);
#pragma unroll
            for (int i = 0; i < NRR; ++i)
                if (lane + 64 * i < NR4) rr[i] = src[lane + 64 * i];
        };
        auto park_rows = [&]() {
#pragma unroll
            for (int i = 0; i < NRR; ++i)
                if (lane + 64 * i < NR4) reinterpret_cast<f32x4*>(sRow)[lane + 64 * i] = rr[i];
        };
        if (n_ser > 0) fetch_rows(0);
        for (int rt = 0; rt < NRT; ++rt) {
            const int rows = min(16, T - rt * 16);
            if (rt < n_ser) {
                park_rows();
                __builtin_amdgcn_wave_barrier();
                if (rt + 1 < n_ser) fetch_rows(rt + 1);
                auto read_row = [&](int tl, float (&r)[RS]) {
#pragma unroll
                    for (int k4 = 0; k4 < RS / 4; ++k4) {
                        const f32x4 q4 = reinterpret_cast<const f32x4*>(sRow + tl * RS)[k4];
                        r[4 * k4] = q4[0]; r[4 * k4 + 1] = q4[1]; r[4 * k4 + 2] = q4[2]; r[4 * k4 + 3] = q4[3];
                    }
                };
                auto one_step = [&](auto masked_tag, int tl, const float (&rc)[RS]) {
                    constexpr bool MASKED = decltype(masked_tag)::value;
                    const int t = rt * 16 + tl;
                    float p = 0.0f, v = 0.0f;
                    if (MP == MPK_MP_PRODMP) {
#pragma unroll
                        for (int k = 0; k < KP; ++k) { p = fmaf(rc[2 * k], x[k], p); v = fmaf(rc[2 * k + 1], x[k], v); }
                    } else {
                        float ph = 0.0f, pl = 0.0f;
#pragma unroll
                        for (int k = 0; k < KP; ++k) {
                            p = fmaf(rc[k], x[k], p);
                            ph = fmaf(rc[KP + k], x[k], ph); pl = fmaf(rc[2 * KP + k], x[k], pl);
                        }
                        v = (ph - pl) * aux[t];
                    }
                    if (MASKED) {
                        const bool at_cond = t == tcond;
                        cpos = at_cond ? p : cpos; cvel = at_cond ? v : cvel;
                    }
                    const double dp = (double)p, dv = (double)v;
                    double uu;
                    if (CT - 3 == MPK_CTRL_MOTOR) uu = pgd * (dp - qs) + dgd * (dv - qds);
                    else if (CT - 3 == MPK_CTRL_POSITION) uu = dp;
                    else uu = dv;
                    uu = clip_f64(uu, lod, hid);
                    const double qds_n = qds + dtp * uu;
                    const double qs_n = qs + dtp * qds_n;
                    if (MASKED) {
                        const bool live = t < nst;
                        qds = live ? qds_n : qds;
                        qs = live ? qs_n : qs;
                        slot[tl * sstep] = live ? (float)uu : 0.0f;
                    } else {
                        qds = qds_n; qs = qs_n;
                        slot[tl * sstep] = (float)uu;
                    }
                };
                auto tile_steps = [&](auto masked_tag) {
                    float r0[RS], r1[RS];
                    read_row(0, r0);
#pragma unroll 1
                    for (int tl = 0; tl < 16; tl += 2) {
                        read_row(tl + 1, r1);
                        one_step(masked_tag, tl, r0);
// ... 48 lines not shown
```

Before: 489.4 million trajectories/s.

## Add phase-aligned tile mapping so tile stores start on 64-byte boundaries

Adds a phased variant of the tile kernel that groups episodes into residue classes by their offset modulo 16 rows and picks per-class row cut points. Each row tile then starts at a cache-line-aligned output address, which should cut the number of partial 64-byte write requests when T*D is not a multiple of 16 floats. The route is taken by default when outputs are 64-byte aligned, write-through is on, and the period is greater than one. In exchange the kernel has extra per-class indexing and may run one more row tile per episode, and a host option reports whether the phased path was used.

```diff
diff --git a/fancy_gym_amd/_lib.py b/fancy_gym_amd/_lib.py
--- a/fancy_gym_amd/_lib.py
+++ b/fancy_gym_amd/_lib.py
@@ -24,7 +24,7 @@
 REWARD_TYPES = {None: 0, "none": 0, "simple_reacher": 1}
 AGG_MODES = {"sum": 0, "mean": 1, "last": 2}
 OPTION_KEYS = ("mapping", "bulk", "quad", "pd_quad", "write_through", "ipw", "phase", "phase_table", "phase_chunk",
-               "pd_simple", "split", "lds_pad", "pipe", "flat", "phase_flat", "ring", "ring_np", "ring_ns", "ring_m", "ring_dbg", "ring_parts", "tiles_wpb", "serial_order", "ring_nc", "pd_generic", "dmp_response", "ablations", "ring_tb", "pd_helper", "phase_waves", "phase_split", "phase_pipe", "pd_pipe", "hole_sampled", "vjp_generic")
+               "pd_simple", "split", "lds_pad", "pipe", "flat", "phase_flat", "ring", "ring_np", "ring_ns", "ring_m", "ring_dbg", "ring_parts", "tiles_wpb", "serial_order", "ring_nc", "pd_generic", "dmp_response", "ablations", "ring_tb", "pd_helper", "phase_waves", "phase_split", "phase_pipe", "pd_pipe", "hole_sampled", "vjp_generic", "tiles_phase")
 
 
 class MPKLibraryError(RuntimeError):
@@ -202,7 +202,7 @@
 KERNEL_UNITS = ("mpk_traj_family.hip", "mpk_traj_ring.hip", "mpk_episode.hip", "mpk_traj_launch.hip", "mpk_traj_wide.hip", "mpk_traj_vjp.hip", "mpk_traj_phase.hip",
                 "mpk_phase_fused.hip", "mpk_rollout.hip", "mpk_rollout_vjp.hip", "mpk_hole.hip", "mpk_reset.hip", "mpk_obs.hip", "mpk_autoreset.hip", "mpk_env_step.hip", "mpk_misc.hip")
 KERNEL_HEADERS = ("mpk_dev.h", "mpk_tile.h", "mpk_traj_tiles.h", "mpk_traj_stream.h", "mpk_traj_flat.h", "mpk_traj_ring.h", "mpk_traj_quad.h",
-                  "mpk_traj_pipe.h", "mpk_traj_route.h", "mpk_reward.h", "mpk_phase.h", "mpk_trace_reader.h", "mpk_nprng.h", "mpk_plant.h", "mpk_reacher_env.h", "mpk_hole_geom.h")
+                  "mpk_traj_pipe.h", "mpk_traj_route.h", "mpk_tile_phase.h", "mpk_reward.h", "mpk_phase.h", "mpk_trace_reader.h", "mpk_nprng.h", "mpk_plant.h", "mpk_reacher_env.h", "mpk_hole_geom.h")
 SOURCE_FILES = (os.path.join(_ROOT, "include", "mpk.h"), os.path.join(_HERE, "csrc", "mpk_internal.h"),
                 os.path.join(_HERE, "csrc", "mpk_host.cpp")) + \
     tuple(os.path.join(_HERE, "csrc", f) for f in KERNEL_HEADERS + KERNEL_UNITS)
diff --git a/fancy_gym_amd/csrc/mpk_host.cpp b/fancy_gym_amd/csrc/mpk_host.cpp
--- a/fancy_gym_amd/csrc/mpk_host.cpp
+++ b/fancy_gym_amd/csrc/mpk_host.cpp
@@ -210,6 +210,7 @@
     std::string kernel_name_buf;
     uint64_t stamp = 0;
     const char* last_kernel = "";
+    int last_tiles_phased = 0;
     Tuning tune;
     float* d_pre = nullptr;
     size_t pre_cap = 0;
@@ -683,7 +684,7 @@
     {"pd_helper", &Tuning::pd_helper, 0, 1},     {"phase_waves", &Tuning::phase_waves, 1, 32},
     {"phase_split", &Tuning::phase_split, 1, 64},   {"phase_pipe", &Tuning::phase_pipe, 0, 1},
     {"pd_pipe", &Tuning::pd_pipe, 0, 1},         {"hole_sampled", &Tuning::hole_sampled, 0, 1},
-    {"vjp_generic", &Tuning::vjp_generic, 0, 1},
+    {"vjp_generic", &Tuning::vjp_generic, 0, 1}, {"tiles_phase", &Tuning::tiles_phase, 0, 1},
 };
 const OptKey* find_opt(const char* key) {
     if (!key) return nullptr;
@@ -715,6 +716,10 @@
 }
 
 int mpk_get_option(mpk_handle hh, const char* key, int64_t* value) {
+    if (hh && key && value && std::strcmp(key, "tiles_phased") == 0) {
+        *value = reinterpret_cast<Handle*>(hh)->last_tiles_phased;
+        return MPK_OK;
+    }
     const OptKey* k = find_opt(key);
     if (!k || !value) { set_error(std::string("unknown option key: ") + (key ? key : "(null)")); return MPK_EINVAL; }
     const Tuning t = hh ? effective_tuning(reinterpret_cast<Handle*>(hh)) : g_tune;
@@ -888,7 +893,7 @@
         unsigned* ticket = ticket_slot(h, stream);
         const char* name = "";
         rc = launch_traj_shared(h->dev_resp, st, params, init_pos, init_vel, pos, vel, actions, rd, c_pos, c_vel,
-                                q_state, qd_state, n_steps, B, h->num_cu, stream, &name, tune, rp, ticket, h->d_fault, gate);
+                                q_state, qd_state, n_steps, B, h->num_cu, stream, &name, tune, rp, ticket, h->d_fault, gate, &h->last_tiles_phased);
         if (rc == MPK_OK) {
             h->kernel_name_buf = name;
             const size_t at = h->kernel_name_buf.find("prodmp");
@@ -903,7 +908,8 @@
         if (rc != MPK_OK) return rc;
         unsigned* ticket = ticket_slot(h, stream);
         rc = launch_traj_shared(h->dev, st, params, init_pos, init_vel, pos, vel, actions, rd, c_pos, c_vel,
-                                q_state, qd_state, n_steps, B, h->num_cu, stream, &h->last_kernel, tune, rp, ticket, h->d_fault, gate);
+                                q_state, qd_state, n_steps, B, h->num_cu, stream, &h->last_kernel, tune, rp, ticket, h->d_fault, gate,
+                                &h->last_tiles_phased);
         if (rc != MPK_ENOTIMPL || actions) return rc;
     }
     if (actions) { set_error("fused actions need a shared-phase configuration with D <= 16 and <= 16 basis columns"); return MPK_ENOTIMPL; }
diff --git a/fancy_gym_amd/csrc/mpk_internal.h b/fancy_gym_amd/csrc/mpk_internal.h
--- a/fancy_gym_amd/csrc/mpk_internal.h
+++ b/fancy_gym_amd/csrc/mpk_internal.h
@@ -29,7 +29,7 @@
         phase_chunk = -1, pd_simple = -1, split = -1, lds_pad = -1, pipe = -1, flat = -1, phase_flat = -1,
         ring = -1, ring_np = -1, ring_ns = -1, ring_m = -1, ring_dbg = -1, ring_parts = -1, tiles_wpb = -1, serial_order = -1, ring_nc = -1,
         pd_generic = -1, dmp_response = -1, ablations = -1, ring_tb = -1, pd_helper = -1, phase_waves = -1, phase_split = -1, phase_pipe = -1, pd_pipe = -1,
-        hole_sampled = -1, vjp_generic = -1;
+        hole_sampled = -1, vjp_generic = -1, tiles_phase = -1;
 };
 
 struct DevCfg {
@@ -107,7 +107,7 @@
                        const double* c_pos, const double* c_vel, double* q_state, double* qd_state,
                        const int32_t* n_steps, int B, int num_cu, void* stream, const char** kernel_name,
                        const Tuning& tune, const ReplanDev* rp = nullptr, unsigned* ticket = nullptr, int* fault = nullptr,
-                       const GateDev* gate = nullptr);
+                       const GateDev* gate = nullptr, int* phased = nullptr);
 int launch_episode_return(const DevCfg& c, const SharedTables& st, const float* params, const float* init_pos, const float* init_vel,
                           const RolloutDev& rc, double* q_state, double* qd_state, const int32_t* n_steps, const ReplanDev* rp,
                           int reward_type, const double* goal, const int32_t* step0, int steps_before_reward, int agg, double* ret,
diff --git a/fancy_gym_amd/csrc/mpk_tile.h b/fancy_gym_amd/csrc/mpk_tile.h
--- a/fancy_gym_amd/csrc/mpk_tile.h
+++ b/fancy_gym_amd/csrc/mpk_tile.h
@@ -46,6 +46,8 @@
     const float* gate_raw;
     int gate_check_td;
     double gate_tb[2], gate_db[2];
+    int ph_pd, ph_sh, ph_nrt;
+    unsigned ph_s[4];
 };
 
 struct ActArgs {
@@ -111,7 +113,7 @@
 };
 
 template <int MP, int KM>
-__device__ __forceinline__ LaneMap<KM> make_lane_map(const TrajArgs& a, int lane) {
+__device__ __forceinline__ LaneMap<KM> make_lane_map(const TrajArgs& a, int lane, const int es = 1) {
     const DevCfg& c = a.c;
     LaneMap<KM> L;
     const int D = c.D, DP = 1 << a.sh;
@@ -128,14 +130,14 @@
         L.isip[m] = L.dvalid && kind == XK_IPOS;
         L.isiv[m] = L.dvalid && kind == XK_IVEL;
         L.cst[m] = L.dvalid && kind == XK_ONE ? 1.0f : 0.0f;
-        L.poff[m] = (unsigned)(L.bl * c.P + c.off + L.dsafe * c.Kloc + loc);
-    }
-    L.ioff = (unsigned)(L.bl * D + L.dsafe);
+        L.poff[m] = (unsigned)(L.bl * es * c.P + c.off + L.dsafe * c.Kloc + loc);
+    }
+    L.ioff = (unsigned)(L.bl * es * D + L.dsafe);
     L.wofs = (unsigned)(L.bl * a.pitch + 4 * L.q * D + L.d);
     L.sseg = (int)(((unsigned)lane * a.inv_cps) >> 16);
     L.w4 = (lane - L.sseg * a.cps) * 4;
     L.rofs = (unsigned)(L.sseg * a.pitch + L.w4);
-    L.gofs = (unsigned)(L.sseg * c.T * D + L.w4);
+    L.gofs = (unsigned)(L.sseg * es * c.T * D + L.w4);
     return L;
 }
 
@@ -156,14 +158,13 @@
 }
 
 template <int MP, bool ACT, int KM>
-__device__ __forceinline__ GroupIn<KM> load_group(const TrajArgs& a, const LaneMap<KM>& L, int g) {
+__device__ __forceinline__ GroupIn<KM> load_group_at(const TrajArgs& a, const LaneMap<KM>& L, const int b0, const int es) {
     const DevCfg& c = a.c;
     GroupIn<KM> in;
-    const int b0 = g * L.NTW;
-    const bool bv = b0 + L.bl < a.B;
+    const bool bv = b0 + L.bl * es < a.B;
     const float* pb = a.params + (size_t)b0 * c.P;
     const unsigned io = bv ? L.ioff : (unsigned)L.dsafe;
-    const unsigned pclamp = bv ? 0u : (unsigned)(L.bl * c.P);
+    const unsigned pclamp = bv ? 0u : (unsigned)(L.bl * es * c.P);
 #pragma unroll
     for (int m = 0; m < KM; ++m) in.raw[m] = ld_off(pb, 4u * (L.poff[m] - pclamp));
     in.ip = MP != MPK_MP_DMP ? ld_off(a.init_pos + (size_t)b0 * c.D, 4u * io) : 0.0f;
@@ -171,6 +172,11 @@
     in.cp = 0.0; in.cv = 0.0;
     if (ACT) { in.cp = ld_off(a.c_pos + (size_t)b0 * c.D, 8u * io); in.cv = ld_off(a.c_vel + (size_t)b0 * c.D, 8u * io); }
     return in;
+}
+
+template <int MP, bool ACT, int KM>
+__device__ __forceinline__ GroupIn<KM> load_group(const TrajArgs& a, const LaneMap<KM>& L, int g) {
+    return load_group_at<MP, ACT, KM>(a, L, g * L.NTW, 1);
 }
 
 template <int KM>
@@ -614,18 +620,19 @@
     __builtin_amdgcn_raw_buffer_store_b128(__builtin_bit_cast(i32x4_t, v), r, (int)off, 0, MPK_STORE_AUX);
 }
 
-template <int MASK, int KM, bool WT>
+template <int MASK, int KM, bool WT, bool PH = false>
 __device__ __forceinline__ void tile_store_sel(const TrajArgs& a, const LaneMap<KM>& L, const float* sSt, int lane,
-                                               int b0, int rt, int rows) {
+                                               int b0, int rt, int rows, const int es = 1) {
     constexpr bool SP = (MASK & 1) != 0, SV = (MASK & 2) != 0, SA = (MASK & 4) != 0;
     const int D = a.c.D, T = a.c.T, len = rows * D;
-    if (a.vec_ok) {
-        const int bb = b0 + L.sseg;
-        const int lo = (int)ep_shift(a, bb), hi = lo + len, c0 = L.w4;
+    const int row0 = PH ? rt : rt * 16;
+    if (PH || a.vec_ok) {
+        const int bb = b0 + L.sseg * es;
+        const int lo = PH ? 0 : (int)ep_shift(a, bb), hi = lo + len, c0 = L.w4;
         const bool in_seg = L.sseg < L.NTW && bb < a.B && c0 < hi && c0 + 4 > lo;
         if (WT && MPK_WT_PRED) {
             const bool whole = in_seg && c0 >= lo && c0 + 4 <= hi;
-            const unsigned off = whole ? (unsigned)((((size_t)bb * T + rt * 16) * D - lo + c0) * sizeof(float)) : kWtSkip;
+            const unsigned off = whole ? (unsigned)((((size_t)bb * T + row0) * D - lo + c0) * sizeof(float)) : kWtSkip;
             const unsigned ro = L.sseg < L.NTW ? L.rofs : 0u;
             if (SP) wt_store16(wt_rsrc(a.pos), off, *reinterpret_cast<const f32x4*>(sSt + ro));
             if (SV) wt_store16(wt_rsrc(a.vel), off, *reinterpret_cast<const f32x4*>(sSt + kStageStride + ro));
@@ -633,7 +640,7 @@
             if (!a.shifted) return;
         }
         if (in_seg) {
-            const size_t go = ((size_t)bb * T + rt * 16) * D - lo + c0;
+            const size_t go = ((size_t)bb * T + row0) * D - lo + c0;
             f32x4 d0 = {0.f, 0.f, 0.f, 0.f}, d1 = d0, d2 = d0;
             if (SP) d0 = *reinterpret_cast<const f32x4*>(sSt + L.rofs);
             if (SV) d1 = *reinterpret_cast<const f32x4*>(sSt + kStageStride + L.rofs);
@@ -671,10 +678,10 @@
     }
 }
 
-template <int NST, int KM, bool WT>
+template <int NST, int KM, bool WT, bool PH = false>
 __device__ __forceinline__ void tile_store(const TrajArgs& a, const LaneMap<KM>& L, const float* sSt, int lane,
-                                           int b0, int rt, int rows) {
-    tile_store_sel<(NST > 2 ? 7 : 3), KM, WT>(a, L, sSt, lane, b0, rt, rows);
+                                           int b0, int rt, int rows, const int es = 1) {
+    tile_store_sel<(NST > 2 ? 7 : 3), KM, WT, PH>(a, L, sSt, lane, b0, rt, rows, es);
 }
 
 __device__ __forceinline__ void demand_args(const TrajArgs& a, unsigned grid_x) {
diff --git a/fancy_gym_amd/csrc/mpk_tile_phase.h b/fancy_gym_amd/csrc/mpk_tile_phase.h
--- /dev/null
+++ b/fancy_gym_amd/csrc/mpk_tile_phase.h
@@ -0,0 +1,55 @@
+#pragma once
+
+namespace mpk {
+
+inline int tile_phase_gcd(int a, int b) {
+    while (b) { const int t = a % b; a = b; b = t; }
+    return a;
+}
+
+inline int tile_phase_m(int D) { return 16 / tile_phase_gcd(D, 16); }
+
+inline int tile_phase_period(int D, int T) {
+    const int m = tile_phase_m(D);
+    return m / tile_phase_gcd(T % m, m);
+}
+
+inline int tile_phase_cut(int D, int T, long e) {
+    const int m = tile_phase_m(D);
+    return 16 - (int)(((long)e * T) % m);
+}
+
+inline int tile_phase_tiles(int T, int s) { return s >= T ? 1 : 1 + (T - s + 15) / 16; }
+
+inline int tile_phase_max_tiles(int D, int T) {
+    const int pd = tile_phase_period(D, T);
+    int n = 1;
+    for (int c = 0; c < pd; ++c) {
+        const int t = tile_phase_tiles(T, tile_phase_cut(D, T, c));
+        if (t > n) n = t;
+    }
+    return n;
+}
+
+inline int tile_phase_rows(int T, int s, int rt, int* r0) {
+    *r0 = rt ? s + 16 * (rt - 1) : 0;
+    const int left = T - *r0;
+    return rt ? (left < 16 ? left : 16) : (s < T ? s : T);
+}
+
+inline long tile_phase_requests(int D, int T, long B, bool phased) {
+    long n = 0;
+    for (long e = 0; e < B; ++e) {
+        const int s = phased ? tile_phase_cut(D, T, e) : 16;
+        const int nt = tile_phase_tiles(T, s);
+        for (int rt = 0; rt < nt; ++rt) {
+            int r0;
+            const int rows = tile_phase_rows(T, s, rt, &r0);
+            const long lo = 4L * D * (e * T + r0), hi = lo + 4L * D * rows;
+            n += (hi + 63) / 64 - lo / 64;
+        }
+    }
+    return n;
+}
+
+}
diff --git a/fancy_gym_amd/csrc/mpk_traj_family.hip b/fancy_gym_amd/csrc/mpk_traj_family.hip
--- a/fancy_gym_amd/csrc/mpk_traj_family.hip
+++ b/fancy_gym_amd/csrc/mpk_traj_family.hip
@@ -42,8 +42,10 @@
                 with_flag(r.bulk, [&](auto bulk) { go(k_traj_stream<MP, CT, KM, decltype(bulk)::value>, 256, decltype(bulk)::value); });
                 break;
             case TrajFamily::Tiles:
-                if constexpr (MP != MPK_MP_DMP && CT < 3)
-                    with_flag(r.write_through, [&](auto wt) { go(k_traj_tiles<MP, CT, KM, decltype(wt)::value>, (unsigned)ta.wpb * 64u); });
+                if constexpr (MP != MPK_MP_DMP && CT < 3) {
+                    if (r.phased) go(k_traj_tiles<MP, CT, KM, true, true>, (unsigned)ta.wpb * 64u);
+                    else with_flag(r.write_through, [&](auto wt) { go(k_traj_tiles<MP, CT, KM, decltype(wt)::value>, (unsigned)ta.wpb * 64u); });
+                }
                 break;
             default: break;
         }
diff --git a/fancy_gym_amd/csrc/mpk_traj_launch.hip b/fancy_gym_amd/csrc/mpk_traj_launch.hip
--- a/fancy_gym_amd/csrc/mpk_traj_launch.hip
+++ b/fancy_gym_amd/csrc/mpk_traj_launch.hip
@@ -6,6 +6,7 @@
 #include "mpk_traj_stream.h"
 #include "mpk_traj_ring.h"
 #include "mpk_traj_route.h"
+#include "mpk_tile_phase.h"
 
 namespace mpk {
 
@@ -242,6 +243,8 @@
     int B, num_cu;
     bool dmp, closed, act, gated;
     bool ptr_ok;
+    bool out64;
+    bool wt_tiles;
     bool in_ok;
     int NTW, NRT, TD, nst;
     long max_waves;
@@ -448,7 +451,18 @@
 
 static void plan_tiles(const TrajFacts& f, TrajArgs& ta, TrajRoute& r) {
     const Tuning& tune = f.tune;
-    const int NRT = f.NRT;
+    const int Pd = tile_phase_period(f.c.D, f.c.T);
+    const bool phased = !f.split && !f.gated && f.wt_tiles && ta.vec_ok && !ta.shifted && f.out64 && Pd > 1 && tune.tiles_phase != 0;
+    if (phased) {
+        const long slab = (long)f.NTW * Pd;
+        ta.G = (int)(((long)f.B + slab - 1) / slab * Pd);
+        ta.ph_pd = Pd;
+        ta.ph_sh = 0;
+        while ((1 << ta.ph_sh) < Pd) ++ta.ph_sh;
+        ta.ph_nrt = tile_phase_max_tiles(f.c.D, f.c.T);
+        for (int c = 0; c < 16; ++c) ta.ph_s[c >> 2] |= (unsigned)tile_phase_cut(f.c.D, f.c.T, c % Pd) << (8 * (c & 3));
+    }
+    const int NRT = phased ? ta.ph_nrt : f.NRT;
     const long items = (long)ta.G * NRT;
     long ipw = (items + f.max_waves - 1) / f.max_waves;
     if (tune.ipw > 0) ipw = tune.ipw;
@@ -461,13 +475,18 @@
     {
         int g8 = 8, rem = NRT;
         while (rem) { const int t = g8 % rem; g8 = rem; rem = t; }
-        const int unit = blocks >= 8 ? NRT / g8 * 8 : NRT;
+        int unit = blocks >= 8 ? NRT / g8 * 8 : NRT;
+        if (phased) {
+            const int q = NRT * Pd / tile_phase_gcd(NRT * Pd, wpb);
+            unit = blocks >= 8 ? q / tile_phase_gcd(q, 8) * 8 : q;
+        }
         blocks = (blocks + unit - 1) / unit * unit;
     }
     ta.gstride = blocks * wpb / NRT;
     ta.nrt_magic = NRT > 1 ? (unsigned)((1ull << 32) / (unsigned long long)NRT) + 1u : 0u;
     if (blocks < 1) blocks = 1;
     r.family = TrajFamily::Tiles;
+    r.phased = phased;
     r.lds = f.lds_pad;
     if (f.split) {
         const int EPW = 64 >> ta.sh;
@@ -534,6 +553,8 @@
     const int SEG = 16 * c.D, seg4 = SEG / 4, TD = f.TD = c.T * c.D;
     auto aligned16 = [](const void* p) { return (reinterpret_cast<uintptr_t>(p) & 15u) == 0; };
     const bool ptr_ok = f.ptr_ok = aligned16(pos) && aligned16(vel) && (!act || aligned16(actions));
+    auto aligned64 = [](const void* p) { return (reinterpret_cast<uintptr_t>(p) & 63u) == 0; };
+    f.out64 = aligned64(pos) && aligned64(vel) && (!act || aligned64(actions));
     f.in_ok = aligned16(params) && aligned16(init_pos) && aligned16(init_vel) && (!act || closed || (aligned16(c_pos) && aligned16(c_vel)));
     ta.shifted = (ptr_ok && TD % 4 != 0 && NTW * (seg4 + 1) <= 64 && NTW * (SEG + 4) <= kStageStride) ? 1 : 0;
     ta.td3 = TD & 3;
@@ -572,6 +593,8 @@
     if (f.serial && !stream_fits) { set_error("trajectory too long for the episode-major kernel's LDS budget"); return MPK_ENOTIMPL; }
     f.episode_major = f.serial || (open_episode_major && stream_fits);
 
+    const bool wt_fits = (double)B * c.T * c.D * 4.0 < 2147483648.0;
+    f.wt_tiles = wt_fits && (tune.write_through >= 0 ? tune.write_through != 0 : true);
     r = TrajRoute{};
     r.ct = dmp ? -1 : ct;
     if (!(plan_ring_open(f, ta, r) || plan_ring_closed(f, ta, r) || plan_pipe(f, ta, r) || plan_quarter(f, ta, r))) {
@@ -582,7 +605,7 @@
     const bool tile_major = r.family == TrajFamily::Tiles || r.family == TrajFamily::Split;
     if (tile_major && ta.gstride <= 0) { set_error("internal: tile-major launch without its group stride"); return MPK_EINVAL; }
     bool wt = tune.write_through >= 0 ? tune.write_through != 0 : (tile_major || out_bytes <= kWtBytes);
-    if ((double)B * c.T * c.D * 4.0 >= 2147483648.0) wt = false;
+    if (!wt_fits) wt = false;
     r.write_through = tile_major && wt;
     ta.wt = !tile_major && wt ? 1 : 0;
     r.name = traj_kernel_name(r, gated && dmp ? MPK_MP_PROMP : c.mp_type, act, closed);
@@ -593,14 +616,16 @@
                        const float* init_vel, float* pos, float* vel, float* actions, const RolloutDev* rc,
                        const double* c_pos, const double* c_vel, double* q_state, double* qd_state,
                        const int32_t* n_steps, int B, int num_cu, void* stream, const char** kernel_name,
-                       const Tuning& tune, const ReplanDev* rp, unsigned* ticket, int* fault, const GateDev* gate) {
+                       const Tuning& tune, const ReplanDev* rp, unsigned* ticket, int* fault, const GateDev* gate, int* phased) {
     TrajArgs ta{};
     ActArgs aa{};
     TrajRoute r{};
+    if (phased) *phased = 0;
     const int rc_ = plan_traj_shared(c, st, params, init_pos, init_vel, pos, vel, actions, rc, c_pos, c_vel, q_state, qd_state, n_steps, B,
                                      num_cu, tune, rp, ticket, fault, gate, ta, aa, r);
     if (r.name) *kernel_name = r.name;
     if (rc_ != MPK_OK) return rc_;
+    if (phased) *phased = r.phased ? 1 : 0;
     switch (r.family) {
         case TrajFamily::RingOpen: case TrajFamily::RingClosed: case TrajFamily::Burst: case TrajFamily::FlatD:
             return by_mp_type(c.mp_type, [&](auto mp) { return launch_traj_ring<decltype(mp)::value>(ta, aa, r, stream); });
diff --git a/fancy_gym_amd/csrc/mpk_traj_route.h b/fancy_gym_amd/csrc/mpk_traj_route.h
--- a/fancy_gym_amd/csrc/mpk_traj_route.h
+++ b/fancy_gym_amd/csrc/mpk_traj_route.h
@@ -20,6 +20,7 @@
     TrajFamily family;
     int ct;
     bool write_through;
+    bool phased;
     bool bulk;
     int nq;
     bool lean, gate;
diff --git a/fancy_gym_amd/csrc/mpk_traj_tiles.h b/fancy_gym_amd/csrc/mpk_traj_tiles.h
--- a/fancy_gym_amd/csrc/mpk_traj_tiles.h
+++ b/fancy_gym_amd/csrc/mpk_traj_tiles.h
@@ -3,7 +3,7 @@
 
 namespace mpk {
 
-template <int MP, int CT, int KM, bool WT>
+template <int MP, int CT, int KM, bool WT, bool PH = false>
 __device__ __forceinline__ void tiles_body(const TrajArgs& a, float* smem, const unsigned bid, const unsigned nblk) {
     static_assert(MP != MPK_MP_DMP, "dmp runs in k_traj_stream");
     static_assert(CT < 3, "closed-loop rollouts run in k_traj_stream / k_traj_split");
@@ -15,38 +15,52 @@
     const int wave = __builtin_amdgcn_readfirstlane(threadIdx.x >> 6);
     const int KP = 4 * KM, TS = a.TS, D = c.D, T = c.T;
     float* sSt = smem + wave * kStageFloats;
-    const LaneMap<KM> L = make_lane_map<MP, KM>(a, lane);
-    const int NRT = (T + 15) >> 4;
+    const int es = PH ? a.ph_pd : 1;
+    const LaneMap<KM> L = make_lane_map<MP, KM>(a, lane, es);
+    const int NRT = PH ? a.ph_nrt : (T + 15) >> 4;
     const int nb8 = (int)(nblk >> 3);
     const int vb = (nblk & 7) == 0 ? (int)(bid & 7) * nb8 + (int)(bid >> 3) : (int)bid;
     const int wid = vb * a.wpb + wave;
     const int gstride = a.gstride;
     int g = a.nrt_magic ? (int)__umulhi((unsigned)wid, a.nrt_magic) : wid;
     const int rt = wid - g * NRT;
-    if (g >= a.G) return;
+    auto first_ep = [&](const int gg) { return PH ? ((gg >> a.ph_sh) * L.NTW << a.ph_sh) + (gg & (es - 1)) : gg * L.NTW; };
+    auto live = [&](const int gg) { return PH ? first_ep(gg) < a.B : gg < a.G; };
+    if (!live(g)) return;
+    int R0 = 0, rows = 0;
+    if (PH) {
+        const int cls = g & (es - 1);
+        const unsigned w01 = (cls & 4) ? a.ph_s[1] : a.ph_s[0], w23 = (cls & 4) ? a.ph_s[3] : a.ph_s[2];
+        const int s = (int)((((cls & 8) ? w23 : w01) >> ((cls & 3) * 8)) & 0xffu);
+        R0 = rt ? s + 16 * (rt - 1) : 0;
+        rows = rt ? min(16, T - R0) : min(s, T);
+        if (rows <= 0) return;
+    }
     MPK_STAMP(1);
-    GroupIn<KM> cur = load_group<MP, ACT, KM>(a, L, g);
+    GroupIn<KM> cur = load_group_at<MP, ACT, KM>(a, L, first_ep(g), es);
     Gains kg{0.0, 0.0, 0.0, 0.0};
     if (ACT) kg = kernarg_gains(L.dvalid ? L.d : 0);
     float af[NOUT][KM];
 #pragma unroll
     for (int j = 0; j < NOUT; ++j)
 #pragma unroll
-        for (int m = 0; m < KM; ++m) af[j][m] = a.A[(size_t)(j * KP + 4 * m + L.q) * TS + rt * 16 + L.col];
+        for (int m = 0; m < KM; ++m)
+            af[j][m] = PH ? a.A[(size_t)(j * KP + 4 * m + L.q) * TS + min(R0 + L.col, T - 1)]
+                          : a.A[(size_t)(j * KP + 4 * m + L.q) * TS + rt * 16 + L.col];
     float dtd[4] = {1.f, 1.f, 1.f, 1.f};
     if (MP == MPK_MP_PROMP) {
 #pragma unroll
-        for (int r = 0; r < 4; ++r) dtd[r] = a.aux[rt * 16 + 4 * L.q + r];
+        for (int r = 0; r < 4; ++r) dtd[r] = PH ? a.aux[min(R0 + 4 * L.q + r, T - 1)] : a.aux[rt * 16 + 4 * L.q + r];
     }
-    const int rows = min(16, T - rt * 16);
+    if (!PH) rows = min(16, T - rt * 16);
 
     float xb[KM];
     finish_group<KM>(L, cur, xb);
     double cp = cur.cp, cv = cur.cv;
     MPK_STAMP(2);
-    while (g < a.G) {
+    while (live(g)) {
         const int gn = g + gstride;
-        const GroupIn<KM> nxt = load_group<MP, ACT, KM>(a, L, gn < a.G ? gn : g);
+        const GroupIn<KM> nxt = load_group_at<MP, ACT, KM>(a, L, first_ep(live(gn) ? gn : g), es);
         f32x4 acc0 = {0.f, 0.f, 0.f, 0.f}, acc1 = {0.f, 0.f, 0.f, 0.f}, acc2 = {0.f, 0.f, 0.f, 0.f};
 #pragma unroll
         for (int m = 0; m < KM; ++m) {
@@ -55,17 +69,17 @@
             if (NOUT > 2) acc2 = __builtin_amdgcn_mfma_f32_16x16x4f32(af[NOUT > 2 ? 2 : 0][m], xb[m], acc2, 0, 0, 0);
         }
         if (L.dvalid)
-            tile_epilogue<MP, CT>(acc0, acc1, acc2, dtd, cp, cv, kg, sSt, L.wofs + ep_shift(a, g * L.NTW + L.bl), D);
+            tile_epilogue<MP, CT>(acc0, acc1, acc2, dtd, cp, cv, kg, sSt, PH ? L.wofs : L.wofs + ep_shift(a, g * L.NTW + L.bl), D);
         __builtin_amdgcn_wave_barrier();
         MPK_STAMP(10);
 #if MPK_TILES_COLLECT_FIRST
         finish_group<KM>(L, nxt, xb);
         asm volatile("" : "+v"(xb[0]));
-        tile_store<NST, KM, WT>(a, L, sSt, lane, g * L.NTW, rt, rows);
+        tile_store<NST, KM, WT, PH>(a, L, sSt, lane, first_ep(g), PH ? R0 : rt, rows, es);
         __builtin_amdgcn_wave_barrier();
         MPK_STAMP(11);
 #else
-        tile_store<NST, KM, WT>(a, L, sSt, lane, g * L.NTW, rt, rows);
+        tile_store<NST, KM, WT, PH>(a, L, sSt, lane, first_ep(g), PH ? R0 : rt, rows, es);
         __builtin_amdgcn_wave_barrier();
         MPK_STAMP(11);
         finish_group<KM>(L, nxt, xb);
@@ -86,11 +100,12 @@
 #endif
 #define MPK_TILES_OCC 7
 #endif
-template <int MP, int CT, int KM, bool WT>
+template <int MP, int CT, int KM, bool WT, bool PH = false>
 __global__ void __launch_bounds__(256, (KM <= 2 ? MPK_TILES_OCC : 1)) k_traj_tiles(const TrajArgs a, const ActArgs act) {
     __shared__ __attribute__((aligned(16))) float smem[4 * kStageFloats];
     demand_args(a, gridDim.x);
-    tiles_body<MP, CT, KM, WT>(a, smem, blockIdx.x, gridDim.x);
+    if (PH) asm volatile("" ::"s"(a.ph_pd), "s"(a.ph_sh), "s"(a.ph_nrt), "s"(a.ph_s[0]), "s"(a.ph_s[1]), "s"(a.ph_s[2]), "s"(a.ph_s[3]));
+    tiles_body<MP, CT, KM, WT, PH>(a, smem, blockIdx.x, gridDim.x);
 }
 
 template <int MP, int CT, int KM, bool WT>
```

Result: slower. 472.6 million trajectories/s (-3.4%).
